# sandialabs/PyNucleus

Measured on AMD Instinct MI355X. Metric: element-pairs/sec assembled (2D P1 fractional s=0.5, dense) + % fp64 roofline, higher is better.
Workload: dtype f64; 1 GPU; 2D unit disc (uniform_disc refined 7x, 98304 cells), P1, 48769 DoFs, fractional s=0.5, horizon=inf, dense getDense incl. zeroExterior; 4831887360 element pairs/step; noRef=7, num_dofs=48769, num_cells=98304, parallelism=block rows of the upper triangle dealt over 1 GPU(s), row-owned one-sided slabs

## Files before the change

include/pnl_hip.h:

```cpp
#ifndef PNL_HIP_H
#define PNL_HIP_H
#include <stdint.h>

#ifdef __cplusplus
extern "C" {
#endif

typedef struct pnl_context pnl_context;

enum pnl_status {
    PNL_OK = 0,
    PNL_ERR_INVALID = -1,
    PNL_ERR_UNSUPPORTED = -2,
    PNL_ERR_HIP = -3,
    PNL_ERR_STATE = -4,
    PNL_ERR_ORDER = -5
};

enum pnl_kernel_type { PNL_FRACTIONAL = 0, PNL_INDICATOR = 1, PNL_PERIDYNAMIC = 2, PNL_GAUSSIAN = 3, PNL_EXPONENTIAL = 4,
                       PNL_GAUSSIAN_BOUNDARY = 5, PNL_EXPONENTIAL_BOUNDARY = 6 };

typedef struct {
    int32_t ktype;
    int32_t interaction;
    double exponent;
    double scale;
    double horizon2;
} pnl_kernel;

typedef struct {
    double c0, a, b, e, den0;
    int32_t clip_num;
    int32_t pad;
} pnl_order_formula;

#define PNL_INTERIOR 0
#define PNL_BOUNDARY 1

enum pnl_counter {
    PNL_C_NUM_CELL_PAIRS = 0,
    PNL_C_NUM_ASSEMBLED_CELL_PAIRS,
    PNL_C_NUM_INTEGRATIONS,
    PNL_C_NUM_BOUNDARY_PAIRS,
    PNL_C_NUM_BOUNDARY_INTEGRATIONS,
    PNL_C_ORDER_OVERFLOW,
    PNL_C_UNIFORM_TILE_PAIRS,
    PNL_C_RESERVED7,
    PNL_C_HIST0 = 8,
    PNL_C_UNIFORM_Q2 = 131,
    PNL_C_SETTLED_TILES = 134,
    PNL_C_CODE_BUILDS = 135,
    PNL_C_WORKLIST_LENGTH = 136
};
#define PNL_NUM_COUNTERS 137

int pnl_set_option(const char *name, const char *value);

enum { PNL_SELFTEST_LOG = 0, PNL_SELFTEST_EXP = 1, PNL_SELFTEST_EXP_RANGED = 2, PNL_SELFTEST_KERNEL = 3, PNL_SELFTEST_SCALING = 4,
       PNL_SELFTEST_QORDER = 5, PNL_SELFTEST_SETTLED_LAYOUT = 6 };
#define PNL_SELFTEST_DISPATCH 100
int pnl_selftest(int op, int path, int dim, int boundary, const void *param, int n, const double *in, double *out);

int pnl_create(int device_id, pnl_context **ctx);
void pnl_destroy(pnl_context *ctx);
const char *pnl_error_string(pnl_context *ctx);
const char *pnl_version(void);
int pnl_set_stream(pnl_context *ctx, void *hip_stream);
int pnl_synchronize(pnl_context *ctx);

int pnl_upload_mesh(pnl_context *ctx, int dim, int nv, const double *vertices_host, int nc, const int32_t *cells_host,
                    const double *vol_host, const double *h_host, double H0);
int pnl_set_cell_order(pnl_context *ctx, int nc, const int32_t *orig_host);
int pnl_set_interaction_transform(pnl_context *ctx, int dim, const double *T_host);
int pnl_upload_dofmap(pnl_context *ctx, int dpe, int dofs_per_vertex, int dofs_per_edge, int num_dofs,
                      const int32_t *dofs_host, const int32_t *dof_perm_table_host);
int pnl_set_classes(pnl_context *ctx, int nclasses, int num_labels, const int32_t *cell_labels_host,
                    const int32_t *facet_labels_host, const int32_t *cls_of_host);
int pnl_set_nonsymmetric(pnl_context *ctx, int on);
int pnl_select_class(pnl_context *ctx, int k);
int pnl_set_kernel(pnl_context *ctx, int which, const pnl_kernel *kernel);
int pnl_set_order_formula(pnl_context *ctx, int which, const pnl_order_formula *formula);
int pnl_upload_distant_rules(pnl_context *ctx, int qmax, const int32_t *off_host, const double *bary_host,
                             const double *w_host, const double *phi_host, const int32_t *foff_host,
                             const double *fbary_host, const double *fw_host);
int pnl_upload_singular_rule(pnl_context *ctx, int which, int panel, int M, int rows, const double *nodes_host,
                             const double *w_host, const double *psi_host, double fac);
int pnl_upload_boundary(pnl_context *ctx, int nb, const int32_t *bcells_host);

int pnl_assemble_pairs_in_horizon(pnl_context *ctx, double *data, double *diag);
int pnl_assemble_pairs_in_horizon_range(pnl_context *ctx, double *data_dev, double *diag_dev, int cell_begin, int cell_end);

#define PNL_FLAG_NO_MIRROR 1
#define PNL_FLAG_SYMMETRIC_FLUSH 2
int pnl_assemble_dense(pnl_context *ctx, double *A_dev, int64_t ldA, int zero_exterior, int cell_begin, int cell_end,
                       int flags);
int pnl_block_row_costs(pnl_context *ctx, double *cost_out, int n);
int pnl_dense_overwrites(pnl_context *ctx, int cell_begin, int cell_end, int flags);
int pnl_tile_cells(pnl_context *ctx);
int pnl_assemble_dense_tiles(pnl_context *ctx, double *A_dev, int64_t ldA, int zero_exterior, int ntiles,
                             const int32_t *tiles_host, int cell_begin, int cell_end, int flags);
int pnl_upload_sparsity(pnl_context *ctx, int nnz, const int32_t *indptr_host, const int32_t *indices_host);
int pnl_upload_sparsity_device(pnl_context *ctx, int nnz, const int32_t *indptr_dev, const int32_t *indices_dev);
int pnl_assemble_pairs_masked(pnl_context *ctx, int np, const int32_t *pairs_host, const uint64_t *masks_host,
                              double *data_dev, double *diag_dev);
int pnl_assemble_boundary_masked(pnl_context *ctx, int ni, const int32_t *cells_host, const int32_t *facets_host,
                                 const uint32_t *masks_host, double fac, double *data_dev, double *diag_dev);
typedef struct {
    int32_t npairs, nnodes, nchunks, chunk_stride, ntiles, num_dslots, nfacets, tile;
    const int32_t *pair_nodes, *node_off, *node_dofs;
    const int32_t *chunk_cells, *chunk_ndof, *chunk_dofs;
    const int16_t *chunk_slot;
    const int32_t *tile_chunkA, *tile_chunkB, *tile_pair, *tile_flags, *tile_dslotA, *tile_dslotB;
    const int32_t *d_cell, *d_pair;
    int32_t n_sing[3];
    int32_t n_btouch;
    const int32_t *sing_items[3];
    const int32_t *pair_foff, *fvid;
    const int32_t *bt_slot, *bt_cell, *bt_facet;
} pnl_cluster_plan;
int pnl_assemble_clusters_tiled(pnl_context *ctx, const pnl_cluster_plan *plan, int cluster_boundary, double *data_dev,
                                double *diag_dev);
typedef struct {
    int32_t nnodes, nleaves, nfar, m, nlevels, nq;
    const double *box;
    const int32_t *parent, *level;
    const int32_t *leaf_node, *leaf_dof_off, *leaf_dofs, *leaf_cell_off, *leaf_cells;
    const int32_t *far;
    const double *transfer;
    const double *qbary, *qw, *qphi;
    const int32_t *far_class;
    int32_t partial_leaves;
} pnl_h2_plan;
int pnl_h2_setup(pnl_context *ctx, const pnl_h2_plan *plan);
int pnl_h2_matvec(pnl_context *ctx, const double *x_dev, double *y_dev);
int pnl_h2_upward(pnl_context *ctx, const double *x_dev, double *cup_dev);
int pnl_h2_interact(pnl_context *ctx, const double *cup_dev, double *cdown_dev);
int pnl_h2_downward(pnl_context *ctx, double *cdown_dev, double *y_dev);
int pnl_h2_sizes(pnl_context *ctx, int32_t *out2);
int pnl_h2_get(pnl_context *ctx, int which, double *dst_host);
int pnl_h2_set(pnl_context *ctx, int which, const double *src_host);

int pnl_spmv(pnl_context *ctx, const double *data_dev, const double *diag_dev, const double *x_dev, double *y_dev);

typedef struct pnl_order_function {
    int32_t type, normalized;
    double p[6];
    int32_t scal_n, pad;
    double scal_mid, scal_half;
    double scal_cheb[32];
} pnl_order_function;

int pnl_set_order_function(pnl_context *ctx, const pnl_order_function *f, const double *cell_smax, const double *facet_smax,
                           double c0, double bc0, double sing_fac, double bsing_fac);
int pnl_set_order_vertex_values(pnl_context *ctx, int nv, const double *values_host);
int pnl_upload_pointwise_rules(pnl_context *ctx, int which, int panel, int nkeys, int M, int rows, const double *nodes,
                               const double *w, const double *phi0, const double *phi1);
int pnl_assemble_dense_pointwise(pnl_context *ctx, double *A, int64_t ldA, int zero_exterior, int cell_begin, int cell_end,
                                 int npairs, const int32_t *pairs, int nbpairs, const int32_t *bpairs);
int pnl_assemble_pairs_masked_pointwise(pnl_context *ctx, int np, const int32_t *pairs, const uint64_t *masks, const int32_t *rule,
                                        double *data);
int pnl_assemble_boundary_masked_pointwise(pnl_context *ctx, int ni, const int32_t *cells, const int32_t *facets, const uint32_t *masks,
                                           const int32_t *rule, const double *sv, double fac, double *data, double *diag);

int pnl_get_counters(pnl_context *ctx, int64_t *out, int n);
int pnl_get_phase_ms(pnl_context *ctx, float *out, int n);
int pnl_get_fold_stages(pnl_context *ctx, int64_t *out, int n);
int pnl_get_fold_plan(pnl_context *ctx, int32_t *images, int64_t nimages, int8_t *tile_stage, int8_t *tile_order, int64_t ntiles);
int pnl_get_settled_tiles(pnl_context *ctx, int32_t *tiles, int64_t ntiles);
enum pnl_kernel_slot { PNL_K_TILE_GENERAL = 0, PNL_K_TILE_UNIFORM2, PNL_K_TILE_UNIFORM3, PNL_K_TILE_UNIFORM4, PNL_K_FOLD_MIRROR,
                       PNL_K_WORKLIST, PNL_K_TILE_SETTLED, PNL_NUM_KERNEL_SLOTS };
int pnl_get_kernel_ms(pnl_context *ctx, float *out, int n);

typedef struct pnl_tree pnl_tree;
typedef struct pnl_nfplan pnl_nfplan;
int pnl_tree_build(int N, int dim, const double *boxes, const int64_t *d2c_ptr, const int32_t *d2c_idx, int nc, double eta,
                   int min_size, int max_levels, int do_admissibility, pnl_tree **out);
int pnl_tree_build_blocks(int N, int dim, const double *boxes, const int64_t *d2c_ptr, const int32_t *d2c_idx, int nc, double eta,
                          int min_size, int max_levels, int do_admissibility, const int32_t *dof_block, int mixed_block,
                          pnl_tree **out);
int pnl_tree_build_refined(int N, int dim, const double *boxes, const int64_t *d2c_ptr, const int32_t *d2c_idx, int nc, double eta,
                           int min_size, int max_levels, int do_admissibility, const int32_t *dof_block, int mixed_block, int ref_type,
                           pnl_tree **out);
int pnl_tree_build_horizon(int N, int dim, const double *boxes, const int64_t *d2c_ptr, const int32_t *d2c_idx, int nc, double eta,
                           int min_size, int max_levels, int do_admissibility, const int32_t *dof_block, int mixed_block, int ref_type,
                           double horizon, pnl_tree **out);
int pnl_tree_build_device(int N, int dim, const double *boxes, const int64_t *d2c_ptr, const int32_t *d2c_idx, int nc, double eta,
                          int min_size, int max_levels, int do_admissibility, int ref_type, pnl_tree **out);
void pnl_tree_destroy(pnl_tree *T);
int pnl_tree_sizes(const pnl_tree *T, int64_t *out3);
int pnl_tree_get(const pnl_tree *T, int32_t *range, int32_t *parent, int32_t *children, int32_t *level, double *box, int32_t *perm,
                 int32_t *near, int32_t *far);
int pnl_tree_node_cells(const pnl_tree *T, int n, const int32_t *node_ids, int64_t *off, int32_t *cells);
int pnl_h2_transfer_matrices(int nnodes, int dim, int m, const double *box, const int32_t *parent, double *out);
int pnl_nfplan_build(int dim, int nv, const double *vertices, int nc, const int32_t *cells, int dpe, int N, const int32_t *dofs,
                     int nnodes, const int64_t *node_off, const int32_t *node_dofs, const int64_t *node_cell_off,
                     const int32_t *node_cells, int npairs, const int32_t *pair_nodes, int tile, int max_chunk_dofs,
                     pnl_nfplan **out);
void pnl_nfplan_destroy(pnl_nfplan *P);
int pnl_nfplan_sizes(const pnl_nfplan *P, int64_t *out9);
int pnl_nfplan_get(const pnl_nfplan *P, int which, void *dst);

typedef struct pnl_pattern pnl_pattern;
int pnl_horizon_pattern(int dim, int nv, const double *vertices, int nc, const int32_t *cells, int dpe, int N, const int32_t *dofs,
                        double delta, int strict_lower, pnl_pattern **out);
int pnl_near_pattern(const pnl_tree *T, int npairs, const int32_t *pairs, int strict_lower, pnl_pattern **out);
int64_t pnl_pattern_set_max_nnz(int64_t max_nnz);
int64_t pnl_pattern_nnz(const pnl_pattern *P);
int pnl_pattern_get(const pnl_pattern *P, int32_t *indptr, int32_t *indices);
void pnl_pattern_destroy(pnl_pattern *P);

int pnl_set_row_slab(pnl_context *ctx, int nrows, const int32_t *rowdofs_host, int ncols, const int32_t *coldofs_host);
int pnl_diag_blocks_size(pnl_context *ctx);
int pnl_get_diag_blocks(pnl_context *ctx, double *dst_dev);
int pnl_slab_matvec(pnl_context *ctx, const double *slab_dev, int64_t ld, const double *diag_blocks_dev, const double *x_dev,
                    double *y_dev);
int pnl_slab_diagonal(pnl_context *ctx, const double *slab_dev, int64_t ld, const double *diag_blocks_dev, double *diag_dev);

int pnl_gemv(pnl_context *ctx, const double *A_dev, int64_t ldA, int n, const double *x_dev, double *y_dev,
             int symmetric_half);
int pnl_cg_jacobi(pnl_context *ctx, const double *A_dev, int64_t ldA, int n, const double *b_dev, double *x_dev,
                  double tol, int maxiter, int *iters, double *residual);

int pnl_gemv_axpby(pnl_context *ctx, const double *A_dev, int64_t ldA, int nrows, int ncols, const double *x_dev, double alpha,
                   double beta, const double *b_dev, double *y_dev);
int pnl_csr_matvec(pnl_context *ctx, int nrows, const int32_t *indptr_dev, const int32_t *indices_dev, const double *data_dev,
                   const double *x_dev, double alpha, double beta, double *y_dev);
typedef struct {
    int32_t n;
    int32_t pad;
    const double *A_dev;
    int64_t ldA;
    const double *diag_dev;
    const int32_t *R_indptr_dev, *R_indices_dev;
    const double *R_data_dev;
    const int32_t *P_indptr_dev, *P_indices_dev;
    const double *P_data_dev;
    int32_t kind, pad2;
    const int32_t *near_indptr_dev, *near_indices_dev;
    const double *near_data_dev;
} pnl_mg_level_desc;
typedef struct pnl_mg pnl_mg;
int pnl_mg_create(pnl_context *ctx, int nlevels, const pnl_mg_level_desc *levels, const double *coarse_inverse_dev, double omega,
                  int presmooth, int postsmooth, pnl_mg **out);
int pnl_mg_destroy(pnl_mg *mg);
int pnl_mg_cycle(pnl_mg *mg, const double *b_dev, double *x_dev, int x_is_zero);
int pnl_mg_solve(pnl_mg *mg, const double *b_dev, double *x_dev, double tol, int maxiter, int x_is_zero, int *iters, double *residuals,
                 int residuals_cap);
int pnl_mg_cg(pnl_mg *mg, const double *A_dev, int64_t ldA, const double *b_dev, double *x_dev, double tol, int maxiter, int x_is_zero,
              int *iters, double *residuals, int residuals_cap);
int pnl_theta_step(pnl_mg *mg, const double *S_dev, int64_t ldS, const int32_t *M_indptr_dev, const int32_t *M_indices_dev,
                   const double *M_data_dev, double dt, double theta, const double *forcing_dev, double *u_dev, double tol, int maxiter,
// ... 53 lines not shown
```

pynucleus_amd/_lib.py:

```python
import ctypes as C
import os
import numpy as np

_HERE = os.path.dirname(os.path.abspath(__file__))
LIB_PATH = os.environ.get('PNL_LIB', os.path.join(_HERE, 'libpnl_hip.so'))

PNL_OK = 0
PNL_ERR_INVALID = -1
PNL_ERR_UNSUPPORTED = -2
PNL_ERR_HIP = -3
PNL_ERR_STATE = -4
PNL_ERR_ORDER = -5
PNL_INTERIOR = 0
PNL_BOUNDARY = 1
PNL_FLAG_NO_MIRROR = 1
PNL_FLAG_SYMMETRIC_FLUSH = 2
PNL_NUM_COUNTERS = 137

EXPORTS = ['pnl_create', 'pnl_destroy', 'pnl_error_string', 'pnl_version', 'pnl_set_stream', 'pnl_synchronize',
           'pnl_upload_mesh', 'pnl_upload_dofmap', 'pnl_set_kernel', 'pnl_set_order_formula', 'pnl_upload_distant_rules',
           'pnl_upload_singular_rule', 'pnl_upload_boundary', 'pnl_assemble_dense', 'pnl_dense_overwrites', 'pnl_block_row_costs', 'pnl_tile_cells',
           'pnl_assemble_dense_tiles', 'pnl_get_counters', 'pnl_get_phase_ms', 'pnl_get_kernel_ms', 'pnl_get_fold_stages', 'pnl_get_fold_plan', 'pnl_get_settled_tiles', 'pnl_tree_build', 'pnl_tree_build_blocks', 'pnl_tree_build_refined', 'pnl_tree_build_horizon', 'pnl_tree_build_device', 'pnl_tree_destroy', 'pnl_tree_sizes', 'pnl_tree_get', 'pnl_tree_node_cells', 'pnl_h2_transfer_matrices', 'pnl_nfplan_build', 'pnl_nfplan_destroy', 'pnl_nfplan_sizes', 'pnl_nfplan_get', 'pnl_horizon_pattern', 'pnl_near_pattern', 'pnl_pattern_set_max_nnz', 'pnl_set_option', 'pnl_set_cell_order', 'pnl_set_interaction_transform', 'pnl_set_order_vertex_values', 'pnl_h2_get', 'pnl_h2_set', 'pnl_pattern_nnz', 'pnl_pattern_get', 'pnl_pattern_destroy', 'pnl_set_row_slab', 'pnl_diag_blocks_size', 'pnl_get_diag_blocks', 'pnl_slab_matvec', 'pnl_slab_diagonal', 'pnl_gemv', 'pnl_cg_jacobi',
           'pnl_inv_diagonal', 'pnl_set_classes', 'pnl_select_class', 'pnl_upload_sparsity', 'pnl_upload_sparsity_device', 'pnl_assemble_pairs_masked', 'pnl_assemble_boundary_masked', 'pnl_assemble_clusters_tiled', 'pnl_h2_setup', 'pnl_h2_matvec', 'pnl_h2_upward', 'pnl_h2_interact', 'pnl_h2_downward', 'pnl_h2_sizes', 'pnl_spmv',
           'pnl_assemble_pairs_in_horizon', 'pnl_assemble_pairs_in_horizon_range', 'pnl_set_nonsymmetric', 'pnl_set_order_function', 'pnl_upload_pointwise_rules', 'pnl_assemble_dense_pointwise',
           'pnl_assemble_pairs_masked_pointwise', 'pnl_assemble_boundary_masked_pointwise',
           'pnl_gemv_axpby', 'pnl_csr_matvec', 'pnl_mg_create', 'pnl_mg_destroy', 'pnl_mg_cycle', 'pnl_mg_solve', 'pnl_mg_cg', 'pnl_theta_step', 'pnl_selftest',
           'pnl_potrf', 'pnl_potrs', 'pnl_getrf', 'pnl_getrs',
           'pnl_csr_cg_jacobi', 'pnl_fe_space_create', 'pnl_fe_space_destroy', 'pnl_assemble_nonlinearity', 'pnl_imex_create',
           'pnl_imex_destroy', 'pnl_imex_sweep', 'pnl_lincomb', 'pnl_gemv_multi']

PNL_FUN_BRUSSELATOR, PNL_FUN_CUBIC = 0, 1
PNL_IMEX_CG_MG, PNL_IMEX_CHOL = 0, 1
PNL_IMEX_MAX_STAGES, PNL_IMEX_MAX_COMP = 4, 2
PNL_INTERP_MAX_OPS = 21


def source_sha16():
    import glob
    import hashlib
    root = os.path.dirname(_HERE)
    files = sorted(glob.glob(os.path.join(_HERE, 'csrc', '*.h'))+glob.glob(os.path.join(_HERE, 'csrc', '*.hip'))
                   +[os.path.join(root, 'include', 'pnl_hip.h'), os.path.join(_HERE, 'csrc', 'Makefile')])
    h = hashlib.sha256()
    for fn in files:
        with open(fn, 'rb') as f:
            h.update(os.path.basename(fn).encode()+b'\0'+f.read())
    return h.hexdigest()[:16]


class pnl_kernel(C.Structure):
    _fields_ = [('ktype', C.c_int32), ('interaction', C.c_int32), ('exponent', C.c_double), ('scale', C.c_double),
                ('horizon2', C.c_double)]


class pnl_order_formula(C.Structure):
    _fields_ = [('c0', C.c_double), ('a', C.c_double), ('b', C.c_double), ('e', C.c_double), ('den0', C.c_double),
                ('clip_num', C.c_int32), ('pad', C.c_int32)]


class pnl_mg_level_desc(C.Structure):
    _fields_ = [('n', C.c_int32), ('pad', C.c_int32), ('A_dev', C.c_void_p), ('ldA', C.c_int64), ('diag_dev', C.c_void_p),
                ('R_indptr_dev', C.c_void_p), ('R_indices_dev', C.c_void_p), ('R_data_dev', C.c_void_p),
                ('P_indptr_dev', C.c_void_p), ('P_indices_dev', C.c_void_p), ('P_data_dev', C.c_void_p),
                ('kind', C.c_int32), ('pad2', C.c_int32), ('near_indptr_dev', C.c_void_p), ('near_indices_dev', C.c_void_p),
                ('near_data_dev', C.c_void_p)]


class pnl_order_function(C.Structure):
    _fields_ = [('type', C.c_int32), ('normalized', C.c_int32), ('p', C.c_double*6), ('scal_n', C.c_int32), ('pad', C.c_int32),
                ('scal_mid', C.c_double), ('scal_half', C.c_double), ('scal_cheb', C.c_double*32)]


class pnl_cluster_plan(C.Structure):
    _fields_ = ([(n, C.c_int32) for n in ('npairs', 'nnodes', 'nchunks', 'chunk_stride', 'ntiles', 'num_dslots', 'nfacets', 'tile')] +
                [(n, C.c_void_p) for n in ('pair_nodes', 'node_off', 'node_dofs', 'chunk_cells', 'chunk_ndof', 'chunk_dofs', 'chunk_slot',
                                           'tile_chunkA', 'tile_chunkB', 'tile_pair', 'tile_flags', 'tile_dslotA', 'tile_dslotB',
                                           'd_cell', 'd_pair')] +
                [('n_sing', C.c_int32*3), ('n_btouch', C.c_int32), ('sing_items', C.c_void_p*3)] +
                [(n, C.c_void_p) for n in ('pair_foff', 'fvid', 'bt_slot', 'bt_cell', 'bt_facet')])


class pnl_h2_plan(C.Structure):
    _fields_ = ([(n, C.c_int32) for n in ('nnodes', 'nleaves', 'nfar', 'm', 'nlevels', 'nq')] +
                [(n, C.c_void_p) for n in ('box', 'parent', 'level', 'leaf_node', 'leaf_dof_off', 'leaf_dofs', 'leaf_cell_off',
                                           'leaf_cells', 'far', 'transfer', 'qbary', 'qw', 'qphi', 'far_class')] +
                [('partial_leaves', C.c_int32)])


class pnl_imex_desc(C.Structure):
    _fields_ = ([(n, C.c_int32) for n in ('s', 'ncomp', 'n', 'fun', 'nparams', 'solver', 'maxiter', 'mass_maxiter')] +
                [('AE', C.c_double*(PNL_IMEX_MAX_STAGES**2)), ('AI', C.c_double*(PNL_IMEX_MAX_STAGES**2)),
                 ('bE', C.c_double*PNL_IMEX_MAX_STAGES), ('bI', C.c_double*PNL_IMEX_MAX_STAGES),
                 ('mass_scale', C.c_double*PNL_IMEX_MAX_COMP), ('params', C.c_double*4),
                 ('dt', C.c_double), ('tol', C.c_double), ('mass_tol', C.c_double),
                 ('S_dev', C.c_void_p), ('ldS', C.c_int64), ('M_indptr_dev', C.c_void_p), ('M_indices_dev', C.c_void_p),
                 ('M_data_dev', C.c_void_p), ('space', C.c_void_p), ('mg', C.c_void_p*PNL_IMEX_MAX_COMP),
                 ('chol_dev', C.c_void_p*PNL_IMEX_MAX_COMP), ('ldchol', C.c_int64*PNL_IMEX_MAX_COMP)])


class PnlError(RuntimeError):
    pass


_LIB = None


def load():
    global _LIB
    if _LIB is not None:
        return _LIB
    if not os.path.exists(LIB_PATH):
        raise PnlError('{} is missing: the HIP extension has not been built (run __graft_entry__.build()); '
                       'there is no CPU fallback for the assembly path'.format(LIB_PATH))
    import torch
    L = C.CDLL(LIB_PATH)
    vp, i32, i64, dbl = C.c_void_p, C.c_int, C.c_int64, C.c_double
    L.pnl_create.argtypes = [i32, C.POINTER(vp)]
    L.pnl_destroy.argtypes = [vp]
    L.pnl_destroy.restype = None
    L.pnl_error_string.argtypes = [vp]
    L.pnl_error_string.restype = C.c_char_p
    L.pnl_version.restype = C.c_char_p
    L.pnl_set_stream.argtypes = [vp, vp]
    L.pnl_synchronize.argtypes = [vp]
    L.pnl_upload_mesh.argtypes = [vp, i32, i32, vp, i32, vp, vp, vp, dbl]
    L.pnl_upload_dofmap.argtypes = [vp, i32, i32, i32, i32, vp, vp]
    L.pnl_set_kernel.argtypes = [vp, i32, C.POINTER(pnl_kernel)]
    L.pnl_selftest.argtypes = [i32, i32, i32, i32, vp, i32, vp, vp]
    L.pnl_set_order_formula.argtypes = [vp, i32, C.POINTER(pnl_order_formula)]
    L.pnl_upload_distant_rules.argtypes = [vp, i32, vp, vp, vp, vp, vp, vp, vp]
    L.pnl_upload_singular_rule.argtypes = [vp, i32, i32, i32, i32, vp, vp, vp, dbl]
    L.pnl_upload_boundary.argtypes = [vp, i32, vp]
    L.pnl_assemble_dense.argtypes = [vp, vp, i64, i32, i32, i32, i32]
    L.pnl_dense_overwrites.argtypes = [vp, i32, i32, i32]
    L.pnl_block_row_costs.argtypes = [vp, vp, i32]
    L.pnl_tile_cells.argtypes = [vp]
    L.pnl_assemble_dense_tiles.argtypes = [vp, vp, i64, i32, i32, vp, i32, i32, i32]
    L.pnl_get_counters.argtypes = [vp, vp, i32]
    L.pnl_get_phase_ms.argtypes = [vp, vp, i32]
    L.pnl_get_kernel_ms.argtypes = [vp, vp, i32]
    L.pnl_get_fold_stages.argtypes = [vp, vp, i32]
    L.pnl_get_fold_plan.argtypes = [vp, vp, C.c_int64, vp, vp, C.c_int64]
    L.pnl_get_settled_tiles.argtypes = [vp, vp, C.c_int64]
    L.pnl_set_row_slab.argtypes = [vp, i32, vp, i32, vp]
    L.pnl_tree_build.argtypes = [i32, i32, vp, vp, vp, i32, dbl, i32, i32, i32, C.POINTER(vp)]
    L.pnl_tree_build_blocks.argtypes = [i32, i32, vp, vp, vp, i32, dbl, i32, i32, i32, vp, i32, C.POINTER(vp)]
    L.pnl_tree_build_refined.argtypes = [i32, i32, vp, vp, vp, i32, dbl, i32, i32, i32, vp, i32, i32, C.POINTER(vp)]
    L.pnl_tree_build_horizon.argtypes = [i32, i32, vp, vp, vp, i32, dbl, i32, i32, i32, vp, i32, i32, dbl, C.POINTER(vp)]
    L.pnl_tree_build_device.argtypes = [i32, i32, vp, vp, vp, i32, dbl, i32, i32, i32, i32, C.POINTER(vp)]
    L.pnl_tree_destroy.argtypes = [vp]
    L.pnl_tree_destroy.restype = None
    L.pnl_tree_sizes.argtypes = [vp, vp]
    L.pnl_tree_get.argtypes = [vp, vp, vp, vp, vp, vp, vp, vp, vp]
    L.pnl_tree_node_cells.argtypes = [vp, i32, vp, vp, vp]
    L.pnl_h2_transfer_matrices.argtypes = [i32, i32, i32, vp, vp, vp]
    L.pnl_nfplan_build.argtypes = [i32, i32, vp, i32, vp, i32, i32, vp, i32, vp, vp, vp, vp, i32, vp, i32, i32, C.POINTER(vp)]
    L.pnl_nfplan_destroy.argtypes = [vp]
    L.pnl_nfplan_destroy.restype = None
    L.pnl_nfplan_sizes.argtypes = [vp, vp]
    L.pnl_nfplan_get.argtypes = [vp, i32, vp]
    L.pnl_horizon_pattern.argtypes = [i32, i32, vp, i32, vp, i32, i32, vp, dbl, i32, C.POINTER(vp)]
    L.pnl_near_pattern.argtypes = [vp, i32, vp, i32, C.POINTER(vp)]
    L.pnl_pattern_nnz.argtypes = [vp]
    L.pnl_pattern_set_max_nnz.argtypes = [i64]
    L.pnl_set_option.argtypes = [C.c_char_p, C.c_char_p]
    L.pnl_set_cell_order.argtypes = [vp, i32, vp]
    L.pnl_set_interaction_transform.argtypes = [vp, i32, vp]
    L.pnl_set_order_vertex_values.argtypes = [vp, i32, vp]
    L.pnl_h2_get.argtypes = [vp, i32, vp]
    L.pnl_h2_set.argtypes = [vp, i32, vp]
    L.pnl_pattern_get.argtypes = [vp, vp, vp]
    L.pnl_pattern_destroy.argtypes = [vp]
    L.pnl_diag_blocks_size.argtypes = [vp]
    L.pnl_get_diag_blocks.argtypes = [vp, vp]
    L.pnl_slab_matvec.argtypes = [vp, vp, i64, vp, vp, vp]
    L.pnl_slab_diagonal.argtypes = [vp, vp, i64, vp, vp]
    L.pnl_gemv.argtypes = [vp, vp, i64, i32, vp, vp, i32]
    L.pnl_cg_jacobi.argtypes = [vp, vp, i64, i32, vp, vp, dbl, i32, C.POINTER(C.c_int), C.POINTER(C.c_double)]
    L.pnl_inv_diagonal.argtypes = [vp, vp, i64, i32, vp]
    L.pnl_gemv_axpby.argtypes = [vp, vp, i64, i32, i32, vp, dbl, dbl, vp, vp]
    L.pnl_csr_matvec.argtypes = [vp, i32, vp, vp, vp, vp, dbl, dbl, vp]
    L.pnl_mg_create.argtypes = [vp, i32, C.POINTER(pnl_mg_level_desc), vp, dbl, i32, i32, C.POINTER(C.c_void_p)]
    L.pnl_mg_destroy.argtypes = [vp]
    L.pnl_mg_cycle.argtypes = [vp, vp, vp, i32]
    L.pnl_mg_solve.argtypes = [vp, vp, vp, dbl, i32, i32, C.POINTER(C.c_int), C.POINTER(C.c_double), i32]
    L.pnl_mg_cg.argtypes = [vp, vp, i64, vp, vp, dbl, i32, i32, C.POINTER(C.c_int), C.POINTER(C.c_double), i32]
    L.pnl_theta_step.argtypes = [vp, vp, i64, vp, vp, vp, dbl, dbl, vp, vp, dbl, i32, C.POINTER(C.c_int), C.POINTER(C.c_double)]
    L.pnl_potrf.argtypes = [vp, vp, i64, i32, C.POINTER(C.c_int)]
    L.pnl_potrs.argtypes = [vp, vp, i64, i32, vp, i64, i32]
    L.pnl_getrf.argtypes = [vp, vp, i64, i32, vp, C.POINTER(C.c_int)]
    L.pnl_getrs.argtypes = [vp, vp, i64, i32, vp, vp, i64, i32]
    L.pnl_csr_cg_jacobi.argtypes = [vp, i32, vp, vp, vp, dbl, vp, vp, dbl, i32, i32, C.POINTER(C.c_int), C.POINTER(C.c_double)]
    L.pnl_fe_space_create.argtypes = [vp, i32, i32, i32, i32, vp, vp, vp, vp, C.POINTER(vp)]
    L.pnl_fe_space_destroy.argtypes = [vp]
    L.pnl_assemble_nonlinearity.argtypes = [vp, i32, vp, i32, i32, vp, i64, i32, dbl, dbl, vp, i64]
    L.pnl_imex_create.argtypes = [vp, C.POINTER(pnl_imex_desc), C.POINTER(vp)]
    L.pnl_imex_destroy.argtypes = [vp]
    L.pnl_imex_sweep.argtypes = [vp, vp, vp, vp, vp]
    L.pnl_lincomb.argtypes = [vp, i32, vp, i64, i32, i32, vp, vp, i64]
    L.pnl_gemv_multi.argtypes = [vp, i32, vp, i64, i32, i32, vp, vp, dbl, dbl, vp, vp]
    L.pnl_upload_sparsity.argtypes = [vp, i32, vp, vp]
    L.pnl_upload_sparsity_device.argtypes = [vp, i32, vp, vp]
    L.pnl_set_classes.argtypes = [vp, i32, i32, vp, vp, vp]
    L.pnl_select_class.argtypes = [vp, i32]
    L.pnl_set_nonsymmetric.argtypes = [vp, i32]
    L.pnl_assemble_pairs_masked.argtypes = [vp, i32, vp, vp, vp, vp]
    L.pnl_assemble_boundary_masked.argtypes = [vp, i32, vp, vp, vp, dbl, vp, vp]
    L.pnl_spmv.argtypes = [vp, vp, vp, vp, vp]
    L.pnl_assemble_clusters_tiled.argtypes = [vp, C.POINTER(pnl_cluster_plan), i32, vp, vp]
    L.pnl_h2_setup.argtypes = [vp, C.POINTER(pnl_h2_plan)]
    L.pnl_h2_matvec.argtypes = [vp, vp, vp]
    L.pnl_h2_upward.argtypes = [vp, vp, vp]
    L.pnl_h2_interact.argtypes = [vp, vp, vp]
    L.pnl_h2_downward.argtypes = [vp, vp, vp]
    L.pnl_h2_sizes.argtypes = [vp, vp]
    L.pnl_assemble_pairs_in_horizon.argtypes = [vp, vp, vp]
    L.pnl_assemble_pairs_in_horizon_range.argtypes = [vp, vp, vp, i32, i32]
    L.pnl_set_order_function.argtypes = [vp, C.POINTER(pnl_order_function), vp, vp, dbl, dbl, dbl, dbl]
    L.pnl_upload_pointwise_rules.argtypes = [vp, i32, i32, i32, i32, i32, vp, vp, vp, vp]
    L.pnl_assemble_dense_pointwise.argtypes = [vp, vp, i64, i32, i32, i32, i32, vp, i32, vp]
    L.pnl_assemble_pairs_masked_pointwise.argtypes = [vp, i32, vp, vp, vp, vp]
    L.pnl_assemble_boundary_masked_pointwise.argtypes = [vp, i32, vp, vp, vp, vp, vp, dbl, vp, vp]
    for name in EXPORTS:
        f = getattr(L, name)
        if name in ('pnl_pattern_nnz', 'pnl_pattern_set_max_nnz'):
            f.restype = C.c_int64
# ... 216 lines not shown
        ip, pip = _hp(indptr, np.int32)
        ix, pix = _hp(indices, np.int32)
        self.check(self.L.pnl_upload_sparsity(self.h, ix.shape[0], pip, pix))

    def upload_sparsity_device(self, indptr_t, indices_t):
        self.check(self.L.pnl_upload_sparsity_device(self.h, int(indices_t.numel()), C.c_void_p(indptr_t.data_ptr()),
                                                     C.c_void_p(indices_t.data_ptr()) if indices_t.numel() else None))

    def assemble_pairs_masked(self, pairs, masks, data_ptr, diag_ptr=None):
        p, pp = _hp(pairs, np.int32)
        if masks is None:
            pm = None
        else:
            m, pm = _hp(masks, np.uint64)
            assert m.shape == (p.shape[0], 4)
        assert p.ndim == 2 and p.shape[1] == 2
        self.check(self.L.pnl_assemble_pairs_masked(self.h, p.shape[0], pp, pm, C.c_void_p(data_ptr),
                                                    C.c_void_p(diag_ptr) if diag_ptr else None))

    def assemble_pairs_masked_pointwise(self, pairs, masks, rule, data_ptr):
        p, pp = _hp(pairs, np.int32)
        m, pm = _hp(masks, np.uint64)
        r, pr = _hp(rule, np.int32)
        assert p.ndim == 2 and p.shape[1] == 2 and m.shape == (p.shape[0], 4) and r.shape == (p.shape[0],)
        self.check(self.L.pnl_assemble_pairs_masked_pointwise(self.h, p.shape[0], pp, pm, pr, C.c_void_p(data_ptr)))

    def assemble_boundary_masked_pointwise(self, cells, facets, masks, rule, sv, fac, data_ptr, diag_ptr=None):
        c, pc = _hp(cells, np.int32)
        f, pf = _hp(facets, np.int32)
        m, pm = _hp(masks, np.uint32)
        r, pr = _hp(rule, np.int32)
        s_, ps = _hp(sv, np.float64)
        assert f.shape[0] == c.shape[0] == m.shape[0] == r.shape[0] == s_.shape[0]
        self.check(self.L.pnl_assemble_boundary_masked_pointwise(self.h, c.shape[0], pc, pf, pm, pr, ps, float(fac), C.c_void_p(data_ptr),
                                                                 C.c_void_p(diag_ptr) if diag_ptr else None))

    def select_class(self, k):
        self.check(self.L.pnl_select_class(self.h, int(k)))

    def assemble_boundary_masked(self, cells, facets, masks, fac, data_ptr, diag_ptr=None):
        c, pc = _hp(cells, np.int32)
        f, pf = _hp(facets, np.int32)
        m, pm = _hp(masks, np.uint32)
        assert f.shape[0] == c.shape[0] == m.shape[0]
        self.check(self.L.pnl_assemble_boundary_masked(self.h, c.shape[0], pc, pf, pm, float(fac), C.c_void_p(data_ptr),
                                                       C.c_void_p(diag_ptr) if diag_ptr else None))

    def assemble_clusters_tiled(self, plan, cluster_boundary, data_ptr, diag_ptr=None):
        keep = []

        def ptr(a, dt):
            a = np.ascontiguousarray(a, dtype=dt)
            keep.append(a)
            return a.ctypes.data

        P = pnl_cluster_plan()
        P.npairs, P.nnodes, P.nchunks = plan.num_pairs, len(plan.nodes), plan.chunk_cells.shape[0]
        P.chunk_stride, P.ntiles, P.num_dslots = plan.nU, plan.tile_chunkA.shape[0], plan.num_dslots
        P.nfacets, P.tile = plan.fvid.shape[0], plan.tile
        for name in ('pair_nodes', 'node_off', 'node_dofs', 'chunk_cells', 'chunk_ndof', 'chunk_dofs', 'tile_chunkA', 'tile_chunkB',
                     'tile_pair', 'tile_flags', 'tile_dslotA', 'tile_dslotB', 'd_cell', 'd_pair', 'pair_foff', 'fvid', 'bt_slot',
                     'bt_cell', 'bt_facet'):
            setattr(P, name, ptr(getattr(plan, name), np.int32))
        P.chunk_slot = ptr(plan.chunk_slot, np.int16)
        for s in range(3):
            P.n_sing[s] = plan.sing_items[s].shape[0]
            P.sing_items[s] = ptr(plan.sing_items[s], np.int32)
        P.n_btouch = plan.bt_cell.shape[0]
        self.check(self.L.pnl_assemble_clusters_tiled(self.h, C.byref(P), int(bool(cluster_boundary)), C.c_void_p(data_ptr),
                                                      C.c_void_p(diag_ptr) if diag_ptr else None))

    def spmv(self, data_ptr, diag_ptr, x_ptr, y_ptr):
        self.check(self.L.pnl_spmv(self.h, C.c_void_p(data_ptr), C.c_void_p(diag_ptr) if diag_ptr else None, C.c_void_p(x_ptr),
                                   C.c_void_p(y_ptr)))

    def counters(self):
        out = np.zeros(PNL_NUM_COUNTERS, dtype=np.int64)
        self.check(self.L.pnl_get_counters(self.h, out.ctypes.data, PNL_NUM_COUNTERS))
        hist = {q: int(out[8+q]) for q in range(120) if out[8+q]}
        sing = {-1-k: int(out[128+k]) for k in range(3)}
        return dict(numCellPairs=int(out[0]), numAssembledCellPairs=int(out[1]), numIntegrations=int(out[2]),
                    numBoundaryPairs=int(out[3]), numBoundaryIntegrations=int(out[4]), orders=hist, singular=sing,
                    uniformTilePairs=int(out[6]), uniformTilePairsByOrder={2+k: int(out[131+k]) for k in range(3)},
                    settledTiles=int(out[134]), codeBuilds=int(out[135]), workListLength=int(out[136]))

    def phase_ms(self):
        out = np.zeros(7, dtype=np.float32)
        self.check(self.L.pnl_get_phase_ms(self.h, out.ctypes.data, 7))
        return dict(tiles=float(out[0]), tiles_uniform=float(out[6]), worklist=float(out[1]), singular=float(out[2]),
                    boundary=float(out[3]), scatter_mirror=float(out[4]), total=float(out[5]))

    def set_row_slab(self, rowdofs, coldofs):
        rd = np.ascontiguousarray(rowdofs, dtype=np.int32)
        cd = np.ascontiguousarray(coldofs, dtype=np.int32)
        self.check(self.L.pnl_set_row_slab(self.h, int(rd.shape[0]), rd.ctypes.data if rd.shape[0] else None, int(cd.shape[0]),
                                           cd.ctypes.data if cd.shape[0] else None))

    def diag_blocks_size(self):
        n = self.L.pnl_diag_blocks_size(self.h)
        self.check(min(n, 0))
        return n

    def get_diag_blocks(self, dst_ptr):
        self.check(self.L.pnl_get_diag_blocks(self.h, C.c_void_p(dst_ptr)))

    def slab_matvec(self, slab_ptr, ld, dblocks_ptr, x_ptr, y_ptr):
        self.check(self.L.pnl_slab_matvec(self.h, C.c_void_p(slab_ptr), int(ld), C.c_void_p(dblocks_ptr), C.c_void_p(x_ptr), C.c_void_p(y_ptr)))

    def slab_diagonal(self, slab_ptr, ld, dblocks_ptr, diag_ptr):
        self.check(self.L.pnl_slab_diagonal(self.h, C.c_void_p(slab_ptr), int(ld), C.c_void_p(dblocks_ptr), C.c_void_p(diag_ptr)))

    def kernel_ms(self):
        out = np.zeros(7, dtype=np.float32)
        self.check(self.L.pnl_get_kernel_ms(self.h, out.ctypes.data, 7))
        return dict(tile_general=float(out[0]), tile_uniform2=float(out[1]), tile_uniform3=float(out[2]), tile_uniform4=float(out[3]),
                    fold_mirror=float(out[4]), worklist=float(out[5]), tile_settled=float(out[6]))

    def fold_stages(self):
        out = np.zeros((17, 5), dtype=np.int64)
        n = self.L.pnl_get_fold_stages(self.h, out.ctypes.data, 17)
        self.check(min(n, 0))
        return [dict(images=int(r[0]), uniform={2: int(r[1]), 3: int(r[2]), 4: int(r[3])}, mixed=int(r[4])) for r in out[:n]]

    def settled_tiles(self):
        n = self.L.pnl_get_settled_tiles(self.h, None, 0)
        self.check(min(n, 0))
        tiles = np.zeros((n, 2), dtype=np.int32)
        if n:
            self.check(min(self.L.pnl_get_settled_tiles(self.h, tiles.ctypes.data, n), 0))
        return tiles

    def fold_plan(self, nblocks):
        nimg = sum(s['images'] for s in self.fold_stages())
        images = np.zeros((nimg, 3), dtype=np.int32)
        stage = np.zeros((nblocks, nblocks), dtype=np.int8)
        order = np.zeros((nblocks, nblocks), dtype=np.int8)
        self.check(self.L.pnl_get_fold_plan(self.h, images.ctypes.data, nimg, stage.ctypes.data, order.ctypes.data, nblocks*nblocks))
        return images, stage, order

    def gemv(self, A_ptr, ldA, n, x_ptr, y_ptr, symmetric_half=False):
        self.check(self.L.pnl_gemv(self.h, C.c_void_p(A_ptr), int(ldA), int(n), C.c_void_p(x_ptr), C.c_void_p(y_ptr),
                                   int(symmetric_half)))

    def cg_jacobi(self, A_ptr, ldA, n, b_ptr, x_ptr, tol, maxiter):
        it, res = C.c_int(0), C.c_double(0.)
        self.check(self.L.pnl_cg_jacobi(self.h, C.c_void_p(A_ptr), int(ldA), int(n), C.c_void_p(b_ptr), C.c_void_p(x_ptr),
                                        float(tol), int(maxiter), C.byref(it), C.byref(res)))
        return it.value, res.value

    def gemv_axpby(self, A_ptr, ldA, nrows, ncols, x_ptr, alpha, beta, b_ptr, y_ptr):
        self.check(self.L.pnl_gemv_axpby(self.h, C.c_void_p(A_ptr), int(ldA), int(nrows), int(ncols), C.c_void_p(x_ptr), float(alpha),
                                         float(beta), C.c_void_p(b_ptr) if b_ptr else None, C.c_void_p(y_ptr)))

    @staticmethod
    def _block_list(A_ptrs, coeffs):
        c = np.ascontiguousarray(coeffs, dtype=np.float64)
        assert c.ndim == 1 and c.shape[0] == len(A_ptrs)
        return (C.c_void_p*max(len(A_ptrs), 1))(*[int(p) if p else None for p in A_ptrs]), c

    def lincomb(self, A_ptrs, ldA, nrows, ncols, coeffs, B_ptr, ldB):
        arr, c = self._block_list(A_ptrs, coeffs)
        self.check(self.L.pnl_lincomb(self.h, len(A_ptrs), arr, int(ldA), int(nrows), int(ncols), c.ctypes.data, C.c_void_p(B_ptr) if B_ptr else None,
                                      int(ldB)))

    def gemv_multi(self, A_ptrs, ldA, nrows, ncols, coeffs, x_ptr, alpha, beta, b_ptr, y_ptr):
        arr, c = self._block_list(A_ptrs, coeffs)
        self.check(self.L.pnl_gemv_multi(self.h, len(A_ptrs), arr, int(ldA), int(nrows), int(ncols), c.ctypes.data, C.c_void_p(x_ptr), float(alpha),
                                         float(beta), C.c_void_p(b_ptr) if b_ptr else None, C.c_void_p(y_ptr)))

    def csr_matvec(self, nrows, indptr_ptr, indices_ptr, data_ptr, x_ptr, alpha, beta, y_ptr):
        self.check(self.L.pnl_csr_matvec(self.h, int(nrows), C.c_void_p(indptr_ptr), C.c_void_p(indices_ptr), C.c_void_p(data_ptr),
                                         C.c_void_p(x_ptr), float(alpha), float(beta), C.c_void_p(y_ptr)))

    def mg_create(self, descs, coarse_inverse_ptr, omega, presmooth, postsmooth):
        arr = (pnl_mg_level_desc*len(descs))(*descs)
        out = C.c_void_p()
        self.check(self.L.pnl_mg_create(self.h, len(descs), arr, C.c_void_p(coarse_inverse_ptr), float(omega), int(presmooth), int(postsmooth),
                                        C.byref(out)))
        return out

    def mg_destroy(self, mg):
        self.L.pnl_mg_destroy(mg)

    def mg_cycle(self, mg, b_ptr, x_ptr, x_is_zero):
        self.check(self.L.pnl_mg_cycle(mg, C.c_void_p(b_ptr), C.c_void_p(x_ptr), int(bool(x_is_zero))))

    def mg_solve(self, mg, b_ptr, x_ptr, tol, maxiter, x_is_zero):
        it = C.c_int(0)
        res = (C.c_double*(maxiter+2))()
        self.check(self.L.pnl_mg_solve(mg, C.c_void_p(b_ptr), C.c_void_p(x_ptr), float(tol), int(maxiter), int(bool(x_is_zero)), C.byref(it),
                                       res, maxiter+2))
        return it.value, list(res[:it.value+1])

    def mg_cg(self, mg, A_ptr, ldA, b_ptr, x_ptr, tol, maxiter, x_is_zero):
        it = C.c_int(0)
        res = (C.c_double*(maxiter+2))(*([float('nan')]*(maxiter+2)))
        self.check(self.L.pnl_mg_cg(mg, C.c_void_p(A_ptr) if A_ptr else None, int(ldA), C.c_void_p(b_ptr), C.c_void_p(x_ptr), float(tol),
                                    int(maxiter), int(bool(x_is_zero)), C.byref(it), res, maxiter+2))
        out = list(res)
        while len(out) > 1 and out[-1] != out[-1]:
            out.pop()
        return it.value, out

    def theta_step(self, mg, S_ptr, ldS, M_indptr_ptr, M_indices_ptr, M_data_ptr, dt, theta, forcing_ptr, u_ptr, tol, maxiter):
        it, res = C.c_int(0), C.c_double(0.)
        self.check(self.L.pnl_theta_step(mg, C.c_void_p(S_ptr), int(ldS), C.c_void_p(M_indptr_ptr), C.c_void_p(M_indices_ptr),
                                         C.c_void_p(M_data_ptr), float(dt), float(theta), C.c_void_p(forcing_ptr) if forcing_ptr else None,
                                         C.c_void_p(u_ptr), float(tol), int(maxiter), C.byref(it), C.byref(res)))
        return it.value, res.value

    def potrf(self, A_ptr, ldA, n):
        info = C.c_int(0)
        self.check(self.L.pnl_potrf(self.h, C.c_void_p(A_ptr) if A_ptr else None, int(ldA), int(n), C.byref(info)))
# ... 64 lines not shown
```

pynucleus_amd/csrc/pnl_context.h:

```cpp
#pragma once
#include <hip/hip_runtime.h>
#include <algorithm>
#include <cmath>
#include <cstdarg>
#include <cstdio>
#include <cstring>
#include <string>
#include <vector>
#include "pnl_hip.h"
#include "pnl_device.h"

constexpr int TILE_P1 = 64;
constexpr int TILE_P2 = 32;

struct DevBuf {
    void *p = nullptr;
    size_t bytes = 0;
    ~DevBuf() { release(); }
    void release() { if (p) { (void)hipFree(p); p = nullptr; bytes = 0; } }
};

enum PhaseEvent {
    EV_START = 0,
    EV_WORKLIST_DONE = 1,
    EV_MIRROR_DONE = 2,
    EV_SINGULAR_DONE = 3,
    EV_BOUNDARY_DONE = 4,
    EV_END = 5,
    EV_TILES_DONE = 6,
    EV_TILES_UNIFORM_DONE = 7,
    EV_COUNT = 8
};

struct AssemblyRun {
    bool ev_valid = false;
    bool tiles_launched = false, pure_launched = false;
    bool symflush = false;
    bool tile_cell_filter = true;
    bool full_tile_list = false;
    bool slot_used = false, fold_event_set = false, stg_active = false;
    int settled_run = 0;
    int tile_off = 0, n_mixed = 0, n_pure = 0;
    int wl_slots = 0;
    int uni_ctr_next = 0, uni_ctr_fresh = 0;
    int kev_n[PNL_NUM_KERNEL_SLOTS] = {}; bool kev_open[PNL_NUM_KERNEL_SLOTS] = {};
    unsigned long long visited_pairs = 0;
    bool visited_is_assembled = false;
};

struct pnl_context {
    int device = 0;
    hipStream_t own_stream = nullptr, stream = nullptr;
    static constexpr int NAUX = 4;
    hipStream_t aux[NAUX] = {};
    hipEvent_t ev_fork = nullptr, ev_join[NAUX] = {};
    hipEvent_t ev_fold = nullptr;
    static constexpr int MAX_STAGES = 16;
    hipEvent_t ev_stage[MAX_STAGES+1] = {};
    hipEvent_t ev_bnd = nullptr;
    std::string err;
    int dim = 0, nv = 0, nc = 0, dpe = 0, dpv = 0, dped = 0, N = 0, nb = 0, qmax = -1;
    int nreal = 0;
    std::vector<int> cell_orig;
    std::vector<int> real_from;
    double H0 = 0.;
    std::vector<double> vertices, vol, h;
    std::vector<int32_t> cells, dofs, perm_table, bcells;
    struct ClassData {
        pnl_kernel kern[2];
        pnl_order_formula form[2];
        bool have_kernel[2] = {false, false}, have_form[2] = {false, false};
        bool have_sing[2][3] = {{false, false, false}, {false, false, false}};
        DevBuf b_sn[3], b_sw[3], b_sp[3], b_bn[2], b_bw[2], b_bp[2], b_spairs[3], b_bpairs[2], b_spairs1[3];
        int sM[3] = {0, 0, 0}, sRows[3] = {0, 0, 0}, bM[2] = {0, 0};
        double sFac = 0., bFac = 0.;
        int n_spairs[3] = {0, 0, 0}, n_bpairs[2] = {0, 0};
        int n_spairs1[3] = {0, 0, 0};
        ClassData() { std::memset(kern, 0, sizeof(kern)); std::memset(form, 0, sizeof(form)); }
    };
    std::vector<ClassData*> cls;
    int cur = 0;
    ClassData &C() { return *cls[cur]; }
    int nlab = 0;
    bool nonsym = false;
    int orient = 0;
    std::vector<int32_t> cell_labels, facet_labels, cls_of;
    bool have_mesh = false, have_dofs = false, have_rules = false, have_boundary = false;
    bool dirty = true;
    DevProblem P;
    DevBuf b_cellv, b_ccen, b_cvol, b_ch, b_clog, b_cvid, b_cdof, b_cslot, b_blk_ndof, b_blk_dofs, b_perm, b_off, b_bary, b_w, b_phi,
        b_foff, b_fbary, b_fw, b_bvid, b_bv, b_bgeo, b_counters, b_D, b_tiles,
        b_vec[6], b_clabel, b_blabel, b_clsof, b_scal, b_wl, b_wlcount, b_tilectr, b_ttn, b_ttoff, b_tttab, b_ttwphi, b_wlsorted, b_wlaux,
        b_vertices, b_sp_indptr, b_sp_indices, b_mp_pairs, b_mp_masks, b_mp_wl, b_mp_sorted, b_mp_aux, b_bi_cells, b_bi_facets,
        b_bi_masks, b_cp[28], b_cpD, b_wlds, b_wlpair, b_h2[20];
    DevBuf b_kcls, b_fcls, b_uni, b_tilecls, b_ttwphif;
    DevBuf b_scolbase, b_srowoff, b_cpoff, b_cpslot, b_cprow, b_foldtab, b_bkcls, b_bfcls, b_bdefer, b_multitiles, b_slotA, b_candtiles, b_candq;
    int slot_S = 0, n_multitiles = 0;
    DevBuf b_codes;
    int n_settled = 0, settled_want = -1;
    std::vector<int2> settled_tiles;
    long long code_builds = 0;
    std::vector<int32_t> rng_blk_off, rng_blk;
    DevBuf b_foldimg, b_unictr;
    int stg_K = 0, stg_want = -1;
    std::vector<int> stg_img_off;
    std::vector<int> stg_uni_off[3];
    std::vector<unsigned> stg_img;
    std::vector<signed char> stg_tile_stage;
    std::vector<unsigned char> stg_tile_q;
    static constexpr int UNI_CTRS = 64;
    long long slot_total = 0;
    DevBuf b_rowmap, b_rowdof, b_colmap, b_coldof;
    DevBuf b_cholinfo;
    DevBuf b_luwork, b_lutmp;
    std::vector<int32_t> slab_rowdofs, slab_coldofs;
    int slab_rows = 0, slab_cols = 0;
    std::vector<DevKernel> kcls_host;
    std::vector<DevKernel> bkcls_host;
    std::vector<DevFormula> bfcls_host;
    std::vector<DevFormula> fcls_host;
    int uni_off[5] = {-1, -1, -1, -1, -1}, uni_np[5] = {0, 0, 0, 0, 0};
    bool uni_struct[5] = {false, false, false, false, false};
    H2Dev h2;
    bool have_h2 = false;
    bool have_tile_order = false;
    struct TileOrderJob *tile_job = nullptr;
    DevBuf b_cellv_t, b_cdof_t, b_cslot_t, b_Dt;
    PwDev pw;
    bool have_pw = false, have_pw_rules[2][3] = {{false, false, false}, {false, false, false}};
    int pw_nkeys[2] = {0, 0};
    std::vector<double> pw_cell_smax, pw_facet_smax;
    std::vector<double> pw_vertex_s;
    DevBuf b_pw_cellsv;
    DevBuf b_pw_csm, b_pw_fsm, b_pw_rule[2][3][4], b_pw_pairs, b_pw_bpairs;
    std::vector<std::vector<int>> h2_levels;
    long long h2_vtot = 0;
    std::vector<size_t> h2_level_off;
    std::vector<int32_t> rule_off, frule_off;
    int sp_nnz = -1;
    unsigned wl_cap = 0;
    int tile = TILE_P1, nblocks = 0, ncp = 0, nU = 0;
    std::vector<int2> spairs_host[3];
    std::vector<int2> tiles_cached;
    size_t tiles_cap = 0;
    int tiles_cb = -1, tiles_ce = -1;
    std::vector<int> cls_tile_off, cls_n_mixed, cls_n_pure;
    std::vector<int> cls_n_uni[3];
    bool single_launch = false;
    int sl_off[4] = {0, 0, 0, 0}, sl_n[4] = {0, 0, 0, 0};
    unsigned wl_cap_each = 0;
    std::vector<pnl_order_formula> tiles_forms;
    pnl_order_formula tiles_form;
    bool tiles_filter = true;
    bool use_pure = true;
    struct PowTab { double exponent, scale; DevBuf buf; };
    std::vector<PowTab*> powtabs;
    struct BlockAgg { double cx, cy, rad, hmax, hmin, Lmin, Lmax; bool full; double tcx, tcy, trad; };
    bool have_xform = false;
    double xform[4] = {1., 0., 0., 1.};
    std::vector<BlockAgg> blocks;
    hipEvent_t ev[EV_COUNT] = {};
    std::vector<hipEvent_t> kev[PNL_NUM_KERNEL_SLOTS];
    AssemblyRun run;
    int ablate = 0;
    bool wl_lane = true;
};

inline void pnl_begin_assembly(pnl_context *ctx) { ctx->run = AssemblyRun{}; }

inline int fail(pnl_context *ctx, int code, const char *fmt, ...) {
    char buf[512];
    va_list ap;
    va_start(ap, fmt);
    vsnprintf(buf, sizeof(buf), fmt, ap);
    va_end(ap);
    if (ctx) ctx->err = buf;
    return code;
}

#define HIPCHK(ctx, call)                                                                            \
    do {                                                                                             \
        hipError_t e_ = (call);                                                                      \
// ... 74 lines not shown
const char *pnl_tune(const char *name);
inline int pnl_grid_cap(int grid) {
    const char *e = pnl_tune("PNL_TILE_WGS");
    const int cap = e ? atoi(e) : 0;
    return cap > 0 ? std::max(1, std::min(grid, cap)) : grid;
}

inline int acc_stride_of(int nU, size_t fixed_bytes = 0) {
    int st = nU+1;
    const int m = pnl_tune("PNL_ACC_PAD") ? atoi(pnl_tune("PNL_ACC_PAD")) : 32;
    if (m > 1) {
        int padded = st;
        while (padded % m != 1) padded++;
        if (fixed_bytes+sizeof(double)*(size_t)(nU+1)*padded <= 80*1024) st = padded;
        else if (st % 2 == 0 && fixed_bytes+sizeof(double)*(size_t)(nU+1)*(st+1) <= 80*1024) st++;
    }
    return st;
}

inline DevProblem tile_problem(const pnl_context *ctx) {
    DevProblem Pt = ctx->P;
    if (ctx->have_tile_order) {
        Pt.cellv = (const double*)ctx->b_cellv_t.p; Pt.cdof = (const int*)ctx->b_cdof_t.p; Pt.cslot = (const short*)ctx->b_cslot_t.p;
    }
    return Pt;
}

inline DevProblem with_mixed_rules(const pnl_context *ctx, DevProblem Pt) {
    Pt.uni = (const double*)ctx->b_uni.p;
    Pt.mix_struct = 0;
    const bool generic = pnl_tune("PNL_MIXED_GENERIC") != nullptr;
    for (int q = 0; q < 5; q++) {
        Pt.uni_off[q] = ctx->uni_off[q] >= 0 ? ctx->uni_off[q] : 0;
        if (q >= 2 && q <= ctx->qmax && ctx->dim == 2 && ctx->dpe == 3 && ctx->uni_off[q] >= 0 && ctx->uni_struct[q] && !generic)
            Pt.mix_struct |= 1 << q;
    }
    return Pt;
}

inline void kt_begin(pnl_context *ctx, int slot) {
    std::vector<hipEvent_t> &v = ctx->kev[slot];
    const size_t k = 2*(size_t)ctx->run.kev_n[slot];
    ctx->run.kev_open[slot] = false;
    while (v.size() < k+2) {
        hipEvent_t e = nullptr;
        if (hipEventCreate(&e) != hipSuccess) { (void)hipGetLastError(); return; }
        v.push_back(e);
    }
    ctx->run.kev_open[slot] = hipEventRecord(v[k], ctx->stream) == hipSuccess;
}
inline void kt_end(pnl_context *ctx, int slot) {
    if (!ctx->run.kev_open[slot]) return;
    ctx->run.kev_open[slot] = false;
    if (hipEventRecord(ctx->kev[slot][2*(size_t)ctx->run.kev_n[slot]+1], ctx->stream) == hipSuccess) ctx->run.kev_n[slot]++;
}

int pnl_tile_order_ready(pnl_context *ctx);

int pnl_assembly_prepare(pnl_context *ctx);
int pnl_assembly_ready(pnl_context *ctx);
void pnl_refresh_tables(pnl_context *ctx);

struct StreamScope {
    pnl_context *ctx;
    hipStream_t prev;
    StreamScope(pnl_context *c, hipStream_t stream) : ctx(c), prev(c->stream) { ctx->stream = stream; }
    StreamScope(const StreamScope&) = delete; StreamScope &operator=(const StreamScope&) = delete;
    void to(hipStream_t stream) { ctx->stream = stream; }
    ~StreamScope() { ctx->stream = prev; }
};
struct ClassScope {
    pnl_context *ctx;
    int leave_at;
    bool refresh_after;
    ClassScope(pnl_context *c, int leave_at_, bool refresh_after_ = false) : ctx(c), leave_at(leave_at_), refresh_after(refresh_after_) {}
    ClassScope(const ClassScope&) = delete; ClassScope &operator=(const ClassScope&) = delete;
    void select(int k, int orient) { ctx->cur = k; ctx->orient = orient; pnl_refresh_tables(ctx); }
    ~ClassScope() { ctx->cur = leave_at; ctx->orient = 0; if (refresh_after) pnl_refresh_tables(ctx); }
};
int pnl_make_tiles(pnl_context *ctx, std::vector<int2> &tiles, int cell_begin, int cell_end);
int pnl_upload_tiles(pnl_context *ctx, std::vector<int2> &tiles, int cell_begin, int cell_end);
int pnl_tile_order_range(pnl_context *ctx, const DevFormula &qo, int ncand, signed char *host_out);
int pnl_tile_pair_codes(pnl_context *ctx, const DevFormula &qo, const int2 *tiles, int n, unsigned short *codes, int *host_stat);
struct WlBins { unsigned *hist, *offs, *coff, *cursor; };
int pnl_wl_sort(pnl_context *ctx, const int4 *wl, const unsigned *count, unsigned cap, unsigned *aux_base, int4 *sorted, WlBins &B);
void pnl_scatter_diag(pnl_context *ctx, const DevProblem &P, const double *D, double *A, int64_t ldA);
int pnl_tile_uniform_order(const pnl_context *ctx, const pnl_order_formula &F, int ta, int tb, int qlimit);
int pnl_sparse_ready(pnl_context *ctx, double *data, double *diag, SparseOut &S);

int pnl_pw_prepare(pnl_context *ctx, int need_boundary);
int pnl_pw_h2_interp(pnl_context *ctx);

int pnl_launch_gemv_symmetric(pnl_context *ctx, const double *A, long long ldA, int n, const double *x, double alpha, double beta,
                              const double *b, double *y);
int pnl_launch_slab_two_sided(pnl_context *ctx, const double *slab, long long ld, int nrows, int ncols, const int *rowdof, const int *coldof,
                              const double *x, double *y);

int pnl2_launch_uniform(pnl_context *ctx, int kt, const DevProblem &Pt, const int2 *tiles, const int *tile_cls, int ntiles, int q,
                        double *A, int64_t ldA, double *Dglob, const SlotOut &SO, int spare = 0);
int pnl2_launch_p2(pnl_context *ctx, int kt, const int2 *tiles, const int *tile_cls, int ntiles, double *A, int64_t ldA,
                   int cell_begin, int cell_end, unsigned wl_cap_each, const SlotOut &SO);
int pnl2_zero_slot_tiles(pnl_context *ctx, const SlotOut &SO);
int pnl2_fold_mirror(pnl_context *ctx, const SlotOut &SO, double *A, int64_t ldA, const unsigned *images = nullptr, int nimages = 0);
inline SlotOut slot_out(const pnl_context *ctx) {
    SlotOut SO;
    SO.A2 = (double*)ctx->b_slotA.p; SO.rowoff = (const long long*)ctx->b_srowoff.p; SO.colbase = (const int*)ctx->b_scolbase.p;
    SO.S = ctx->slot_S; SO.nU = ctx->nU;
    return SO;
}
```

pynucleus_amd/csrc/pnl_device.h:

```cpp
#pragma once
#include <hip/hip_runtime.h>
#include <stdint.h>

#define PNL_NTHREADS 256
#define PNL_MAXQ 120
#define PNL_NCOUNTERS 134
#define PNL_WL_SLOTS 256
#define PNL_WL_BINS 128
#define PNL_POW_TAB_DOUBLES 384
#define PNL_TT_MAXPTS 96
#define PNL_GEN_MAXPTS 16

struct DevKernel {
    int ktype;
    int fast;
    double exponent, scale, horizon2;
    int interaction, qm;
    double pb[6];
    const double *ptab;
};

struct DevFormula {
    double c0, a, b, e, den0;
    int clip;
    int pad;
};

struct DevProblem {
    int dim, dpe, nc, ncp, N, dpv, dped, nb;
    double H0;
    const double *cellv;
    const double *ccen;
    const double *cvol, *ch;
    const double *clog;
    const int *cvid;
    const int *cdof;
    const short *cslot;
    const int *blk_ndof;
    const int *blk_dofs;
    int blk_stride, nblocks;
    const int *perm_table;
    DevKernel k, bk;
    DevKernel bkn;
    DevFormula qo, bqo;
    int qmax, pad0;
    const int *off;
    const double *bary;
    const double *w;
    const double *phi;
    const int *foff;
    const double *fbary;
    const double *fw;
    const int *tt_n, *tt_off;
    const double *tt_tab;
    const double *tt_wphi;
    const double *tt_wphif;
    int tt_npts, pad1;
    int sM[3], sRows[3];
    const double *sNodes[3], *sW[3], *sPsi[3];
    double sFac;
    int bM[2];
    const double *bNodes[2], *bW[2], *bPhi[2];
    double bFac;
    const int *bvid;
    const double *bv;
    const double *bgeo;
    const int *clabel, *blabel, *cls_of;
    int nlab, cur_class;
    int orient, pad2;
    double idfac;
    unsigned long long *counters;
    const int *rowmap, *colmap;
    int onesided, pad3;
    const double *uni = nullptr;
    int uni_off[5] = {0, 0, 0, 0, 0};
    int mix_struct = 0;
};

#ifndef PNL_DIAG_MULT
#define PNL_DIAG_MULT 21
#endif
__host__ __device__ constexpr int tile_sweep_row(int tid, int k, int tile, int nt) { return k*(nt/tile)+tid/tile; }
__host__ __device__ constexpr int tile_diag_cell(int r, int j, int tile) { return (r+PNL_DIAG_MULT*j)%tile; }

__device__ __forceinline__ long long pnl_row(const DevProblem &P, int I) { return P.rowmap ? (long long)P.rowmap[I] : (long long)I; }
__device__ __forceinline__ int pnl_col(const DevProblem &P, int J) { return P.colmap ? P.colmap[J] : J; }

#define PNL_FOLD_TAB 63
struct FoldEntry { long long off; int ar, cy; };

struct H2Dev {
    int dim, m, M, nnodes, nleaves, nfar;
    const double *box;
    const int *parent;
    const int *leaf_node;
    const int *leaf_dof_off, *leaf_dofs;
    const int *leaf_cell_off, *leaf_cells;
    const long long *leaf_val_off;
    const int *far;
    double *V, *K;
    const double *T;
    double *cup, *cdown;
};

__device__ __forceinline__ double cheb_node(double a, double b, int m, int j) {
    return (b-a)*0.5*(cos((2.0*(m-j)-1.0)/(2.0*m)*3.14159265358979323846)+1.0)+a;
}

__device__ __forceinline__ double lagrange1d(double a, double b, int m, int l, double x) {
    const double xl = cheb_node(a, b, m, l);
    double v = 1.;
    for (int k = 0; k < m; k++)
        if (k != l) {
            const double xk = cheb_node(a, b, m, k);
            v *= (x-xk)/(xl-xk);
        }
    return v;
}

struct PwDev {
    int type, normalized;
    double p[6];
    int scal_n, pad0;
    double scal_mid, scal_inv_half, scal_cheb[32];
    double c0, bc0;
    const double *cell_smax, *facet_smax;
    int M[3], rows[3];
    const double *nodes[3], *w[3], *phi0[3], *phi1[3];
    int bM[2], pad;
    const double *bnodes[2], *bw[2], *bphi[2];
    double sfac, bfac;
    const double *cell_sv;
    long long sv_stride;
};

struct SparseOut {
    const int *indptr, *indices;
    double *data, *diag;
    const int *pairs;
    const unsigned long long *masks;
};

struct SlotOut {
    double *A2;
    const long long *rowoff;
    const int *colbase;
    int S, nU;
};
```

pynucleus_amd/csrc/pnl_hip.hip:

```cpp
#include "pnl_context.h"
#include "pnl_kernels.h"
#include "pnl_bndtile.h"
#include "pnl_launch.h"

namespace {

__global__ void __launch_bounds__(PNL_NTHREADS)
k_mirror(double *__restrict__ A, long long ldA, int N) {
    __shared__ double t1[32][33], t2[32][33];
    const int nb = (N+31)/32;
    int bid = blockIdx.x;
    int bi = 0;
    {
        double fb = ((2.*nb+1.)-sqrt((2.*nb+1.)*(2.*nb+1.)-8.*bid))*0.5;
        bi = (int)fb;
        while (bi > 0 && (long long)bi*nb-(long long)bi*(bi-1)/2 > bid) bi--;
        while ((long long)(bi+1)*nb-(long long)(bi+1)*bi/2 <= bid) bi++;
    }
    const int bj = bi+(bid-(int)((long long)bi*nb-(long long)bi*(bi-1)/2));
    const int tx = threadIdx.x & 31, ty = threadIdx.x >> 5;
    for (int r = ty; r < 32; r += 8) {
        const int I = bi*32+r, J = bj*32+tx;
        t1[r][tx] = (I < N && J < N) ? A[(long long)I*ldA+J] : 0.;
        const int I2 = bj*32+r, J2 = bi*32+tx;
// ... 61 lines not shown
        long long load[pnl_context::NAUX] = {};
        slot.assign(n, 0);
        for (int k : order) {
            int best = 0;
            for (int j = 1; j < pnl_context::NAUX; j++) if (load[j] < load[best]) best = j;
            slot[k] = best; load[best] += std::max(1, weight[k]);
        }
    }
    void use(int k) {
        if (!on) return;
        const int j = k < (int)slot.size() ? slot[k] : k % pnl_context::NAUX;
        if (!used[j]) { (void)hipStreamWaitEvent(ctx->aux[j], start, 0); used[j] = true; }
        scope.to(ctx->aux[j]);
    }
    void join() {
        if (!on) return;
        scope.to(scope.prev);
        for (int j = 0; j < pnl_context::NAUX; j++)
            if (used[j]) {
                (void)hipEventRecord(ctx->ev_join[j], ctx->aux[j]);
                (void)hipStreamWaitEvent(scope.prev, ctx->ev_join[j], 0);
                used[j] = false;
            }
        on = false;
    }
    ~ClassFork() { join(); }
};

template <int DIM, int DPE, int KT>
int run_worklist(pnl_context *ctx, const int4 *wl, const unsigned *wlc, unsigned cap, double *A, int64_t ldA, bool sym, int region = 0,
                 int nregions = 1) {
    int rc;
    if ((rc = ensure(ctx, ctx->b_wlsorted, (size_t)cap*nregions*sizeof(int4)))) return rc;
    if ((rc = ensure(ctx, ctx->b_wlaux, sizeof(unsigned)*(4*(PNL_WL_BINS+1))*nregions))) return rc;
    const int4 *wlsorted = (const int4*)ctx->b_wlsorted.p+(size_t)region*cap;
    WlBins B;
    if ((rc = pnl_wl_sort(ctx, wl, wlc, cap, (unsigned*)ctx->b_wlaux.p+(size_t)region*4*(PNL_WL_BINS+1), (int4*)wlsorted, B))) return rc;
    int dbg = 0;
#ifdef PNL_DEBUG_ABLATE
    dbg = pnl_tune("PNL_WL_DBG") ? atoi(pnl_tune("PNL_WL_DBG")) : 0;
#endif
    const int nmin = ctx->wl_lane ? PNL_WL_LANE_MAXPTS+1 : 0;
    return worklist_eval<DIM, DPE, KT, false>(ctx, "PNL_WL_LDS_KB", 18, wlsorted, B, A, ldA, (double*)ctx->b_D.p, SparseOut{}, ClusterTiles{},
                                              PNL_WL_BINS-1, nmin | (sym ? 1 << 16 : 0), ctx->wl_lane, dbg | (sym ? 8 : 0));
}

int ensure_worklist(pnl_context *ctx, double pairs, int regions) {
    const double frac = pnl_tune("PNL_WL_FRAC") ? atof(pnl_tune("PNL_WL_FRAC")) : 0.05;
    const double floor_entries = pnl_tune("PNL_WL_FRAC") ? 64. : (double)(1 << 20);
    const size_t each = (size_t)std::min<double>(std::max<double>(pairs*frac, floor_entries), 400e6);
    int rc;
    if ((rc = ensure(ctx, ctx->b_wl, each*(size_t)regions*sizeof(int4)))) return rc;
    ctx->wl_cap = (unsigned)std::min<size_t>(ctx->b_wl.bytes/sizeof(int4), 0xffffffffu);
    ctx->wl_cap_each = (unsigned)each;
    if ((rc = ensure(ctx, ctx->b_tilectr, sizeof(unsigned)))) return rc;
    return PNL_OK;
}

template <int DIM, int DPE, int TILE, int KT, bool SETTLED = false>
int launch_mixed_tiles(pnl_context *ctx, unsigned *wlc, double *A, int64_t ldA, int cell_begin, int cell_end, const SlotOut &SO) {
    using S = TileSmem<DIM, DPE, TILE, KT == 0>;
    constexpr bool can_settle = DIM == 2 && DPE == 3 && TILE == 64;
    int ntiles = ctx->run.n_mixed, first = 0, ns = 0;
    unsigned *ctr = (unsigned*)ctx->b_tilectr.p;
    if (can_settle && ctx->cls.size() == 1 && SO.A2 && !ctx->run.symflush && !ctx->nonsym && ctx->b_codes.p && cell_begin <= 0 && cell_end >= ctx->nc)
        ns = std::min(ctx->n_settled, ntiles);
    if (SETTLED) {
        first = ntiles-ns; ntiles = ns;
        ctr = (unsigned*)ctx->b_unictr.p+ctx->run.uni_ctr_next;
        ctx->run.uni_ctr_next = (ctx->run.uni_ctr_next+1)%pnl_context::UNI_CTRS;
        if (ctx->run.uni_ctr_fresh > 0) ctx->run.uni_ctr_fresh--;
        else HIPCHK(ctx, hipMemsetAsync(ctr, 0, sizeof(unsigned), ctx->stream));
    } else {
        ntiles -= ns;
        ctx->run.settled_run = ns;
        HIPCHK(ctx, hipMemsetAsync(ctr, 0, sizeof(unsigned), ctx->stream));
    }
    const int acc_stride = acc_stride_of(ctx->nU, S::fixed_bytes);
    const size_t lds = S::fixed_bytes+sizeof(double)*(size_t)(ctx->nU+1)*acc_stride;
    if (lds > 160*1024)
        return fail(ctx, PNL_ERR_UNSUPPORTED, "a block of %d cells touches %d DoFs: LDS sub-block of %zu bytes exceeds 160 KiB "
                    "(cells must be numbered with spatial locality)", TILE, ctx->nU, lds);
    auto kfun = k_tile_distant<DIM, DPE, TILE, KT, false, false, SETTLED>;
    const int grid_mult = pnl_tune("PNL_GRID_MULT") ? atoi(pnl_tune("PNL_GRID_MULT")) : 1;
    const PersistentGrid g = persistent_grid(ctx, kfun, tile_threads(DPE, KT), lds, ntiles, 2, grid_mult);
    if (g.rc) return g.rc;
    if (pnl_tune("PNL_VERBOSE"))
        fprintf(stderr, "[pnl] %stiles=%d nU=%d lds=%zu bytes, occupancy API: %d blocks/CU\n", SETTLED ? "settled " : "", ntiles, ctx->nU, lds, g.per_cu);
    SlotOut SOk = SO;
    SOk.nU = ctx->nU;
    kt_begin(ctx, PNL_K_TILE_GENERAL);
    if (SETTLED) kt_begin(ctx, PNL_K_TILE_SETTLED);
    if (g.grid > 0)
        hipLaunchKernelGGL(kfun, dim3(g.grid), dim3(tile_threads(DPE, KT)), lds, ctx->stream, with_mixed_rules(ctx, tile_problem(ctx)),
                           (const int2*)ctx->b_tiles.p+ctx->run.tile_off+first, A,
                           (long long)ldA, (double*)(ctx->have_tile_order ? ctx->b_Dt.p : ctx->b_D.p), cell_begin, cell_end, acc_stride, (int4*)ctx->b_wl.p,
                           wlc, ctx->wl_cap_each, ctx->ablate | (ctx->run.symflush ? 256 : 0), ntiles, ClusterTiles{},
                           ctr, SOk, SETTLED ? (const unsigned short*)ctx->b_codes.p : (const unsigned short*)nullptr);
    if (SETTLED) kt_end(ctx, PNL_K_TILE_SETTLED);
    kt_end(ctx, PNL_K_TILE_GENERAL);
    HIPCHK(ctx, hipGetLastError());
    if constexpr (can_settle && !SETTLED) {
        if (ns > 0) return launch_mixed_tiles<DIM, DPE, TILE, KT, true>(ctx, wlc, A, ldA, cell_begin, cell_end, SO);
    }
    return PNL_OK;
}

#ifndef PNL_UNI_SPARE_DEFAULT
#define PNL_UNI_SPARE_DEFAULT 1
#endif
template <int DIM, int DPE, int TILE, int KT>
int launch_tiles(pnl_context *ctx, int wl_slot, double *A, int64_t ldA, int cell_begin, int cell_end, const SlotOut &SO = SlotOut{}) {
    HIPCHK(ctx, hipEventRecord(ctx->ev[EV_TILES_UNIFORM_DONE], ctx->stream));
    ctx->run.pure_launched = false;
    const bool staged = DIM == 2 && DPE == 3 && SO.A2 && ctx->stg_K > 0 && ctx->cls.size() == 1 && !ctx->nonsym;
    ctx->run.stg_active = staged;
    if (staged) {
        int rc;
        const int K = ctx->stg_K;
        const int spare = pnl_tune("PNL_UNI_SPARE") ? atoi(pnl_tune("PNL_UNI_SPARE")) : PNL_UNI_SPARE_DEFAULT;
        const bool side = !pnl_tune("PNL_NO_OVERLAP");
        hipStream_t const caller = ctx->stream;
        hipStream_t const folds = side ? ctx->aux[2] : caller;
        constexpr int wl_aux = 3;
        hipStream_t const wls = side ? ctx->aux[wl_aux] : caller;
        const int2 *tiles = (const int2*)ctx->b_tiles.p+ctx->run.tile_off;
        double *Dt = (double*)(ctx->have_tile_order ? ctx->b_Dt.p : ctx->b_D.p);
        unsigned *wlc = (unsigned*)ctx->b_wlcount.p+wl_slot;
        auto uniform_stage = [&](int s, int spare_s) -> int {
            int off = ctx->run.n_mixed;
            for (int q = 2; q <= 4; q++) {
                const std::vector<int> &so = ctx->stg_uni_off[q-2];
                const int n = so[s+1]-so[s];
                int rcu = pnl2_launch_uniform(ctx, KT, tile_problem(ctx), tiles+off+so[s], nullptr, n, q, A, ldA, Dt, SO, spare_s);
                if (rcu) return rcu;
                ctx->run.pure_launched = ctx->run.pure_launched || n > 0;
                off += so[K+1];
            }
            return PNL_OK;
        };
        auto fold_stage = [&](int s) -> int {
            if (side) HIPCHK(ctx, hipStreamWaitEvent(folds, ctx->ev_stage[s], 0));
            StreamScope on(ctx, folds);
            return pnl2_fold_mirror(ctx, SO, A, ldA, (const unsigned*)ctx->b_foldimg.p+ctx->stg_img_off[s], ctx->stg_img_off[s+1]-ctx->stg_img_off[s]);
        };
        if ((rc = uniform_stage(0, 0))) return rc;
        HIPCHK(ctx, hipEventRecord(ctx->ev[EV_TILES_UNIFORM_DONE], ctx->stream));
        if ((rc = launch_mixed_tiles<DIM, DPE, TILE, KT>(ctx, wlc, A, ldA, cell_begin, cell_end, SO))) return rc;
        HIPCHK(ctx, hipEventRecord(ctx->ev_stage[0], caller));
        if ((rc = fold_stage(0))) return rc;
        HIPCHK(ctx, hipEventRecord(ctx->ev_fold, folds));
        ctx->run.fold_event_set = true;
        if (side && wls != folds) HIPCHK(ctx, hipStreamWaitEvent(wls, ctx->ev_fold, 0));
        {
            StreamScope on(ctx, wls);
            if ((rc = run_worklist<DIM, DPE, KT>(ctx, (const int4*)ctx->b_wl.p, wlc, ctx->wl_cap_each, A, ldA, true))) return rc;
        }
        if (side && wls != folds) HIPCHK(ctx, hipEventRecord(ctx->ev_join[wl_aux], wls));
        for (int s = 1; s <= K; s++) {
            if ((rc = uniform_stage(s, spare))) return rc;
            HIPCHK(ctx, hipEventRecord(ctx->ev_stage[s], caller));
            if ((rc = fold_stage(s))) return rc;
        }
        HIPCHK(ctx, hipEventRecord(ctx->ev[EV_TILES_DONE], caller));
        if (side) {
            HIPCHK(ctx, hipEventRecord(ctx->ev_join[2], folds));
            HIPCHK(ctx, hipStreamWaitEvent(caller, ctx->ev_join[2], 0));
            if (wls != folds) HIPCHK(ctx, hipStreamWaitEvent(caller, ctx->ev_join[wl_aux], 0));
        }
        return PNL_OK;
    }
    if (TILE == 64 && DPE <= 3) {
        int rc;
        if (DIM == 2 && DPE == 3 && !pnl_tune("PNL_PURE_V1") && ctx->uni_off[2] >= 0 && ctx->uni_np[2] == 3)
            rc = pnl2_launch_uniform(ctx, KT, tile_problem(ctx), (const int2*)ctx->b_tiles.p+ctx->run.tile_off+ctx->run.n_mixed, nullptr, ctx->run.n_pure, 2,
                                     A, ldA, (double*)(ctx->have_tile_order ? ctx->b_Dt.p : ctx->b_D.p), SO);
        else rc = launch_pure<DIM, (DPE <= 3 ? DPE : 3), KT>(ctx, A, ldA, SO);
        if (rc) return rc;
        ctx->run.pure_launched = ctx->run.n_pure > 0;
        if (DIM == 2 && DPE == 3) {
            int off = ctx->run.tile_off+ctx->run.n_mixed+ctx->run.n_pure;
// ... 531 lines not shown
__global__ void k_wl_scan(const unsigned *__restrict__ hist, unsigned *__restrict__ offs, unsigned *__restrict__ chunk_off,
                          unsigned *__restrict__ cursor) {
    if (threadIdx.x == 0) {
        unsigned run = 0, crun = 0;
        for (int q = 0; q < PNL_WL_BINS; q++) {
            offs[q] = run; chunk_off[q] = crun; cursor[q] = 0;
            run += hist[q]; crun += (hist[q]+15)/16;
        }
        offs[PNL_WL_BINS] = run; chunk_off[PNL_WL_BINS] = crun;
    }
}

__global__ void __launch_bounds__(PNL_NTHREADS)
k_wl_scatter(const int4 *__restrict__ wl, const unsigned *__restrict__ wl_count, unsigned wl_cap, const unsigned *__restrict__ offs,
             unsigned *__restrict__ cursor, int4 *__restrict__ sorted) {
    constexpr int NW = PNL_NTHREADS/64;
    __shared__ unsigned h[NW][PNL_WL_BINS], base[NW][PNL_WL_BINS];
    const unsigned count = min(*wl_count, wl_cap);
    const unsigned per = (count+gridDim.x-1)/gridDim.x;
    const unsigned b0 = blockIdx.x*per, b1 = min(count, b0+per);
    const int lane = threadIdx.x & 63, wave = threadIdx.x >> 6;
    const unsigned perw = ((b1 > b0 ? b1-b0 : 0u)+NW-1)/NW;
    const unsigned i0 = min(b1, b0+wave*perw), i1 = min(b1, i0+perw);
    const unsigned long long lt = (1ull << lane)-1ull;
    for (int t = threadIdx.x; t < NW*PNL_WL_BINS; t += PNL_NTHREADS) (&h[0][0])[t] = 0;
    __syncthreads();
    auto sweep = [&](bool place) {
        for (unsigned i = i0; i < i1; i += 64) {
            const bool act = i+lane < i1;
            int4 e = make_int4(0, 0, 0, 0);
            if (act) e = wl[i+lane];
            const int q = act ? ((e.w >> 16) & (PNL_WL_BINS-1)) : -1;
            unsigned long long todo = __ballot(act);
            while (todo) {
                const int leader = __ffsll((long long)todo)-1;
                const int qL = __builtin_amdgcn_readlane(q, leader);
                const unsigned long long same = __ballot(q == qL);
                if (place) {
                    const unsigned start = base[wave][qL]+h[wave][qL];
                    if (q == qL) sorted[start+__popcll(same & lt)] = e;
                }
                __builtin_amdgcn_wave_barrier();
                if (lane == leader) h[wave][qL] += (unsigned)__popcll(same);
                __builtin_amdgcn_fence(__ATOMIC_ACQ_REL, "wavefront");
                __builtin_amdgcn_wave_barrier();
                todo &= ~same;
            }
        }
    };
    sweep(false);
    __syncthreads();
    if (threadIdx.x < PNL_WL_BINS) {
        unsigned tot = 0;
        for (int w = 0; w < NW; w++) tot += h[w][threadIdx.x];
        unsigned run = tot ? offs[threadIdx.x]+atomicAdd(&cursor[threadIdx.x], tot) : 0u;
        for (int w = 0; w < NW; w++) { base[w][threadIdx.x] = run; run += h[w][threadIdx.x]; h[w][threadIdx.x] = 0; }
    }
    __syncthreads();
    sweep(true);
}

int pnl_wl_sort(pnl_context *ctx, const int4 *wl, const unsigned *count, unsigned cap, unsigned *aux_base, int4 *sorted, WlBins &B) {
    B.hist = aux_base; B.offs = B.hist+(PNL_WL_BINS+1); B.coff = B.offs+(PNL_WL_BINS+1); B.cursor = B.coff+(PNL_WL_BINS+1);
    HIPCHK(ctx, hipMemsetAsync(B.hist, 0, sizeof(unsigned)*(PNL_WL_BINS+1), ctx->stream));
    hipLaunchKernelGGL(k_wl_hist, dim3(512), dim3(PNL_NTHREADS), 0, ctx->stream, wl, count, cap, B.hist);
    hipLaunchKernelGGL(k_wl_scan, dim3(1), dim3(64), 0, ctx->stream, (const unsigned*)B.hist, B.offs, B.coff, B.cursor);
    hipLaunchKernelGGL(k_wl_scatter, dim3(512), dim3(PNL_NTHREADS), 0, ctx->stream, wl, count, cap, (const unsigned*)B.offs, B.cursor, sorted);
    return PNL_OK;
}

int pnl_tile_pair_codes(pnl_context *ctx, const DevFormula &qo, const int2 *tiles, int n, unsigned short *codes, int *host_stat) {
    if (n <= 0) return PNL_OK;
    if (ctx->tile != 64) return fail(ctx, PNL_ERR_STATE, "pair codes: tiles of 64 cells");
    int rc;
    if (host_stat && (rc = ensure(ctx, ctx->b_candq, sizeof(int)*(size_t)n))) return rc;
    DevProblem P = ctx->P;
    P.qmax = ctx->qmax;
    P.tt_n = (const int*)ctx->b_ttn.p;
    if (!P.tt_n || !P.cslot) return fail(ctx, PNL_ERR_STATE, "pair codes: rules and DoF map first");
    hipLaunchKernelGGL(k_tile_pair_codes<64>, dim3(std::min(n, 256*8)), dim3(512), 0, ctx->stream, P, qo, tiles, n, codes,
                       host_stat ? (int*)ctx->b_candq.p : (int*)nullptr);
    HIPCHK(ctx, hipGetLastError());
    if (host_stat) HIPCHK(ctx, hipMemcpyAsync(host_stat, ctx->b_candq.p, sizeof(int)*(size_t)n, hipMemcpyDeviceToHost, ctx->stream));
    HIPCHK(ctx, hipStreamSynchronize(ctx->stream));
    return PNL_OK;
}

int pnl_tile_order_range(pnl_context *ctx, const DevFormula &qo, int ncand, signed char *host_out) {
    const int grid = std::min(ncand, 256*8);
    if (ctx->tile == 64)
        hipLaunchKernelGGL(k_tile_order_range<64>, dim3(grid), dim3(256), 0, ctx->stream, ctx->P, qo, (const int2*)ctx->b_candtiles.p,
                           ncand, (signed char*)ctx->b_candq.p);
    else
        hipLaunchKernelGGL(k_tile_order_range<32>, dim3(grid), dim3(256), 0, ctx->stream, ctx->P, qo, (const int2*)ctx->b_candtiles.p,
                           ncand, (signed char*)ctx->b_candq.p);
    HIPCHK(ctx, hipGetLastError());
    HIPCHK(ctx, hipMemcpyAsync(host_out, ctx->b_candq.p, ncand, hipMemcpyDeviceToHost, ctx->stream));
    HIPCHK(ctx, hipStreamSynchronize(ctx->stream));
    return PNL_OK;
}

extern "C" {

static int slab_prepare(pnl_context *ctx, int &flags, int cell_begin, int cell_end) {
    if (ctx->slab_rows <= 0) return PNL_OK;
    if (flags & PNL_FLAG_SYMMETRIC_FLUSH) return fail(ctx, PNL_ERR_INVALID, "a row slab is one-sided: PNL_FLAG_SYMMETRIC_FLUSH does not apply");
    if (ctx->have_pw) return fail(ctx, PNL_ERR_UNSUPPORTED, "row slabs are not implemented for kernels with an order per quadrature point");
    const auto &rd = ctx->slab_rowdofs, &cd = ctx->slab_coldofs;
    for (int c = cell_begin; c < ctx->nc; c++)
        for (int k = 0; k < ctx->dpe; k++) {
            const int g = ctx->dofs[(size_t)c*ctx->dpe+k];
            if (g < 0) continue;
            if (c < cell_end && !std::binary_search(rd.begin(), rd.end(), g))
                return fail(ctx, PNL_ERR_INVALID, "DoF %d of cell %d is not a row of the slab", g, c);
            if (!std::binary_search(cd.begin(), cd.end(), g))
                return fail(ctx, PNL_ERR_INVALID, "DoF %d of cell %d is not a column of the slab", g, c);
        }
    flags |= PNL_FLAG_NO_MIRROR;
    return PNL_OK;
}

int pnl_assemble_dense(pnl_context *ctx, double *A, int64_t ldA, int zero_exterior, int cell_begin, int cell_end, int flags) {
    if (!ctx) return PNL_ERR_INVALID;
    int rc;
    if ((rc = pnl_assembly_ready(ctx))) return rc;
    if ((rc = pnl_tile_order_ready(ctx))) return rc;
    if (!A || ldA < (ctx->slab_rows ? ctx->slab_cols : ctx->N)) return fail(ctx, PNL_ERR_INVALID, "bad output matrix (ldA=%lld, num_dofs=%d)", (long long)ldA, ctx->N);
    if (cell_begin < 0 || cell_end > ctx->nc || cell_begin > cell_end) return fail(ctx, PNL_ERR_INVALID, "bad cell range");
    if ((rc = slab_prepare(ctx, flags, cell_begin, cell_end))) return rc;
    pnl_begin_assembly(ctx);
    ctx->run.full_tile_list = true;
    std::vector<int2> tiles;
    if (cell_end > cell_begin) pnl_make_tiles(ctx, tiles, cell_begin, cell_end);
    if ((rc = pnl_upload_tiles(ctx, tiles, cell_begin, cell_end))) return rc;
    for (long long c = cell_begin; c < cell_end; c++)
        if (ctx->real_from[c] != ctx->real_from[c+1]) ctx->run.visited_pairs += (unsigned long long)ctx->real_from[c];
    if (pnl_tune("PNL_FORCE_SYMFLUSH")) flags |= PNL_FLAG_SYMMETRIC_FLUSH;
    return dispatch(ctx, A, ldA, zero_exterior, (int)tiles.size(), cell_begin, cell_end, flags);
}

int pnl_dense_overwrites(pnl_context *ctx, int cell_begin, int cell_end, int flags) {
    if (!ctx) return PNL_ERR_INVALID;
    int rc;
    if ((rc = pnl_assembly_ready(ctx))) return rc;
    if (pnl_tune("PNL_FORCE_SYMFLUSH")) return 0;
    return slot_eligible(ctx, true, cell_begin, cell_end, flags) && slot_storage_ready(ctx) ? 1 : 0;
}

int pnl_assemble_dense_tiles(pnl_context *ctx, double *A, int64_t ldA, int zero_exterior, int ntiles, const int32_t *tiles_host,
                             int cell_begin, int cell_end, int flags) {
    if (!ctx) return PNL_ERR_INVALID;
    int rc;
    if ((rc = pnl_assembly_ready(ctx))) return rc;
    if ((rc = pnl_tile_order_ready(ctx))) return rc;
    if (!A || ldA < (ctx->slab_rows ? ctx->slab_cols : ctx->N) || ntiles < 0 || (ntiles && !tiles_host)) return fail(ctx, PNL_ERR_INVALID, "bad arguments");
    if (cell_begin < 0 || cell_end > ctx->nc || cell_begin > cell_end) return fail(ctx, PNL_ERR_INVALID, "bad cell range");
    if ((rc = slab_prepare(ctx, flags, cell_begin, cell_end))) return rc;
    std::vector<int2> tiles(ntiles);
    for (int i = 0; i < ntiles; i++) {
        tiles[i] = make_int2(tiles_host[2*i], tiles_host[2*i+1]);
        if (tiles[i].x < 0 || tiles[i].y >= ctx->nblocks || tiles[i].x > tiles[i].y) return fail(ctx, PNL_ERR_INVALID, "bad tile %d", i);
    }
    pnl_begin_assembly(ctx);
    ctx->run.tile_cell_filter = false;
    if ((rc = pnl_upload_tiles(ctx, tiles, cell_begin, cell_end))) return rc;
    return dispatch(ctx, A, ldA, zero_exterior, ntiles, cell_begin, cell_end, flags);
// ... 136 lines not shown
```

pynucleus_amd/csrc/pnl_kernels.h:

```cpp
#pragma once
#include "pnl_device.h"
#include "pnl_common.h"


template <int DIM, int DPE, int KT>
__device__ __forceinline__ void eval_distant_generic(const DevProblem &P, int off, int n, const double *av, const double *bv,
                                                     PairAcc<DIM, DPE> &R) {
    constexpr int NV = DIM+1;
    const double *__restrict__ bary = P.bary+3*(size_t)off;
    const double *__restrict__ w = P.w+off;
    const double *__restrict__ phi = P.phi+(size_t)off*DPE;
    for (int i = 0; i < n; i++) {
        double x[DIM];
#pragma unroll
        for (int d = 0; d < DIM; d++) {
            double s = 0.;
#pragma unroll
            for (int k = 0; k < NV; k++) s = __builtin_fma(bary[3*i+k], av[k*DIM+d], s);
            x[d] = s;
        }
        const double wi = w[i];
        double r = 0., u[DPE];
#pragma unroll
        for (int b = 0; b < DPE; b++) u[b] = 0.;
// ... 384 lines not shown
    static constexpr size_t fixed_bytes = sizeof(double)*n_dbl+sizeof(int)*n_int+sizeof(short)*((n_short+3)/4*4);
};

__device__ __forceinline__ int wave_bucket_add(int *counters, int q, bool fetch) {
    int pos = 0;
    unsigned long long todo = __ballot(q > 0);
    const unsigned long long lt = (1ull << (threadIdx.x & 63))-1ull;
    while (todo) {
        const int leader = __ffsll((long long)todo)-1;
        const int qL = __builtin_amdgcn_readlane(q, leader);
        const unsigned long long same = __ballot(q == qL);
        int base = 0;
        if ((int)(threadIdx.x & 63) == leader) base = atomicAdd(&counters[qL], __popcll(same));
        if (fetch) {
            base = __builtin_amdgcn_readlane(base, leader);
            if (q == qL) pos = base+__popcll(same & lt);
        }
        todo &= ~same;
    }
    return pos;
}

#ifdef PNL_ONLY_N3
__device__ __forceinline__ bool tile_eligible(int n) { return n == 3; }
#else
__device__ __forceinline__ bool tile_eligible(int n) { return n == 2 || n == 3 || n == 4 || n == 6 || n == 7; }
#endif

#ifndef PNL_PURE_WAVES
#define PNL_PURE_WAVES 4
#endif
#define PNL_CUT_SHIFT 60
#define PNL_INTERACT 0
#define PNL_REMOTE 1
#define PNL_CUT 2
#define PNL_WL_LANE_MAXPTS 40
template <int DIM>
__device__ __forceinline__ int rel_position(double h2, const double *av, const double *bv);
template <int DIM, int DPE>
__device__ __forceinline__ unsigned eval_distant_cut(const DevProblem &P, const double *__restrict__ tab, int stp, int n, const double *av,
                                                     const double *bv, PairAcc<DIM, DPE> &R);

template <int DIM, int TILE, class Between>
__device__ __forceinline__ int tile_pair_order(const DevFormula &qo, bool sel, int2 cfa, int2 cfb, const double *s_cen, const double (&cenb)[DIM],
                                               const int *s_vid, const float *s_lh, float lhb, float Llb, const double *s_h, const double *s_Ld,
                                               int i, int j, bool order2, Between &&between) {
    constexpr int NV = DIM+1;
    if (!((cfa.x & cfb.x & 1) && sel)) return 0;
    const bool any_dof = ((cfa.x | cfb.x) & 2) != 0;
    double d2 = 0.;
#pragma unroll
    for (int d = 0; d < DIM; d++) {
        const double t = s_cen[(0*DIM+d)*TILE+i]-cenb[d];
        d2 += t*t;
    }
    bool shared = false;
    const float rs = __int_as_float(cfa.y)+__int_as_float(cfb.y);
    if ((float)d2 <= rs*rs) {
#pragma unroll
        for (int k = 0; k < NV; k++) {
            const int va = s_vid[(0*NV+k)*TILE+i];
#pragma unroll
            for (int m = 0; m < NV; m++) shared = shared || (va == s_vid[(1*NV+m)*TILE+j]);
        }
    }
    if (!between(any_dof, shared) || !any_dof || shared) return 0;
    if (order2) return 2;
    int q = quad_order_try(qo, s_lh[i], lhb, s_lh[TILE+i], Llb, d2);
    if (q < 0) q = quad_order_exact(qo, s_h[i], s_h[TILE+j], s_Ld[i], s_Ld[TILE+j], sqrt(d2));
    return q;
}

#ifndef PNL_TILE_THREADS
#define PNL_TILE_THREADS 512
#endif
#ifndef PNL_TILE_WAVES
#define PNL_TILE_WAVES 4
#endif
#ifndef PNL_KT0_WIDE
#define PNL_KT0_WIDE 1
#endif
__host__ __device__ constexpr int tile_threads(int dpe, int kt, bool fh = false) { return (dpe > 3 || (kt == 0 && !PNL_KT0_WIDE) || fh) ? 256 : PNL_TILE_THREADS; }
__host__ __device__ constexpr int tile_waves(int dpe, int kt, bool fh = false) { return dpe > 3 ? 1 : (((kt == 0 && !PNL_KT0_WIDE) || fh) ? 2 : PNL_TILE_WAVES); }
template <int DIM, int DPE, int TILE, int KT, bool CLUSTER, bool FH = false, bool SETTLED = false>
__global__ void __launch_bounds__(tile_threads(DPE, KT, FH), tile_waves(DPE, KT, FH))
k_tile_distant(const DevProblem P, const int2 *__restrict__ tiles, double *__restrict__ A, long long ldA,
               double *__restrict__ Dglob, int cell_begin, int cell_end, int acc_stride, int4 *__restrict__ worklist,
               unsigned *__restrict__ wl_count, unsigned wl_cap, int ablate, int ntiles, const ClusterTiles CT,
               unsigned *__restrict__ tile_ctr, const SlotOut SO, const unsigned short *__restrict__ codes) {
    static_assert(!SETTLED || (!CLUSTER && !FH && DIM == 2 && DPE == 3 && TILE*TILE == 8*tile_threads(DPE, KT, FH)),
                  "settled tiles: dense 2D P1, eight pairs per thread");
#ifdef PNL_DEBUG_ABLATE
    const int abl = ablate;
#else
    const int abl = ablate & 256;
#endif
    using S = TileSmem<DIM, DPE, TILE, KT == 0>;
    constexpr int NV = S::NV, NC = S::NC, ND = S::ND, NT = tile_threads(DPE, KT, FH);
    constexpr int PAIRS = TILE*TILE, PER_THREAD = (PAIRS+NT-1)/NT;
    extern __shared__ double smem[];
    double *s_dbl = smem;
    int *s_int = (int*)(s_dbl+S::n_dbl);
    short *s_short = (short*)(s_int+S::n_int);
    double *s_acc = (double*)(s_short+(S::n_short+3)/4*4);
    double *s_v = s_dbl+S::o_v, *s_cen = s_dbl+S::o_cen, *s_vol = s_dbl+S::o_vol, *s_h = s_dbl+S::o_h, *s_D = s_dbl+S::o_D;
    int *s_vid = s_int+S::o_vid, *s_cnt = s_int+S::o_cnt, *s_cur = s_int+S::o_cur, *s_misc = s_int+S::o_misc;
    int2 *s_cf = (int2*)(s_int+S::o_cf);
    short *s_slot = s_short+S::o_slot;
    unsigned short *s_list = (unsigned short*)(s_short+S::o_list);
    float *s_lh = (float*)(s_int+S::o_lh);
    int *s_ttn = s_int+S::o_ttn, *s_tto = s_int+S::o_tto;
    double *s_tt = s_dbl+S::o_tt, *s_Ld = s_dbl+S::o_Ld;

    const int tid = threadIdx.x;
    int *s_chunk = s_int+S::o_chunk;
    int *s_dslot = s_int+S::o_dslot, *s_cell = s_int+S::o_cell;
    unsigned short *s_code = (unsigned short*)s_vid;
    unsigned long long st_cnt[(PNL_MAXQ+NT)/NT] = {0}, st_ev[(PNL_MAXQ+NT)/NT] = {0};
    for (int t = tid; t < PNL_MAXQ+2; t += NT) { s_ttn[t] = P.tt_n[t]; s_tto[t] = P.tt_off[t]; }
    for (int t = tid; t < P.tt_npts*(4+DPE); t += NT) s_tt[t] = P.tt_tab[t];
    double *s_pow = s_dbl+S::o_pow;
    if (KT == 0) pnl_pow_tab_fill(s_pow, P.k.ptab, tid, NT);
    const double *__restrict__ lpow = (KT == 0 && P.k.ptab) ? s_pow : nullptr;
    constexpr bool fh = !CLUSTER && FH;
    int qA0 = 0, qB0 = 0;
    for (int q = 17; q >= 2; q--) {
        const int n = P.tt_n[q];
        qA0 = (n == ((DIM == 2) ? 3 : 2)) ? q : qA0;
        qB0 = (n == ((DIM == 2) ? 6 : 3)) ? q : qB0;
    }
    __shared__ int s_tile_next;
    auto stage = [&](int tile_idx) {
    const int ta = CLUSTER ? CT.chunkA[tile_idx] : tiles[tile_idx].x, tb = CLUSTER ? CT.chunkB[tile_idx] : tiles[tile_idx].y;
    const int nA = CLUSTER ? CT.chunk_ndof[ta] : P.blk_ndof[ta], nB = CLUSTER ? CT.chunk_ndof[tb] : P.blk_ndof[tb];
    for (int t = tid; t < 2*TILE; t += NT) {
        const int side = t/TILE, l = t%TILE;
        const int craw = CLUSTER ? CT.chunk_cells[(size_t)(side ? tb : ta)*TILE+l] : (side ? tb : ta)*TILE+l;
        const bool real = craw >= 0;
        const int c = real ? craw : 0;
        if (CLUSTER) {
            s_cell[side*TILE+l] = craw;
            s_dslot[side*TILE+l] = (side ? CT.dslotB : CT.dslotA)[(size_t)tile_idx*TILE+l];
        }
#pragma unroll
        for (int k = 0; k < NC; k++) s_v[(side*NC+k)*TILE+l] = P.cellv[(size_t)k*P.ncp+c];
        s_vol[side*TILE+l] = P.cvol[c];
        int vid0 = -1;
        if (!SETTLED) {
#pragma unroll
        for (int d = 0; d < DIM; d++) s_cen[(side*DIM+d)*TILE+l] = P.ccen[(size_t)d*P.ncp+c];
        s_h[side*TILE+l] = P.ch[c];
        const double lh = P.clog[c], Ld = P.clog[(size_t)P.ncp+c];
        s_Ld[side*TILE+l] = Ld;
        s_lh[(side*2+0)*TILE+l] = (float)lh;
        s_lh[(side*2+1)*TILE+l] = (float)Ld;
#pragma unroll
        for (int k = 0; k < NV; k++) {
            const int v = real ? P.cvid[(size_t)k*P.ncp+c] : -1-k;
            s_vid[(side*NV+k)*TILE+l] = v;
            vid0 = k == 0 ? v : vid0;
        }
        }
        bool has_dof = false;
#pragma unroll
        for (int k = 0; k < DPE; k++) {
            const short sl = CLUSTER ? (real ? CT.chunk_slot[((size_t)(side ? tb : ta)*DPE+k)*TILE+l] : (short)-1) : P.cslot[(size_t)k*P.ncp+c];
            s_slot[(side*DPE+k)*TILE+l] = sl >= 0 ? sl : (short)(side ? nB : nA);
            has_dof = has_dof || sl >= 0;
        }
        if (!SETTLED) s_cf[side*TILE+l] = make_int2((vid0 >= 0 ? 1 : 0) | (has_dof ? 2 : 0), __float_as_int((float)P.clog[2*(size_t)P.ncp+c]));
    }
    if (SETTLED) s_code[tid] = codes[(size_t)tile_idx*NT+tid];
    };
    const bool pipe = !(abl & 256);
    if (pipe) {
        for (int t = tid; t < ((CLUSTER ? CT.chunk_stride : SO.nU)+1)*acc_stride; t += NT) s_acc[t] = 0.;
        for (int t = tid; t < 2*TILE*ND; t += NT) s_D[t] = 0.;
        for (int t = tid; t < 2*(PNL_MAXQ+2)+4; t += NT) s_cnt[t] = 0;
        if ((int)blockIdx.x < ntiles) stage(blockIdx.x);
    }
#pragma unroll 1
    for (int tile_idx = blockIdx.x; tile_idx < ntiles; tile_idx = s_tile_next) {
    const int ta = CLUSTER ? CT.chunkA[tile_idx] : tiles[tile_idx].x, tb = CLUSTER ? CT.chunkB[tile_idx] : tiles[tile_idx].y;
    const int nA = CLUSTER ? CT.chunk_ndof[ta] : P.blk_ndof[ta], nB = CLUSTER ? CT.chunk_ndof[tb] : P.blk_ndof[tb];
    const bool sym = CLUSTER ? (CT.flags[tile_idx] & 1) != 0 : true;
    if (!pipe) {
        stage(tile_idx);
        for (int t = tid; t < (nA+1)*acc_stride; t += NT) s_acc[t] = 0.;
        for (int t = tid; t < 2*TILE*ND; t += NT) s_D[t] = 0.;
        for (int t = tid; t < 2*(PNL_MAXQ+2)+4; t += NT) s_cnt[t] = 0;
    }
    lds_barrier();

    constexpr int NA = (DIM == 2) ? 3 : 2, NB = (DIM == 2) ? 6 : 3;
    int *s_l32 = (int*)(s_list+PAIRS+((((size_t)(s_list+PAIRS)) & 2) ? 1 : 0));
    int overflow = 0;
    const int lane = tid & 63;
    const unsigned long long lt = (1ull << lane)-1ull;
    int cnt234[3] = {0, 0, 0};
    static_assert(NT%TILE == 0 && PAIRS%NT == 0 && PER_THREAD <= 16, "tile workgroup: whole rows of the tile per sweep");
    constexpr int NG = (PER_THREAD+3)/4;
    const int j = tid%TILE;
    const unsigned code = SETTLED ? s_code[tid] : 0u;
    double cenb[DIM] = {};
    int2 cfb = make_int2(0, 0);
    float lhb = 0.f, Llb = 0.f;
    int labb = 0;
    if constexpr (!SETTLED) {
#pragma unroll
        for (int d = 0; d < DIM; d++) cenb[d] = s_cen[(1*DIM+d)*TILE+j];
        cfb = s_cf[TILE+j];
        lhb = s_lh[2*TILE+j]; Llb = s_lh[3*TILE+j];
        labb = (!CLUSTER && P.cur_class >= 0) ? P.clabel[tb*TILE+j] : 0;
    }
    int nw0 = 0, nw1 = 0, nw2 = 0, nw3 = 0;
    unsigned long long recs[NG];
#pragma unroll
    for (int g = 0; g < NG; g++) {
    recs[g] = 0ull;
#pragma unroll 2
    for (int it4 = 0; it4 < (PER_THREAD-4*g < 4 ? PER_THREAD-4*g : 4); it4++) {
        const int r = tile_sweep_row(tid, 4*g+it4, TILE, NT);
        const int i = tile_diag_cell(r, j, TILE);
        int q = 0, fkey = 0;
        if constexpr (SETTLED) {
            const int c = (int)(code >> (2*(4*g+it4))) & 3;
            q = c ? c+1 : 0;
        } else {
        const int ca = ta*TILE+i;
        bool sel = !(abl & 8) &&
                   (CLUSTER ? (!sym || ta < tb || i < j) : ((ta < tb || i < j || (fh && i == j)) && (ca >= cell_begin) && (ca < cell_end)));
        if (!CLUSTER && P.cur_class >= 0 && sel) {
            const int la = P.clabel[ca];
            sel = P.cls_of[P.orient ? labb*P.nlab+la : la*P.nlab+labb] == P.cur_class;
        }
        int rel = PNL_INTERACT;
        q = tile_pair_order<DIM, TILE>(P.qo, sel, s_cf[i], cfb, s_cen, cenb, s_vid, s_lh, lhb, Llb, s_h, s_Ld, i, j, (abl & 16) != 0,
                                       [&](bool any_dof, bool shared) {
            if (!CLUSTER && fh && any_dof) {
                if (shared) {
                    int common = 0;
#pragma unroll
                    for (int k = 0; k < NV; k++)
#pragma unroll
                        for (int m = 0; m < NV; m++) common += (s_vid[(0*NV+k)*TILE+i] == s_vid[(1*NV+m)*TILE+j]);
                    fkey = 121+common-1;
                } else {
                    double av[NC], bv[NC];
#pragma unroll
                    for (int k = 0; k < NC; k++) { av[k] = s_v[(0*NC+k)*TILE+i]; bv[k] = s_v[(1*NC+k)*TILE+j]; }
                    rel = rel_position<DIM>(P.k.horizon2, av, bv);
                }
            }
            return rel != PNL_REMOTE;
        });
        if (q) {
            if (q > P.qmax || q > PNL_MAXQ) { overflow++; q = 0; }
            else if (rel == PNL_CUT) {
                if (q > PNL_CUT_SHIFT || P.off[q+1]-P.off[q] > PNL_WL_LANE_MAXPTS) { overflow++; q = 0; }
                else fkey = q+PNL_CUT_SHIFT;
            }
        }
        }
        const int nq = SETTLED ? 1 : (q ? s_ttn[q] : 0);
        const int key = fkey ? fkey : q;
        const int cls = !key ? 0 : (fkey ? 4 : (q == qA0 ? 1 : (q == qB0 ? 2 : (nq > 0 ? 3 : 4))));
        const int qs = (fh && cls == 4) ? 0 : q;
        if (!(abl & 32)) {
        cnt234[0] += __popcll(__ballot(qs == 2)); cnt234[1] += __popcll(__ballot(qs == 3)); cnt234[2] += __popcll(__ballot(qs == 4));
        if (!SETTLED) wave_bucket_add(s_cnt, qs > 4 ? qs : 0, false);
        }
        nw0 += __popcll(__ballot(cls == 1)); nw1 += __popcll(__ballot(cls == 2));
        if (!SETTLED) nw2 += __popcll(__ballot(cls == 4));
        nw3 += __popcll(__ballot(cls == 3));
        const unsigned rec = (unsigned)cls | ((unsigned)key << 3) | ((fh && fkey > PNL_CUT_SHIFT+1 && fkey < 121 && nq > 0) ? (1u << 11) : 0u);
        recs[g] |= (unsigned long long)rec << (16*it4);
    }
    }
    {
        int mybase = 0;
        const int mine = lane == 0 ? nw0 : (lane == 1 ? nw1 : (lane == 2 ? nw2 : nw3));
        if (lane < 4 && mine) mybase = atomicAdd(&s_misc[lane], mine);
        int bA = __builtin_amdgcn_readlane(mybase, 0), bB = __builtin_amdgcn_readlane(mybase, 1);
        int bF = __builtin_amdgcn_readlane(mybase, 2), bC = __builtin_amdgcn_readlane(mybase, 3);
        if (!(abl & 128))
#pragma unroll
        for (int g = 0; g < NG; g++)
#pragma unroll
            for (int it4 = 0; it4 < (PER_THREAD-4*g < 4 ? PER_THREAD-4*g : 4); it4++) {
                const unsigned rec = (unsigned)(recs[g] >> (16*it4)) & 0xffffu;
                const int cls = rec & 7, key = (rec >> 3) & 255;
                const int p = tile_sweep_row(tid, 4*g+it4, TILE, NT)*TILE+j;
                if (nw0) {
                    const unsigned long long m = __ballot(cls == 1);
                    if (cls == 1) s_list[bA+__popcll(m & lt)] = (unsigned short)(p | ((qA0-2) << 12));
                    bA += __popcll(m);
                }
                if (nw1) {
                    const unsigned long long m = __ballot(cls == 2);
                    if (cls == 2) s_l32[bB+__popcll(m & lt)] = p | ((qB0-2) << 12);
                    bB += __popcll(m);
                }
                if (nw3) {
                    const unsigned long long m = __ballot(cls == 3);
                    if (cls == 3) s_list[PAIRS-1-(bC+__popcll(m & lt))] = (unsigned short)(p | ((key-2) << 12));
                    bC += __popcll(m);
                }
                if (!SETTLED && nw2) {
                    const unsigned long long m = __ballot(cls == 4);
                    if (cls == 4) s_l32[PAIRS-1-(bF+__popcll(m & lt))] = p | (key << 12) | ((rec & (1u << 11)) ? (1 << 20) : 0);
                    bF += __popcll(m);
                }
            }
    }
    if (!SETTLED && overflow) atomicAdd(&P.counters[5], (unsigned long long)overflow);
    if (lane == 0) {
#pragma unroll
        for (int k = 0; k < 3; k++) if (cnt234[k]) atomicAdd(&s_cnt[2+k], cnt234[k]);
    }
    lds_barrier();
    int next_tile = 0;
    if (tid == 0) next_tile = (int)(gridDim.x+atomicAdd(tile_ctr, 1u));
    const int nC = __builtin_amdgcn_readfirstlane(s_misc[3]), nBl = __builtin_amdgcn_readfirstlane(s_misc[1]);
    if (nC && tid == 64 && !(abl & 2)) {
        int run = 0, nch = 0;
        for (int q = min(17, P.qmax); q >= 2; q--) {
            const int nq = s_ttn[q], c = s_cnt[q];
            if (!c || nq == 0 || q == qA0 || q == qB0) continue;
            s_cur[q] = run;
            for (int st = 0; st < c && nch < PNL_GEN_MAXCHUNKS; st += 64) s_chunk[nch++] = (q << 20) | ((run+st) << 7) | (min(64, c-st)-1);
            run += c;
        }
        s_cnt[0] = nch;
    }
    bool published = false;
    {
        const int nF = SETTLED ? 0 : s_misc[2];
        if (fh) {
#pragma unroll 1
            for (int t0 = (tid >> 6)*64; t0 < nF; t0 += NT) {
                const int t = t0+lane;
                const int ent = t < nF ? s_l32[PAIRS-1-t] : (1 << 20);
                const bool exp = !(ent & (1 << 20));
                const unsigned long long m = __ballot(exp);
                if (m) {
                    unsigned base = 0;
                    const int leader = __ffsll((long long)m)-1;
                    if (lane == leader) base = atomicAdd(wl_count, (unsigned)__popcll(m));
                    base = (unsigned)__builtin_amdgcn_readlane((int)base, leader);
                    const unsigned pos = base+(unsigned)__popcll(m & lt);
                    if (exp && pos < wl_cap) {
                        const int p = ent & 4095, key = (ent >> 12) & 255;
                        const int j = p%TILE, i = (p/TILE+PNL_DIAG_MULT*j)%TILE;
                        const int qq = key >= 121 ? 0 : (key > PNL_CUT_SHIFT+1 ? key-PNL_CUT_SHIFT : key);
                        const int o2 = qq ? P.off[qq] : 0, n2 = qq ? P.off[qq+1]-o2 : 0;
                        worklist[pos] = make_int4((int)pos, 0, o2, n2 | (key << 16));
                        CT.wl_ds[pos] = make_int2(ta*TILE+i, tb*TILE+j);
                    }
                }
            }
        } else if (nF) {
            if (tid == 0) s_cur[0] = (int)atomicAdd(wl_count, (unsigned)nF);
            lds_barrier();
            published = true;
            const unsigned base = (unsigned)s_cur[0];
            for (int t = tid; t < nF; t += NT) {
                const int ent = s_l32[PAIRS-1-t];
                const int p = ent & 4095, q = ent >> 12;
                const int j = p%TILE, i = (p/TILE+PNL_DIAG_MULT*j)%TILE;
                const int off = P.off[q];
                if (base+t < wl_cap) {
                    if (CLUSTER) {
                        worklist[base+t] = make_int4(s_cell[i], s_cell[TILE+j], (int)(base+t), (P.off[q+1]-off) | (q << 16));
                        const int dA = s_dslot[i], dB = s_dslot[TILE+j];
                        CT.wl_ds[base+t] = make_int2(dA, (dB >= 0 && (sym || dA < 0)) ? dB : -1);
                        CT.wl_pair[base+t] = CT.pair[tile_idx];
                    } else
                        worklist[base+t] = make_int4(ta*TILE+i, tb*TILE+j, off, (P.off[q+1]-off) | (q << 16));
                }
            }
        }
    }
#pragma unroll
    for (int r = 0; r < (PNL_MAXQ+NT)/NT; r++) {
        const int q = 2+tid+r*NT;
        if (q <= P.qmax) {
            const int cq = s_cnt[q];
            if (cq) {
                const int ne = s_ttn[q];
                const unsigned long long n = (unsigned long long)(ne ? ne : P.off[q+1]-P.off[q]);
                st_cnt[r] += (unsigned long long)cq;
                st_ev[r] += n*n*cq;
            }
        }
    }

    const int wave = tid >> 6;
    auto accumulate = [&](const PairAcc<DIM, DPE> &R, int i, int j) {
        const double vv = 2.*s_vol[i]*s_vol[TILE+j]*kern_scale<KT>(P.k);
        if (abl & 1) {
            double keep = 0.;
#pragma unroll
            for (int a = 0; a < DPE; a++)
#pragma unroll
                for (int b = 0; b < DPE; b++) keep += R.G[a][b];
#pragma unroll
            for (int e2 = 0; e2 < ND; e2++) keep += R.S1[e2]+R.S2[e2];
            if (keep == 1.2345e300) s_D[0] = keep*vv;
            return;
        }
        int e = 0;
#pragma unroll
        for (int a = 0; a < DPE; a++) {
            const int sa = s_slot[(0*DPE+a)*TILE+i];
#pragma unroll
            for (int b = 0; b < DPE; b++) {
                const int sb = s_slot[(1*DPE+b)*TILE+j];
                lds_add_f64(&s_acc[sa*acc_stride+sb], -vv*R.G[a][b]);
            }
#pragma unroll
            for (int b = a; b < DPE; b++) {
                if (CLUSTER) {
                    const int dA = s_dslot[i], dB = s_dslot[TILE+j];
                    if (dA >= 0) lds_add_f64(&s_D[(0*TILE+i)*ND+e], vv*R.S1[e]);
                    if (dB >= 0 && (sym || dA < 0)) lds_add_f64(&s_D[(1*TILE+j)*ND+e], vv*R.S2[e]);
                } else if (!(abl & 64)) {
                    lds_add_f64(&s_D[(0*TILE+i)*ND+e], vv*R.S1[e]);
                    lds_add_f64(&s_D[(1*TILE+j)*ND+e], vv*R.S2[e]);
                } else if (R.S1[e]+R.S2[e] == 1.2345e300) s_D[0] = 1.;
                e++;
            }
        }
    };
    if (nC && !(abl & 2)) {
        if (!published) lds_barrier();
        for (int t = tid; t < nC; t += NT) {
            const int ent = s_list[PAIRS-1-t];
            const int q = (ent >> 12)+2;
            s_l32[nBl+atomicAdd(&s_cur[q], 1)] = ent & 4095;
        }
        lds_barrier();
    }
    if (!(abl & 2))
    kern_dispatch<KT, fh>(P.k, lpow, [&](auto ktag) {
    constexpr int KTE = decltype(ktag)::value;
    const int nAl = __builtin_amdgcn_readfirstlane(s_misc[0]);
    const int nchC = nC ? __builtin_amdgcn_readfirstlane(s_cnt[0]) : 0, nchB = (nBl+63) >> 6, nchA = (nAl+63) >> 6;
    const int total = nchC+nchB+nchA;
#pragma unroll 1
    for (;;) {
        int c = 0;
        if (lane == 0) c = atomicAdd(&s_cnt[1], 1);
        c = __builtin_amdgcn_readfirstlane(c);
        if (c >= total) break;
        int q, p;
        bool act;
        if (c < nchC) {
            const int desc = __builtin_amdgcn_readfirstlane(s_chunk[c]);
            const int start = (desc >> 7) & 8191, cnt = (desc & 127)+1;
            q = desc >> 20;
            act = lane < cnt;
            p = s_l32[nBl+start+(act ? lane : 0)];
        } else if (c < nchC+nchB) {
            const int idx = (c-nchC)*64+lane;
            q = qB0;
            act = idx < nBl;
            p = s_l32[act ? idx : 0] & 4095;
        } else {
            const int idx = (c-nchC-nchB)*64+lane;
            q = qA0;
            act = idx < nAl;
            p = (int)s_list[act ? idx : 0] & 4095;
        }
        const int j = p%TILE, i = (p/TILE+PNL_DIAG_MULT*j)%TILE;
        double av[NC], bv[NC];
#pragma unroll
        for (int k = 0; k < NC; k++) { av[k] = s_v[(0*NC+k)*TILE+i]; bv[k] = s_v[(1*NC+k)*TILE+j]; }
        PairAcc<DIM, DPE> R;
        R.clear();
        const int nq = __builtin_amdgcn_readfirstlane(s_ttn[q]), to = __builtin_amdgcn_readfirstlane(s_tto[q]);
        if constexpr (DIM == 2 && DPE == 3 && !FH) {
            if (q <= 4 && ((P.mix_struct >> q) & 1) && (nq == 3 || nq == 6)) {
                const pnl_const_f64_ptr rule = (pnl_const_f64_ptr)(unsigned long long)(P.uni+P.uni_off[q]);
                if (nq == 6) eval_struct6<KTE>(P.k, rule, s_tt+to*(4+DPE), av, bv, R, lpow);
                else eval_struct3<KTE>(P.k, rule, av, bv, R, lpow);
                if (act) accumulate(R, i, j);
                continue;
            }
        }
        if (nq == NB) eval_distant_fixed<DIM, DPE, KTE, NB>(P, s_tt+to*(4+DPE), P.tt_wphi+to*DPE, av, bv, R, lpow);
        else if (nq == NA) eval_distant_fixed<DIM, DPE, KTE, NA>(P, s_tt+to*(4+DPE), P.tt_wphi+to*DPE, av, bv, R, lpow);
        else eval_distant_lds<DIM, DPE, KTE>(P, s_tt+to*(4+DPE), 4+DPE, nq, av, bv, R, lpow);
        if (act) accumulate(R, i, j);
    }
    });
    if (fh) {
        const int nF = __builtin_amdgcn_readfirstlane(s_misc[2]);
        unsigned long long ncutp = 0, ncute = 0;
#pragma unroll 1
        for (int t0 = wave*64; t0 < nF; t0 += NT) {
            const int t = t0+lane;
            const int ent = t < nF ? s_l32[PAIRS-1-t] : 0;
            const bool cutl = (ent & (1 << 20)) != 0;
            if (!__ballot(cutl)) continue;
            const int p = ent & 4095, q = cutl ? ((ent >> 12) & 255)-PNL_CUT_SHIFT : 2;
            const int j = p%TILE, i = (p/TILE+PNL_DIAG_MULT*j)%TILE;
            double av[NC], bv[NC];
#pragma unroll
            for (int k = 0; k < NC; k++) { av[k] = s_v[(0*NC+k)*TILE+i]; bv[k] = s_v[(1*NC+k)*TILE+j]; }
            PairAcc<DIM, DPE> R;
            R.clear();
            if (cutl) {
                ncute += eval_distant_cut<DIM, DPE>(P, s_tt+s_tto[q]*(4+DPE), 4+DPE, s_ttn[q], av, bv, R);
                ncutp++;
                accumulate(R, i, j);
            }
            unsigned long long todo = __ballot(cutl);
            while (todo) {
                const int leader = __ffsll((long long)todo)-1;
                const int qL = __builtin_amdgcn_readlane(q, leader);
                const unsigned long long same = __ballot(cutl && q == qL);
                if (lane == leader) atomicAdd(&P.counters[8+qL], (unsigned long long)__popcll(same));
                todo &= ~same;
            }
        }
        if (ncutp) { atomicAdd(&P.counters[1], ncutp); atomicAdd(&P.counters[2], ncute); }
    }
    if (tid == 0) s_tile_next = next_tile;
    lds_barrier();

    if (pipe) {
        const int nx = s_tile_next;
        auto flush_D = [&]() {
            for (int t = tid; t < 2*TILE*ND; t += NT) {
                const double v = s_D[t];
                s_D[t] = 0.;
                if (v != 0. && !(abl & 4)) {
                    const int side = t/(TILE*ND), rem = t-side*TILE*ND;
                    if (CLUSTER) {
// ... 2094 lines not shown
        int mn = 1 << 30, mx = 0, bad = 0;
        for (int p = tid; p < TILE*TILE; p += 256) {
            const int i = p/TILE, j = p-i*TILE;
            const int a0 = s_vid[0][i], a1 = s_vid[1][i], a2 = s_vid[2][i];
            const int b0 = s_vid[3][j], b1 = s_vid[4][j], b2 = s_vid[5][j];
            if (a0 < 0 || b0 < 0) continue;
            bad |= (a0 == b0) | (a0 == b1) | (a0 == b2) | (a1 == b0) | (a1 == b1) | (a1 == b2) | (a2 == b0) | (a2 == b1) | (a2 == b2);
            const double dx = s_cen[0][i]-s_cen[2][j], dy = s_cen[1][i]-s_cen[3][j];
            const int q = quad_order_fast(qo, s_h[0][i], s_h[1][j], s_lh[0][i], s_lh[2][j], s_lh[1][i], s_lh[3][j], s_Ld[0][i], s_Ld[1][j],
                                          dx*dx+dy*dy);
            mn = min(mn, q); mx = max(mx, q);
        }
        atomicMin(&s_red[0], mn); atomicMax(&s_red[1], mx); atomicOr(&s_red[2], bad);
        __syncthreads();
        if (tid == 0)
            out[t] = (signed char)((!s_red[2] && s_red[0] == s_red[1] && s_red[0] >= 2 && s_red[0] < 120) ? s_red[0]
                                   : ((!s_red[2] && s_red[0] >= 2 && s_red[0] < s_red[1] && s_red[1] <= 4) ? -1 : 0));
        __syncthreads();
    }
}

template <int TILE>
__global__ void __launch_bounds__(512)
k_tile_pair_codes(const DevProblem P, const DevFormula qo, const int2 *__restrict__ tiles, int ntiles, unsigned short *__restrict__ codes,
                  int *__restrict__ stat) {
    constexpr int DIM = 2, NV = 3, DPE = 3, NT = 512, SWEEPS = TILE*TILE/NT;
    static_assert(SWEEPS == 8, "2 bits per pair, one 16-bit word per thread");
    __shared__ double s_cen[2*DIM*TILE], s_h[2*TILE], s_Ld[2*TILE];
    __shared__ float s_lh[4*TILE];
    __shared__ int s_vid[2*NV*TILE];
    __shared__ int2 s_cf[2*TILE];
    __shared__ int s_red[2];
    const int tid = threadIdx.x;
#pragma unroll 1
    for (int t = blockIdx.x; t < ntiles; t += gridDim.x) {
        const int2 tl = tiles[t];
        for (int u = tid; u < 2*TILE; u += NT) {
            const int side = u/TILE, l = u%TILE, c = (side ? tl.y : tl.x)*TILE+l;
#pragma unroll
            for (int d = 0; d < DIM; d++) s_cen[(side*DIM+d)*TILE+l] = P.ccen[(size_t)d*P.ncp+c];
            s_h[side*TILE+l] = P.ch[c];
            const double lh = P.clog[c], Ld = P.clog[(size_t)P.ncp+c];
            s_Ld[side*TILE+l] = Ld;
            s_lh[(side*2+0)*TILE+l] = (float)lh;
            s_lh[(side*2+1)*TILE+l] = (float)Ld;
#pragma unroll
            for (int k = 0; k < NV; k++) s_vid[(side*NV+k)*TILE+l] = P.cvid[(size_t)k*P.ncp+c];
            bool has_dof = false;
#pragma unroll
            for (int k = 0; k < DPE; k++) has_dof = has_dof || P.cslot[(size_t)k*P.ncp+c] >= 0;
            s_cf[side*TILE+l] = make_int2((P.cvid[c] >= 0 ? 1 : 0) | (has_dof ? 2 : 0), __float_as_int((float)P.clog[2*(size_t)P.ncp+c]));
        }
        if (tid < 2) s_red[tid] = 0;
        __syncthreads();
        const int j = tid%TILE;
        double cenb[DIM];
#pragma unroll
        for (int d = 0; d < DIM; d++) cenb[d] = s_cen[(1*DIM+d)*TILE+j];
        const int2 cfb = s_cf[TILE+j];
        const float lhb = s_lh[2*TILE+j], Llb = s_lh[3*TILE+j];
        unsigned code = 0u;
        int bad = 0, n6 = 0;
#pragma unroll 2
        for (int k = 0; k < SWEEPS; k++) {
            const int i = tile_diag_cell(tile_sweep_row(tid, k, TILE, NT), j, TILE);
            const int q = tile_pair_order<DIM, TILE>(qo, true, s_cf[i], cfb, s_cen, cenb, s_vid, s_lh, lhb, Llb, s_h, s_Ld, i, j, false,
                                                     [&](bool any_dof, bool shared) { bad |= (any_dof && shared) ? 1 : 0; return true; });
            if (q) {
                const int nq = (q <= 4 && q <= P.qmax) ? P.tt_n[q] : 0;
                if (nq <= 0) bad = 1;
                else { code |= (unsigned)(q-1) << (2*k); n6 += nq == 6 ? 1 : 0; }
            }
        }
        if (codes) codes[(size_t)t*NT+tid] = (unsigned short)code;
        if (stat) {
            if (bad) atomicOr(&s_red[0], 1);
            if (n6) atomicAdd(&s_red[1], n6);
            __syncthreads();
            if (tid == 0) stat[t] = s_red[0] ? -1 : s_red[1];
        }
        __syncthreads();
    }
}
```

pynucleus_amd/csrc/pnl_setup.hip:

```cpp
#include <hip/hip_runtime.h>
#include <algorithm>
#include <cmath>
#include <cstdio>
#include <cstring>
#include <deque>
#include <map>
#include <mutex>
#include <string>
#include <thread>
#include <vector>
#include "pnl_hip.h"
#include "pnl_context.h"

template <class F>
static void host_threads(F body) {
    const int nthr = (int)std::max(1u, std::min(8u, std::thread::hardware_concurrency()));
    std::vector<std::thread> pool;
    for (int th = 0; th < nthr; th++) pool.emplace_back([&body, th, nthr]() { body(th, nthr); });
    for (auto &t : pool) t.join();
}

struct TileOrderJob {
    std::vector<int> cells, lperm;
    int nc = 0, T = 0, nblocks = 0, ncp = 0, dim = 0, dpe = 0;
// ... 514 lines not shown
    P.k = to_dev(ctx->C().kern[0], ctx->dim);
    P.bk = to_dev(ctx->C().kern[1], ctx->dim);
    P.bkn = to_dev_bkn(ctx->C().kern[1], ctx->dim);
    P.qo = to_dev(ctx->C().form[0]);
    P.bqo = to_dev(ctx->C().form[1]);
    P.qmax = ctx->qmax;
    P.off = (const int*)ctx->b_off.p; P.bary = (const double*)ctx->b_bary.p; P.w = (const double*)ctx->b_w.p;
    P.phi = (const double*)ctx->b_phi.p; P.foff = (const int*)ctx->b_foff.p; P.fbary = (const double*)ctx->b_fbary.p;
    P.fw = (const double*)ctx->b_fw.p;
    P.tt_n = (const int*)ctx->b_ttn.p; P.tt_off = (const int*)ctx->b_ttoff.p; P.tt_tab = (const double*)ctx->b_tttab.p;
    P.tt_wphi = (const double*)ctx->b_ttwphi.p;
    P.tt_wphif = (const double*)ctx->b_ttwphif.p;
    for (int s = 0; s < 3; s++) {
        P.sNodes[s] = (const double*)ctx->C().b_sn[s].p; P.sW[s] = (const double*)ctx->C().b_sw[s].p; P.sPsi[s] = (const double*)ctx->C().b_sp[s].p;
    }
    for (int s = 0; s < 2; s++) {
        P.bNodes[s] = (const double*)ctx->C().b_bn[s].p; P.bW[s] = (const double*)ctx->C().b_bw[s].p; P.bPhi[s] = (const double*)ctx->C().b_bp[s].p;
    }
    for (int s = 0; s < 3; s++) { P.sM[s] = ctx->C().sM[s]; P.sRows[s] = ctx->C().sRows[s]; }
    for (int s = 0; s < 2; s++) P.bM[s] = ctx->C().bM[s];
    P.sFac = ctx->C().sFac; P.bFac = ctx->C().bFac;
    P.cur_class = ctx->nlab > 0 ? ctx->cur : -1;
    P.orient = ctx->nonsym ? ctx->orient : 0;
    P.idfac = ctx->nonsym ? 2. : 1.;
    if (ctx->nonsym) P.k.scale *= 0.5;
    P.k.ptab = pnl_pow_table(ctx, P.k);
}

static int check_ready(pnl_context *ctx) {
    for (auto *c : ctx->cls)
        if (!c->have_kernel[0] || !c->have_form[0] || !ctx->have_rules)
            return fail(ctx, PNL_ERR_STATE, "kernel, order formula and distant rules must be set (for every class) before assembling");
    return PNL_OK;
}

int pnl_assembly_ready(pnl_context *ctx) {
    int rc;
    if ((rc = check_ready(ctx))) return rc;
    return finalize(ctx);
}
int pnl_assembly_prepare(pnl_context *ctx) {
    int rc;
    if ((rc = pnl_assembly_ready(ctx))) return rc;
    pnl_refresh_tables(ctx);
    return PNL_OK;
}

int pnl_tile_uniform_order(const pnl_context *ctx, const pnl_order_formula &F, int ta, int tb, int qlimit) {
    if (ta == tb) return 0;
    const auto &A = ctx->blocks[ta], &B = ctx->blocks[tb];
    if (!A.full || !B.full || !(F.e >= 0.) || !(F.den0 > 0.)) return 0;
    const double dx = A.cx-B.cx, dy = A.cy-B.cy, dc = std::sqrt(dx*dx+dy*dy);
    const double dmin = dc-A.rad-B.rad, dmax = dc+A.rad+B.rad;
    if (!(dmin > A.hmax+B.hmax)) return 0;
    typedef pnl_context::BlockAgg Agg;
    auto upper = [&](const Agg &S, const Agg &O, double q) {
        const double l_self = std::log(dmin/S.hmax), n_other = std::log(dmin/O.hmax);
        const double aL = std::max(F.a*O.Lmin, F.a*O.Lmax);
        const double bL = std::max(F.b*std::max(S.Lmin, O.Lmin), F.b*std::max(S.Lmax, O.Lmax));
        const double num = F.c0+aL+bL-F.e*n_other, den = l_self+F.den0;
        return num <= q*den*(1.-1e-9)-1e-9;
    };
    auto lower = [&](const Agg &S, const Agg &O, double q) {
        const double l_self = std::log(dmax/S.hmin), n_other = std::log(dmax/O.hmin);
        const double aL = std::min(F.a*O.Lmin, F.a*O.Lmax);
        const double bL = std::min(F.b*std::max(S.Lmin, O.Lmin), F.b*std::max(S.Lmax, O.Lmax));
        const double num = F.c0+aL+bL-F.e*n_other, den = l_self+F.den0;
        return den > 0. && num >= q*den*(1.+1e-9)+1e-9;
    };
    for (int q = 2; q <= qlimit; q++)
        if (upper(A, B, q) && upper(B, A, q)) {
            if (q == 2) return 2;
            return (lower(A, B, q-1) || lower(B, A, q-1)) ? q : 0;
        }
    return 0;
}

namespace {
std::mutex g_opt_mutex;
std::map<std::string, const std::string*> g_options;
std::deque<std::string> g_option_values;
const char *const k_product_options[] = {"PNL_WL_FRAC", "PNL_FH_NOTILES", "PNL_NO_POWTAB", "PNL_VERBOSE", "PNL_PLAN_TIMING", "PNL_PLAN_THREADS", "PNL_BND_OLD",
                                         "PNL_NO_OVERLAP", "PNL_NO_FORK",
                                         "PNL_TILE_WGS", "PNL_UNI_GENERIC", "PNL_MIXED_GENERIC", "PNL_MIXED_UNSETTLED",
                                         "PNL_FOLD_STAGES", "PNL_UNI_SPARE", "PNL_BND_MODE"};
}

const char *pnl_tune(const char *name) {
    {
        std::lock_guard<std::mutex> lk(g_opt_mutex);
        auto it = g_options.find(name);
        if (it != g_options.end()) return it->second->c_str();
    }
#ifdef PNL_TUNING
    return getenv(name);
#else
    return nullptr;
#endif
}

extern "C" {

const char *pnl_version(void) {
#ifdef PNL_TUNING
    return "pnl_hip 0.1 (gfx950, tuning build)";
#else
    return "pnl_hip 0.1 (gfx950)";
#endif
}

int pnl_set_option(const char *name, const char *value) {
    if (!name) return PNL_ERR_INVALID;
#ifndef PNL_TUNING
    bool known = false;
    for (const char *k : k_product_options) known = known || std::strcmp(k, name) == 0;
    if (!known) return PNL_ERR_UNSUPPORTED;
#endif
    std::lock_guard<std::mutex> lk(g_opt_mutex);
    if (value) {
        const std::string *v = nullptr;
        for (const std::string &have : g_option_values) if (have == value) { v = &have; break; }
        if (!v) { g_option_values.emplace_back(value); v = &g_option_values.back(); }
        g_options[name] = v;
    } else g_options.erase(name);
    return PNL_OK;
}

int pnl_create(int device_id, pnl_context **out) {
    if (!out) return PNL_ERR_INVALID;
    *out = nullptr;
    int ndev = 0;
    hipError_t e0;
    auto hiperr = [](const char *what, hipError_t e) { fprintf(stderr, "[pnl] pnl_create: %s failed: %s\n", what, hipGetErrorString(e)); return PNL_ERR_HIP; };
    if ((e0 = hipGetDeviceCount(&ndev)) != hipSuccess || ndev <= 0) return hiperr("hipGetDeviceCount", e0);
    if (device_id < 0 || device_id >= ndev) return PNL_ERR_INVALID;
    if ((e0 = hipSetDevice(device_id)) != hipSuccess) return hiperr("hipSetDevice", e0);
    pnl_context *ctx = new pnl_context();
    ctx->device = device_id;
    if ((e0 = hipStreamCreate(&ctx->own_stream)) != hipSuccess) { delete ctx; return hiperr("hipStreamCreate", e0); }
    ctx->stream = ctx->own_stream;
    for (auto &st : ctx->aux)
        if ((e0 = hipStreamCreateWithFlags(&st, hipStreamNonBlocking)) != hipSuccess) { delete ctx; return hiperr("hipStreamCreateWithFlags", e0); }
    if (hipEventCreateWithFlags(&ctx->ev_fork, hipEventDisableTiming) != hipSuccess) { delete ctx; return PNL_ERR_HIP; }
    if (hipEventCreateWithFlags(&ctx->ev_fold, hipEventDisableTiming) != hipSuccess) { delete ctx; return PNL_ERR_HIP; }
    if (hipEventCreateWithFlags(&ctx->ev_bnd, hipEventDisableTiming) != hipSuccess) { delete ctx; return PNL_ERR_HIP; }
    for (auto &e : ctx->ev_join)
        if (hipEventCreateWithFlags(&e, hipEventDisableTiming) != hipSuccess) { delete ctx; return PNL_ERR_HIP; }
    for (auto &e : ctx->ev)
        if (hipEventCreate(&e) != hipSuccess) { delete ctx; return PNL_ERR_HIP; }
    for (auto &e : ctx->ev_stage)
        if (hipEventCreateWithFlags(&e, hipEventDisableTiming) != hipSuccess) { delete ctx; return PNL_ERR_HIP; }
    std::memset(&ctx->P, 0, sizeof(ctx->P));
#ifdef PNL_DEBUG_ABLATE
    if (const char *e = pnl_tune("PNL_ABLATE")) ctx->ablate = atoi(e);
#endif
    if (const char *e = pnl_tune("PNL_WL_LANE")) ctx->wl_lane = atoi(e) != 0;
    if (const char *e = pnl_tune("PNL_PURE")) ctx->use_pure = atoi(e) != 0;
    ctx->cls.push_back(new pnl_context::ClassData());
    *out = ctx;
    return PNL_OK;
}

void pnl_destroy(pnl_context *ctx) {
    if (!ctx) return;
    (void)hipSetDevice(ctx->device);
    (void)hipStreamSynchronize(ctx->stream);
    for (auto &e : ctx->ev)
// ... 271 lines not shown
            npts += npad; nb++;
            (void)st;
        }
        if ((rc = upload(ctx, ctx->b_ttn, tn.data(), tn.size()))) return rc;
        if ((rc = upload(ctx, ctx->b_ttoff, to.data(), to.size()))) return rc;
        if ((rc = upload(ctx, ctx->b_tttab, tab.data(), tab.size()))) return rc;
        if ((rc = upload(ctx, ctx->b_ttwphi, wphi.data(), wphi.size()))) return rc;
        ctx->P.tt_npts = npts;
        std::vector<double> wphif;
        for (int q = 2; q <= qmax && q < 18; q++)
            for (int i = 0; i < tn[q]; i++) {
                const size_t p = (size_t)off[q]+(i < tn[q] ? i : 0);
                const double wp = i < tn[q] ? w[p] : 0.;
                wphif.push_back(wp);
                for (int a = 0; a < dpe; a++) wphif.push_back(wp*phi[p*dpe+a]);
            }
        if ((rc = upload(ctx, ctx->b_ttwphif, wphif.data(), wphif.size()))) return rc;
        if ((rc = upload_uniform_rule_blocks(ctx, qmax, off, bary, w, phi))) return rc;
        ctx->tiles_cached.clear(); ctx->tiles_forms.clear();
    }
    ctx->qmax = qmax;
    ctx->have_rules = true;
    return PNL_OK;
}

int pnl_upload_singular_rule(pnl_context *ctx, int which, int panel, int M, int rows, const double *nodes, const double *w,
                             const double *psi, double facv) {
    if (!ctx) return PNL_ERR_INVALID;
    if (!ctx->have_dofs) return fail(ctx, PNL_ERR_STATE, "upload the DoF map first");
    const int slot = -panel-1;
    const int nslots = which == PNL_INTERIOR ? ctx->dim+1 : ctx->dim;
    if (which < 0 || which > 1 || slot < 0 || slot >= nslots || M <= 0 || rows <= 0 || !nodes || !w || !psi)
        return fail(ctx, PNL_ERR_INVALID, "bad singular-rule arguments");
    const int dim = ctx->dim, dpe = ctx->dpe, dpv = ctx->dpv, dped = ctx->dped, nV = dim+1;
    int rc;
    if (which == PNL_INTERIOR) {
        const int common = slot+1;
        const int expect = common == nV ? dpe : (common == 1 ? 2*dpe-dpv : 2*dpe-2*dpv-dped);
        if (rows != expect) return fail(ctx, PNL_ERR_INVALID, "singular rule has %d rows, expected %d", rows, expect);
        if ((rc = upload(ctx, ctx->C().b_sn[slot], nodes, (size_t)2*nV*M))) return rc;
        if ((rc = upload(ctx, ctx->C().b_sw[slot], w, (size_t)M))) return rc;
        if ((rc = upload(ctx, ctx->C().b_sp[slot], psi, (size_t)rows*M))) return rc;
        ctx->C().sM[slot] = M; ctx->C().sRows[slot] = rows; ctx->C().sFac = facv;
    } else {
        if (rows != dpe) return fail(ctx, PNL_ERR_INVALID, "boundary singular rule has %d rows, expected %d", rows, dpe);
        if ((rc = upload(ctx, ctx->C().b_bn[slot], nodes, (size_t)(nV+dim)*M))) return rc;
        if ((rc = upload(ctx, ctx->C().b_bw[slot], w, (size_t)M))) return rc;
        if ((rc = upload(ctx, ctx->C().b_bp[slot], psi, (size_t)rows*M))) return rc;
        ctx->C().bM[slot] = M; ctx->C().bFac = facv;
    }
    ctx->C().have_sing[which][slot] = true;
    return PNL_OK;
}

int pnl_upload_boundary(pnl_context *ctx, int nb, const int32_t *bcells) {
    if (!ctx) return PNL_ERR_INVALID;
    if (!ctx->have_mesh) return fail(ctx, PNL_ERR_STATE, "upload the mesh first");
    if (nb < 0 || (nb > 0 && !bcells)) return fail(ctx, PNL_ERR_INVALID, "bad boundary arguments");
    ctx->nb = nb;
    ctx->bcells.assign(bcells, bcells+(size_t)nb*ctx->dim);
    ctx->have_boundary = true;
    ctx->dirty = true;
    return PNL_OK;
}

int pnl_tile_cells(pnl_context *ctx) {
    if (!ctx) return PNL_ERR_INVALID;
    int rc = finalize(ctx);
    return rc ? rc : ctx->tile;
}

}

struct TilePlan {
    int T, ncls, L, qlimit, cell_begin, cell_end;
    bool filter, p1, p2, allow, q2ok;
    std::vector<pnl_order_formula> forms;
    std::vector<std::vector<int>> blk_labels;
    std::vector<std::vector<int2>> mixed, uni[3];
};

static int fold_stages_wanted();
static int settled_wanted() { return pnl_tune("PNL_MIXED_UNSETTLED") ? 0 : 1; }

static bool tiles_resident(const pnl_context *ctx, const std::vector<int2> &tiles, const TilePlan &R) {
    const std::vector<pnl_order_formula> &forms = R.forms;
    return tiles.size() == ctx->tiles_cached.size() && ctx->b_tiles.p && ctx->tiles_cb == R.cell_begin && ctx->tiles_ce == R.cell_end &&
        forms.size() == ctx->tiles_forms.size() && std::memcmp(forms.data(), ctx->tiles_forms.data(), sizeof(pnl_order_formula)*R.ncls) == 0 &&
        ctx->tiles_filter == ctx->run.tile_cell_filter && ctx->stg_want == fold_stages_wanted() && ctx->settled_want == settled_wanted() &&
        (tiles.empty() || std::memcmp(tiles.data(), ctx->tiles_cached.data(), tiles.size()*sizeof(int2)) == 0);
}

static int tile_orders(pnl_context *ctx, const TilePlan &R, const std::vector<int2> &tiles, int k, std::vector<signed char> &qof,
                       std::vector<size_t> &open_234) {
    open_234.clear();
    const int T = R.T, L = R.L, qlimit = R.qlimit, cell_begin = R.cell_begin, cell_end = R.cell_end;
    const bool filter = R.filter, allow = R.allow, q2ok = R.q2ok;
    const std::vector<std::vector<int>> &blk_labels = R.blk_labels;
    host_threads([&](int th, int nthr) {
        const size_t i0 = tiles.size()*th/nthr, i1 = tiles.size()*(th+1)/nthr;
        for (size_t i = i0; i < i1; i++) {
            const int2 &t = tiles[i];
            bool single = true;
            if (L > 0) {
                bool has = false;
                for (int la : blk_labels[t.x]) for (int lb : blk_labels[t.y])
                    has = has || ctx->cls_of[(size_t)la*L+lb] == k || ctx->cls_of[(size_t)lb*L+la] == k;
                if (!has) { qof[i] = -1; continue; }
                single = blk_labels[t.x].size() == 1 && blk_labels[t.y].size() == 1;
            }
            int q = (allow && single) ? pnl_tile_uniform_order(ctx, R.forms[k], t.x, t.y, qlimit) : 0;
            if (q == 2 && !q2ok) q = 0;
            if (q && filter && !(t.x*T >= cell_begin && (t.x+1)*T <= cell_end)) q = 0;
            qof[i] = (signed char)q;
        }
    });
    if (!(allow && ctx->dim == 2 && (T == 64 || T == 32) && !pnl_tune("PNL_NO_EXACT_TILES"))) return PNL_OK;
    std::vector<int2> cand;
    std::vector<size_t> cand_idx;
    for (size_t i = 0; i < tiles.size(); i++) {
        const int2 &t = tiles[i];
        if (qof[i] != 0 || t.x == t.y || !ctx->blocks[t.x].full || !ctx->blocks[t.y].full) continue;
        if (L > 0 && !(blk_labels[t.x].size() == 1 && blk_labels[t.y].size() == 1)) continue;
        if (filter && !(t.x*T >= cell_begin && (t.x+1)*T <= cell_end)) continue;
        cand.push_back(t); cand_idx.push_back(i);
    }
    if (cand.empty()) return PNL_OK;
    int rc;
    if ((rc = upload(ctx, ctx->b_candtiles, cand.data(), cand.size()))) return rc;
    if ((rc = ensure(ctx, ctx->b_candq, cand.size()))) return rc;
    std::vector<signed char> cq(cand.size());
    if ((rc = pnl_tile_order_range(ctx, to_dev(R.forms[k]), (int)cand.size(), cq.data()))) return rc;
    size_t moved = 0;
    for (size_t c = 0; c < cand.size(); c++) {
        const int q = cq[c];
        if (q == -1) open_234.push_back(cand_idx[c]);
        if (q < 2 || q > qlimit || (q == 2 && !q2ok)) continue;
        qof[cand_idx[c]] = (signed char)q; moved++;
    }
    if (pnl_tune("PNL_VERBOSE")) fprintf(stderr, "[pnl] exact order range: %zu of %zu open tiles are uniform\n", moved, cand.size());
    return PNL_OK;
}

static int settle_tiles(pnl_context *ctx, const TilePlan &R, const std::vector<int2> &tiles, const std::vector<size_t> &open_234,
                        std::vector<int2> &settled, std::vector<char> &is_settled) {
    settled.clear();
    is_settled.assign(tiles.size(), 0);
    if (!settled_wanted() || open_234.empty() || !(R.p1 && ctx->dim == 2 && ctx->dpe == 3 && R.T == 64) || R.ncls != 1 || R.L > 0 ||
        ctx->nonsym || !ctx->b_ttn.p || !ctx->b_cslot.p || R.cell_begin > 0 || R.cell_end < ctx->nc || open_234.size() > (size_t)0x7fffffff/512) return PNL_OK;
    std::vector<int2> cand(open_234.size());
    for (size_t c = 0; c < cand.size(); c++) cand[c] = tiles[open_234[c]];
    int rc;
    if ((rc = upload(ctx, ctx->b_candtiles, cand.data(), cand.size()))) return rc;
    std::vector<int> stat(cand.size());
    if ((rc = pnl_tile_pair_codes(ctx, to_dev(R.forms[0]), (const int2*)ctx->b_candtiles.p, (int)cand.size(), nullptr, stat.data()))) return rc;
    std::vector<size_t> keep;
    for (size_t c = 0; c < cand.size(); c++) if (stat[c] >= 0) keep.push_back(c);
    if (keep.empty()) return PNL_OK;
    if (ensure(ctx, ctx->b_codes, keep.size()*512*sizeof(unsigned short)) != PNL_OK) {
        (void)hipGetLastError();
        ctx->err.clear();
        return PNL_OK;
    }
    std::stable_sort(keep.begin(), keep.end(), [&](size_t x, size_t y) { return stat[x] > stat[y]; });
    for (size_t c : keep) { settled.push_back(cand[c]); is_settled[open_234[c]] = 1; }
    return PNL_OK;
}

#ifndef PNL_FOLD_STAGES_DEFAULT
#define PNL_FOLD_STAGES_DEFAULT 0
#endif
static int fold_stages_wanted() {
// ... 146 lines not shown
        for (int o = 0; o < norient; o++)
            for (const int2 &t : mixed[k]) {
                if (one_visit) { const unsigned m = tile_mask[(size_t)t.x*ctx->nblocks+t.y]; if (m & (m-1u)) continue; }
                all.push_back(t); allcls.push_back(2*k+o);
            }
    }
    ctx->sl_n[0] = (int)all.size();
    for (int u = 0; u < 3; u++) {
        ctx->sl_off[u+1] = (int)all.size();
        for (int k = 0; k < ncls; k++) {
            ctx->cls_n_uni[u][k] = (int)uni[u][k].size();
            for (const int2 &t : uni[u][k]) { all.push_back(t); allcls.push_back(2*k); }
        }
        ctx->sl_n[u+1] = (int)all.size()-ctx->sl_off[u+1];
    }
    for (int k = 0; k < ncls; k++) ctx->cls_n_pure[k] = ctx->cls_n_uni[0][k];
    std::vector<long long> keys(all.size());
    for (size_t i = 0; i < all.size(); i++) keys[i] = (long long)all[i].x*ctx->nblocks+all[i].y;
    std::vector<long long> sorted(keys);
    std::sort(sorted.begin(), sorted.end());
    std::vector<int2> multi;
    for (size_t i = 0; i+1 < sorted.size(); i++)
        if (sorted[i] == sorted[i+1] && (i == 0 || sorted[i-1] != sorted[i]))
            multi.push_back(make_int2((int)(sorted[i]/ctx->nblocks), (int)(sorted[i]%ctx->nblocks)));
    std::vector<long long> mk(multi.size());
    for (size_t i = 0; i < multi.size(); i++) mk[i] = (long long)multi[i].x*ctx->nblocks+multi[i].y;
    for (size_t i = 0; i < all.size(); i++)
        if (std::binary_search(mk.begin(), mk.end(), keys[i])) allcls[i] |= (1 << 30);
    ctx->n_multitiles = (int)multi.size();
    int rc;
    if ((rc = upload(ctx, ctx->b_multitiles, multi.data(), multi.size()))) return rc;
    return upload(ctx, ctx->b_tilecls, allcls.data(), allcls.size());
}

int pnl_upload_tiles(pnl_context *ctx, std::vector<int2> &tiles, int cell_begin, int cell_end) {
    TilePlan R;
    const int ncls = R.ncls = (int)ctx->cls.size();
    R.cell_begin = cell_begin; R.cell_end = cell_end;
    R.forms = std::vector<pnl_order_formula>(ncls);
    for (int k = 0; k < ncls; k++) R.forms[k] = ctx->cls[k]->form[0];
    if (tiles_resident(ctx, tiles, R)) return PNL_OK;
    const int T = R.T = ctx->tile;
    R.filter = ctx->run.tile_cell_filter;
    R.p1 = T == 64 && (ctx->dpe == 3 || ctx->dpe == 2); R.p2 = ctx->dim == 2 && ctx->dpe == 6;
    R.allow = ctx->use_pure && (R.p1 || R.p2) && ctx->qmax >= 2 && !ctx->nonsym;
    int qlimit = 2;
    if (ctx->dim == 2) for (int q = 3; q <= 4 && ctx->uni_off[q] >= 0 && ctx->uni_np[q] == 6 && q <= ctx->qmax; q++) qlimit = q;
    R.q2ok = R.p1 ? true : (ctx->uni_off[2] >= 0 && ctx->uni_np[2] == 3);
    if (pnl_tune("PNL_UNI_QMAX")) qlimit = std::min(qlimit, std::max(2, atoi(pnl_tune("PNL_UNI_QMAX"))));
    R.qlimit = qlimit;
    const int L = R.L = ctx->nlab;
    std::vector<std::vector<int>> &blk_labels = R.blk_labels;
    if (L > 0) {
        blk_labels.resize(ctx->nblocks);
        for (int b = 0; b < ctx->nblocks; b++) {
            auto &v = blk_labels[b];
            for (int c = b*T; c < std::min((b+1)*T, ctx->nc); c++) v.push_back(ctx->cell_labels[c]);
            std::sort(v.begin(), v.end());
            v.erase(std::unique(v.begin(), v.end()), v.end());
        }
    }
    ctx->cls_tile_off.assign(ncls, 0); ctx->cls_n_mixed.assign(ncls, 0); ctx->cls_n_pure.assign(ncls, 0);
    for (int u = 0; u < 3; u++) ctx->cls_n_uni[u].assign(ncls, 0);
    std::vector<std::vector<int2>> &mixed = R.mixed, *uni = R.uni;
    mixed.resize(ncls);
    for (int u = 0; u < 3; u++) uni[u].resize(ncls);
    std::vector<signed char> qof(tiles.size());
    std::vector<size_t> open_234;
    std::vector<int2> settled;
    std::vector<char> is_settled;
    int rc;
    ctx->n_settled = 0;
    for (int k = 0; k < ncls; k++) {
        if ((rc = tile_orders(ctx, R, tiles, k, qof, open_234))) return rc;
        if ((rc = settle_tiles(ctx, R, tiles, open_234, settled, is_settled))) return rc;
        for (size_t i = 0; i < tiles.size(); i++) {
            const int q = qof[i];
            if (q < 0 || is_settled[i]) continue;
            (q ? uni[q-2][k] : mixed[k]).push_back(tiles[i]);
        }
        mixed[k].insert(mixed[k].end(), settled.begin(), settled.end());
    }
    if (settled.empty()) ctx->b_codes.release();
    ctx->settled_tiles.clear();
    std::vector<int2> all;
    ctx->single_launch = R.p2;
    const int stages_wanted = fold_stages_wanted();
    if ((rc = stage_plan(ctx, R, tiles, stages_wanted))) return rc;
    if (!R.p2) tile_lists_per_class(ctx, R, all);
    else if ((rc = tile_lists_single_launch(ctx, R, tiles, all))) return rc;
    if (pnl_tune("PNL_VERBOSE")) {
        size_t nm = 0, nu[3] = {0, 0, 0};
        for (int k = 0; k < ncls; k++) { nm += mixed[k].size(); for (int u = 0; u < 3; u++) nu[u] += uni[u][k].size(); }
        fprintf(stderr, "[pnl] tiles: %zu mixed (%zu of them settled), uniform order 2/3/4: %zu / %zu / %zu (qlimit %d)\n", nm, settled.size(),
                nu[0], nu[1], nu[2], qlimit);
    }
    if ((rc = upload(ctx, ctx->b_tiles, all.data(), all.size()))) return rc;
    if (!settled.empty()) {
        const int first = ctx->cls_tile_off[0]+ctx->cls_n_mixed[0]-(int)settled.size();
        if ((rc = pnl_tile_pair_codes(ctx, to_dev(R.forms[0]), (const int2*)ctx->b_tiles.p+first, (int)settled.size(),
                                      (unsigned short*)ctx->b_codes.p, nullptr))) return rc;
        ctx->n_settled = (int)settled.size();
        ctx->settled_tiles = settled;
        ctx->code_builds++;
    }
    ctx->settled_want = settled_wanted();
    ctx->tiles_cached = tiles; ctx->tiles_cb = cell_begin; ctx->tiles_ce = cell_end; ctx->tiles_forms = R.forms;
    ctx->tiles_filter = ctx->run.tile_cell_filter;
    ctx->stg_want = stages_wanted;
    return PNL_OK;
}

int pnl_make_tiles(pnl_context *ctx, std::vector<int2> &tiles, int cell_begin, int cell_end) {
    const int T = ctx->tile, nbk = ctx->nblocks;
    const int a0 = cell_begin/T, a1 = (cell_end+T-1)/T;
    for (int d = 0; d < nbk; d++)
        for (int a = a0; a < a1 && a+d < nbk; a++) tiles.push_back(make_int2(a, a+d));
    return PNL_OK;
}

extern "C" {

int pnl_block_row_costs(pnl_context *ctx, double *out, int n) {
    if (!ctx || !out) return PNL_ERR_INVALID;
    int rc;
    if ((rc = check_ready(ctx))) return rc;
    if ((rc = finalize(ctx))) return rc;
    if (n != ctx->nblocks) return fail(ctx, PNL_ERR_INVALID, "pnl_block_row_costs: %d blocks expected", ctx->nblocks);
    const int T = ctx->tile, nb = ctx->nblocks;
    const bool p1 = T == 64 && (ctx->dpe == 3 || ctx->dpe == 2), p2 = ctx->dim == 2 && ctx->dpe == 6;
    const bool allow = ctx->use_pure && (p1 || p2) && ctx->qmax >= 2 && !ctx->nonsym && ctx->cls.size() == 1;
    int qlimit = 2;
    if (ctx->dim == 2) for (int q = 3; q <= 4 && ctx->uni_off[q] >= 0 && ctx->uni_np[q] == 6 && q <= ctx->qmax; q++) qlimit = q;
    const pnl_order_formula F = ctx->cls[0]->form[0];
    const double w_uni3 = p2 ? 1.75 : 2.7, w_mixed = p2 ? 2.5 : 4.0, w_cells = p2 ? 30. : 57.;
    host_threads([&](int t, int nthreads) {
        for (int a = t; a < nb; a += nthreads) {
            double c = w_cells;
            for (int b = a; b < nb; b++) {
                const int q = allow ? pnl_tile_uniform_order(ctx, F, a, b, qlimit) : 0;
                c += q == 2 ? 1. : (q ? w_uni3 : w_mixed);
            }
            out[a] = c;
        }
    });
    return PNL_OK;
}

int pnl_set_order_function(pnl_context *ctx, const pnl_order_function *f, const double *cell_smax, const double *facet_smax,
                           double c0, double bc0, double sing_fac, double bsing_fac) {
    if (!ctx || !f || !cell_smax) return fail(ctx, PNL_ERR_INVALID, "bad order-function arguments");
    if (!ctx->have_mesh) return fail(ctx, PNL_ERR_STATE, "upload the mesh first");
    if (f->type < 1 || f->type > 5) return fail(ctx, PNL_ERR_UNSUPPORTED, "order function type %d is not implemented", f->type);
    if (ctx->have_dofs && !(ctx->dpe == ctx->dim+1 || (ctx->dim == 2 && ctx->dpe == 6) || (ctx->dim == 1 && ctx->dpe == 3)))
        return fail(ctx, PNL_ERR_UNSUPPORTED, "pointwise variable orders: P1 and P2 elements");
    if (!pw_set_function(ctx->pw, *f)) return fail(ctx, PNL_ERR_INVALID, "bad Chebyshev series of the scaling");
    ctx->pw.c0 = c0; ctx->pw.bc0 = bc0; ctx->pw.sfac = sing_fac; ctx->pw.bfac = bsing_fac;
    ctx->pw_cell_smax.assign(cell_smax, cell_smax+ctx->nc);
    ctx->pw_facet_smax.clear();
    if (facet_smax && ctx->have_boundary) ctx->pw_facet_smax.assign(facet_smax, facet_smax+ctx->nb);
    for (int w = 0; w < 2; w++) for (int s = 0; s < 3; s++) ctx->have_pw_rules[w][s] = false;
    ctx->pw_vertex_s.clear();
    ctx->have_pw = true;
    return PNL_OK;
}

int pnl_set_order_vertex_values(pnl_context *ctx, int nv, const double *values) {
    if (!ctx || !values) return PNL_ERR_INVALID;
    if (!ctx->have_pw || ctx->pw.type != 5) return fail(ctx, PNL_ERR_STATE, "set an order function of type 5 first");
    if (nv != ctx->nv) return fail(ctx, PNL_ERR_INVALID, "pnl_set_order_vertex_values: %d vertices expected", ctx->nv);
    ctx->pw_vertex_s.assign(values, values+nv);
    return PNL_OK;
}

int pnl_upload_pointwise_rules(pnl_context *ctx, int which, int panel, int nkeys, int M, int rows, const double *nodes,
                               const double *w, const double *phi0, const double *phi1) {
    if (!ctx) return PNL_ERR_INVALID;
    if (!ctx->have_pw || !ctx->have_dofs) return fail(ctx, PNL_ERR_STATE, "set the order function and the DoF map first");
    const int slot = -panel-1, dim = ctx->dim, nV = dim+1, dpe = ctx->dpe;
    const int nslots = which == PNL_INTERIOR ? nV : dim;
    if (which < 0 || which > 1 || slot < 0 || slot >= nslots || nkeys <= 0 || M <= 0 || !nodes || !w || !phi0 ||
        (which == PNL_INTERIOR && !phi1))
        return fail(ctx, PNL_ERR_INVALID, "bad pointwise-rule arguments");
    int rc;
    if (which == PNL_INTERIOR) {
        const int common = slot+1;
        const int expect = common == nV ? dpe : (common == 1 ? 2*dpe-ctx->dpv : 2*dpe-2*ctx->dpv-ctx->dped);
        if (rows != expect) return fail(ctx, PNL_ERR_INVALID, "pointwise rule has %d rows, expected %d", rows, expect);
        if ((rc = upload(ctx, ctx->b_pw_rule[0][slot][0], nodes, (size_t)nkeys*2*nV*M))) return rc;
        if ((rc = upload(ctx, ctx->b_pw_rule[0][slot][1], w, (size_t)nkeys*M))) return rc;
        if ((rc = upload(ctx, ctx->b_pw_rule[0][slot][2], phi0, (size_t)nkeys*rows*M))) return rc;
        if ((rc = upload(ctx, ctx->b_pw_rule[0][slot][3], phi1, (size_t)nkeys*rows*M))) return rc;
        ctx->pw.M[slot] = M; ctx->pw.rows[slot] = rows;
        ctx->pw.nodes[slot] = (const double*)ctx->b_pw_rule[0][slot][0].p; ctx->pw.w[slot] = (const double*)ctx->b_pw_rule[0][slot][1].p;
        ctx->pw.phi0[slot] = (const double*)ctx->b_pw_rule[0][slot][2].p; ctx->pw.phi1[slot] = (const double*)ctx->b_pw_rule[0][slot][3].p;
    } else {
        if (rows != dpe) return fail(ctx, PNL_ERR_INVALID, "pointwise boundary rule has %d rows, expected %d", rows, dpe);
        if ((rc = upload(ctx, ctx->b_pw_rule[1][slot][0], nodes, (size_t)nkeys*(nV+dim)*M))) return rc;
        if ((rc = upload(ctx, ctx->b_pw_rule[1][slot][1], w, (size_t)nkeys*M))) return rc;
        if ((rc = upload(ctx, ctx->b_pw_rule[1][slot][2], phi0, (size_t)nkeys*rows*M))) return rc;
        ctx->pw.bM[slot] = M;
        ctx->pw.bnodes[slot] = (const double*)ctx->b_pw_rule[1][slot][0].p; ctx->pw.bw[slot] = (const double*)ctx->b_pw_rule[1][slot][1].p;
        ctx->pw.bphi[slot] = (const double*)ctx->b_pw_rule[1][slot][2].p;
    }
    ctx->pw_nkeys[which] = nkeys;
    ctx->have_pw_rules[which][slot] = true;
    return PNL_OK;
}

}

int pnl_pw_prepare(pnl_context *ctx, int need_boundary) {
    int rc;
    if (!ctx->have_pw || !ctx->have_rules) return fail(ctx, PNL_ERR_STATE, "order function and distant rules must be set before assembling");
    if ((rc = finalize(ctx))) return rc;
    if (ctx->pw.type == 5) {
        if ((int)ctx->pw_vertex_s.size() != ctx->nv) return fail(ctx, PNL_ERR_STATE, "order function of type 5 without vertex values");
        const int nV = ctx->dim+1;
        std::vector<double> sv((size_t)nV*ctx->ncp, 0.);
        for (int c = 0; c < ctx->nc; c++)
            for (int k = 0; k < nV; k++) sv[(size_t)k*ctx->ncp+c] = ctx->pw_vertex_s[ctx->cells[(size_t)c*nV+k]];
        if ((rc = upload(ctx, ctx->b_pw_cellsv, sv.data(), sv.size()))) return rc;
        ctx->pw.cell_sv = (const double*)ctx->b_pw_cellsv.p; ctx->pw.sv_stride = ctx->ncp;
    }
    if (!(ctx->dpe == ctx->dim+1 || (ctx->dim == 2 && ctx->dpe == 6) || (ctx->dim == 1 && ctx->dpe == 3)))
        return fail(ctx, PNL_ERR_UNSUPPORTED, "pointwise variable orders: P1 and P2 elements");
    for (int s = 0; s <= ctx->dim; s++)
        if (!ctx->have_pw_rules[0][s]) return fail(ctx, PNL_ERR_STATE, "pointwise rule for %d common vertices not uploaded", s+1);
    if (need_boundary) {
        if (!ctx->have_boundary || (int)ctx->pw_facet_smax.size() != ctx->nb)
            return fail(ctx, PNL_ERR_STATE, "the boundary term needs boundary facets and their orders");
        for (int s = 0; s < ctx->dim; s++)
            if (!ctx->have_pw_rules[1][s]) return fail(ctx, PNL_ERR_STATE, "pointwise boundary rule for %d common vertices not uploaded", s+1);
    }
    std::vector<double> sm(ctx->ncp, 0.);
    std::copy(ctx->pw_cell_smax.begin(), ctx->pw_cell_smax.end(), sm.begin());
    if ((rc = upload(ctx, ctx->b_pw_csm, sm.data(), sm.size()))) return rc;
    if ((rc = upload(ctx, ctx->b_pw_fsm, ctx->pw_facet_smax.data(), ctx->pw_facet_smax.size()))) return rc;
    ctx->pw.cell_smax = (const double*)ctx->b_pw_csm.p; ctx->pw.facet_smax = (const double*)ctx->b_pw_fsm.p;
    DevProblem &P = ctx->P;
    P.qmax = ctx->qmax;
    P.off = (const int*)ctx->b_off.p; P.bary = (const double*)ctx->b_bary.p; P.w = (const double*)ctx->b_w.p;
    P.phi = (const double*)ctx->b_phi.p; P.foff = (const int*)ctx->b_foff.p; P.fbary = (const double*)ctx->b_fbary.p;
    P.fw = (const double*)ctx->b_fw.p;
    P.cur_class = -1;
    return PNL_OK;
}

extern "C" {

int pnl_get_counters(pnl_context *ctx, int64_t *out, int n) {
    if (!ctx || !out || n <= 0) return PNL_ERR_INVALID;
    if (!ctx->b_counters.p) return fail(ctx, PNL_ERR_STATE, "nothing assembled yet");
    unsigned long long tmp[PNL_NCOUNTERS];
    HIPCHK(ctx, hipStreamSynchronize(ctx->stream));
    HIPCHK(ctx, hipMemcpy(tmp, ctx->b_counters.p, sizeof(tmp), hipMemcpyDeviceToHost));
    tmp[0] = ctx->run.visited_is_assembled ? tmp[1] : ctx->run.visited_pairs;
    for (int i = 0; i < n && i < PNL_NCOUNTERS; i++) out[i] = (int64_t)tmp[i];
    if (n > PNL_C_SETTLED_TILES) out[PNL_C_SETTLED_TILES] = ctx->run.settled_run;
    if (n > PNL_C_CODE_BUILDS) out[PNL_C_CODE_BUILDS] = ctx->code_builds;
    if (n > PNL_C_WORKLIST_LENGTH) {
        unsigned wl[PNL_WL_SLOTS];
        const int ns = std::min(ctx->run.wl_slots, PNL_WL_SLOTS);
        out[PNL_C_WORKLIST_LENGTH] = 0;
        if (ctx->b_wlcount.p && ctx->wl_cap_each > 0) {
            HIPCHK(ctx, hipMemcpy(wl, ctx->b_wlcount.p, sizeof(unsigned)*std::max(1, ns), hipMemcpyDeviceToHost));
            for (int i = 0; i < ns; i++) out[PNL_C_WORKLIST_LENGTH] += wl[i];
        }
    }
    return check_overflow(ctx);
}

int pnl_get_phase_ms(pnl_context *ctx, float *out, int n) {
    if (!ctx || !out || n <= 0) return PNL_ERR_INVALID;
    if (!ctx->run.ev_valid) return fail(ctx, PNL_ERR_STATE, "nothing assembled yet");
    HIPCHK(ctx, hipEventSynchronize(ctx->ev[EV_END]));
    float t[7] = {0, 0, 0, 0, 0, 0, 0}, tmp;
    if (ctx->run.tiles_launched) {
        HIPCHK(ctx, hipEventElapsedTime(&t[0], ctx->ev[EV_START], ctx->ev[EV_TILES_DONE]));
        HIPCHK(ctx, hipEventElapsedTime(&t[1], ctx->ev[EV_TILES_DONE], ctx->ev[EV_WORKLIST_DONE]));
        if (ctx->run.pure_launched && ctx->cls.size() == 1) {
            HIPCHK(ctx, hipEventElapsedTime(&t[6], ctx->ev[EV_START], ctx->ev[EV_TILES_UNIFORM_DONE]));
            t[0] -= t[6];
        }
    }
    HIPCHK(ctx, hipEventElapsedTime(&tmp, ctx->ev[EV_WORKLIST_DONE], ctx->ev[EV_MIRROR_DONE]));
    HIPCHK(ctx, hipEventElapsedTime(&t[2], ctx->ev[EV_MIRROR_DONE], ctx->ev[EV_SINGULAR_DONE]));
    HIPCHK(ctx, hipEventElapsedTime(&t[3], ctx->ev[EV_SINGULAR_DONE], ctx->ev[EV_BOUNDARY_DONE]));
    HIPCHK(ctx, hipEventElapsedTime(&t[4], ctx->ev[EV_BOUNDARY_DONE], ctx->ev[EV_END]));
    t[4] += tmp;
    HIPCHK(ctx, hipEventElapsedTime(&t[5], ctx->ev[EV_START], ctx->ev[EV_END]));
    for (int i = 0; i < n && i < 7; i++) out[i] = t[i];
    return PNL_OK;
}

int pnl_get_fold_stages(pnl_context *ctx, int64_t *out, int n) {
    if (!ctx || n < 0 || (n && !out)) return PNL_ERR_INVALID;
    if (!ctx->b_tiles.p || ctx->cls_n_mixed.empty()) return fail(ctx, PNL_ERR_STATE, "no tile plan yet");
    const int K = ctx->stg_K;
    for (int s = 0; s <= K && s < n; s++) {
        int64_t *o = out+5*(size_t)s;
        if (K == 0) {
            const long long nr = (ctx->N+31)/32;
            o[0] = nr*(nr+1)/2;
            for (int u = 0; u < 3; u++) { o[1+u] = 0; for (int k : ctx->cls_n_uni[u]) o[1+u] += k; }
        } else {
            o[0] = ctx->stg_img_off[s+1]-ctx->stg_img_off[s];
            for (int u = 0; u < 3; u++) o[1+u] = ctx->stg_uni_off[u][s+1]-ctx->stg_uni_off[u][s];
        }
        o[4] = 0;
        if (s == 0) for (int k : ctx->cls_n_mixed) o[4] += k;
    }
    return K+1;
}

int pnl_get_settled_tiles(pnl_context *ctx, int32_t *tiles, int64_t ntiles) {
    if (!ctx || ntiles < 0 || (ntiles && !tiles)) return PNL_ERR_INVALID;
    if (!ctx->b_tiles.p || ctx->cls_n_mixed.empty()) return fail(ctx, PNL_ERR_STATE, "no tile plan yet");
    const std::vector<int2> &st = ctx->settled_tiles;
    if ((int)st.size() != ctx->n_settled) return fail(ctx, PNL_ERR_STATE, "the resident tile list is not that of a dense assembly");
    for (size_t i = 0; i < st.size() && (int64_t)i < ntiles; i++) { tiles[2*i] = st[i].x; tiles[2*i+1] = st[i].y; }
    return (int)st.size();
}

int pnl_get_fold_plan(pnl_context *ctx, int32_t *images, int64_t nimages, int8_t *tile_stage, int8_t *tile_order, int64_t ntiles) {
    if (!ctx) return PNL_ERR_INVALID;
    if (ctx->stg_K <= 0) return fail(ctx, PNL_ERR_STATE, "the resident tile plan has no fold stages");
    const int K = ctx->stg_K;
    const size_t nb2 = (size_t)ctx->nblocks*ctx->nblocks;
    if (images) {
        if (nimages != ctx->stg_img_off[K+1]) return fail(ctx, PNL_ERR_INVALID, "the plan has %d images", ctx->stg_img_off[K+1]);
        for (int s = 0; s <= K; s++)
            for (int i = ctx->stg_img_off[s]; i < ctx->stg_img_off[s+1]; i++) {
                images[3*(size_t)i] = (int32_t)(ctx->stg_img[i] >> 16); images[3*(size_t)i+1] = (int32_t)(ctx->stg_img[i] & 0xffffu);
                images[3*(size_t)i+2] = s;
            }
    }
    if (tile_stage || tile_order) {
        if ((size_t)ntiles != nb2) return fail(ctx, PNL_ERR_INVALID, "the tile tables have %zu entries", nb2);
        if (tile_stage) std::memcpy(tile_stage, ctx->stg_tile_stage.data(), nb2);
        if (tile_order) std::memcpy(tile_order, ctx->stg_tile_q.data(), nb2);
    }
    return PNL_OK;
}

int pnl_get_kernel_ms(pnl_context *ctx, float *out, int n) {
    if (!ctx || !out || n <= 0) return PNL_ERR_INVALID;
    if (!ctx->run.ev_valid) return fail(ctx, PNL_ERR_STATE, "nothing assembled yet");
    HIPCHK(ctx, hipEventSynchronize(ctx->ev[EV_END]));
    for (int s = 0; s < n && s < PNL_NUM_KERNEL_SLOTS; s++) {
        out[s] = 0.f;
        for (int k = 0; k < ctx->run.kev_n[s]; k++) {
            float t = 0.f;
            HIPCHK(ctx, hipEventElapsedTime(&t, ctx->kev[s][2*k], ctx->kev[s][2*k+1]));
            out[s] += t;
        }
    }
    return PNL_OK;
}

}
```

Measured before the change: 62.31 billion element-pairs/s.

## Precompute per-tile sorted pair lists for settled tiles to skip in-kernel classification

Adds a setup kernel that turns each settled tile's 2-bit quadrature-order codes into a compact record: counts per order (4, 3, 2) followed by pair indices grouped by order. The settled tile kernel gains a LISTS variant that copies this record into LDS and walks the grouped pairs directly, skipping the per-tile counting, binning and chunk-building pass it used to run. This trades about 8 KiB of extra device memory per settled tile, plus a one-time list build at plan setup, for less per-tile classification work and fewer barriers at assembly time. It is on by default and can be disabled with PNL_SETTLED_CODES.

```diff
diff --git a/include/pnl_hip.h b/include/pnl_hip.h
--- a/include/pnl_hip.h
+++ b/include/pnl_hip.h
@@ -50,9 +50,10 @@
     PNL_C_UNIFORM_Q2 = 131,
     PNL_C_SETTLED_TILES = 134,
     PNL_C_CODE_BUILDS = 135,
-    PNL_C_WORKLIST_LENGTH = 136
+    PNL_C_WORKLIST_LENGTH = 136,
+    PNL_C_SETTLED_LIST_TILES = 137
 };
-#define PNL_NUM_COUNTERS 137
+#define PNL_NUM_COUNTERS 138
 
 int pnl_set_option(const char *name, const char *value);
 
@@ -167,6 +168,7 @@
 int pnl_get_fold_stages(pnl_context *ctx, int64_t *out, int n);
 int pnl_get_fold_plan(pnl_context *ctx, int32_t *images, int64_t nimages, int8_t *tile_stage, int8_t *tile_order, int64_t ntiles);
 int pnl_get_settled_tiles(pnl_context *ctx, int32_t *tiles, int64_t ntiles);
+int pnl_get_settled_lists(pnl_context *ctx, uint16_t *codes, uint16_t *lists, int64_t ntiles);
 enum pnl_kernel_slot { PNL_K_TILE_GENERAL = 0, PNL_K_TILE_UNIFORM2, PNL_K_TILE_UNIFORM3, PNL_K_TILE_UNIFORM4, PNL_K_FOLD_MIRROR,
                        PNL_K_WORKLIST, PNL_K_TILE_SETTLED, PNL_NUM_KERNEL_SLOTS };
 int pnl_get_kernel_ms(pnl_context *ctx, float *out, int n);
diff --git a/pynucleus_amd/_lib.py b/pynucleus_amd/_lib.py
--- a/pynucleus_amd/_lib.py
+++ b/pynucleus_amd/_lib.py
@@ -15,7 +15,7 @@
 PNL_BOUNDARY = 1
 PNL_FLAG_NO_MIRROR = 1
 PNL_FLAG_SYMMETRIC_FLUSH = 2
-PNL_NUM_COUNTERS = 137
+PNL_NUM_COUNTERS = 138
 
 EXPORTS = ['pnl_create', 'pnl_destroy', 'pnl_error_string', 'pnl_version', 'pnl_set_stream', 'pnl_synchronize',
            'pnl_upload_mesh', 'pnl_upload_dofmap', 'pnl_set_kernel', 'pnl_set_order_formula', 'pnl_upload_distant_rules',
@@ -23,7 +23,7 @@
            'pnl_assemble_dense_tiles', 'pnl_get_counters', 'pnl_get_phase_ms', 'pnl_get_kernel_ms', 'pnl_get_fold_stages', 'pnl_get_fold_plan', 'pnl_get_settled_tiles', 'pnl_tree_build', 'pnl_tree_build_blocks', 'pnl_tree_build_refined', 'pnl_tree_build_horizon', 'pnl_tree_build_device', 'pnl_tree_destroy', 'pnl_tree_sizes', 'pnl_tree_get', 'pnl_tree_node_cells', 'pnl_h2_transfer_matrices', 'pnl_nfplan_build', 'pnl_nfplan_destroy', 'pnl_nfplan_sizes', 'pnl_nfplan_get', 'pnl_horizon_pattern', 'pnl_near_pattern', 'pnl_pattern_set_max_nnz', 'pnl_set_option', 'pnl_set_cell_order', 'pnl_set_interaction_transform', 'pnl_set_order_vertex_values', 'pnl_h2_get', 'pnl_h2_set', 'pnl_pattern_nnz', 'pnl_pattern_get', 'pnl_pattern_destroy', 'pnl_set_row_slab', 'pnl_diag_blocks_size', 'pnl_get_diag_blocks', 'pnl_slab_matvec', 'pnl_slab_diagonal', 'pnl_gemv', 'pnl_cg_jacobi',
            'pnl_inv_diagonal', 'pnl_set_classes', 'pnl_select_class', 'pnl_upload_sparsity', 'pnl_upload_sparsity_device', 'pnl_assemble_pairs_masked', 'pnl_assemble_boundary_masked', 'pnl_assemble_clusters_tiled', 'pnl_h2_setup', 'pnl_h2_matvec', 'pnl_h2_upward', 'pnl_h2_interact', 'pnl_h2_downward', 'pnl_h2_sizes', 'pnl_spmv',
            'pnl_assemble_pairs_in_horizon', 'pnl_assemble_pairs_in_horizon_range', 'pnl_set_nonsymmetric', 'pnl_set_order_function', 'pnl_upload_pointwise_rules', 'pnl_assemble_dense_pointwise',
-           'pnl_assemble_pairs_masked_pointwise', 'pnl_assemble_boundary_masked_pointwise',
+           'pnl_assemble_pairs_masked_pointwise', 'pnl_assemble_boundary_masked_pointwise', 'pnl_get_settled_lists',
            'pnl_gemv_axpby', 'pnl_csr_matvec', 'pnl_mg_create', 'pnl_mg_destroy', 'pnl_mg_cycle', 'pnl_mg_solve', 'pnl_mg_cg', 'pnl_theta_step', 'pnl_selftest',
            'pnl_potrf', 'pnl_potrs', 'pnl_getrf', 'pnl_getrs',
            'pnl_csr_cg_jacobi', 'pnl_fe_space_create', 'pnl_fe_space_destroy', 'pnl_assemble_nonlinearity', 'pnl_imex_create',
@@ -142,6 +142,7 @@
     L.pnl_get_fold_stages.argtypes = [vp, vp, i32]
     L.pnl_get_fold_plan.argtypes = [vp, vp, C.c_int64, vp, vp, C.c_int64]
     L.pnl_get_settled_tiles.argtypes = [vp, vp, C.c_int64]
+    L.pnl_get_settled_lists.argtypes = [vp, vp, vp, C.c_int64]
     L.pnl_set_row_slab.argtypes = [vp, i32, vp, i32, vp]
     L.pnl_tree_build.argtypes = [i32, i32, vp, vp, vp, i32, dbl, i32, i32, i32, C.POINTER(vp)]
     L.pnl_tree_build_blocks.argtypes = [i32, i32, vp, vp, vp, i32, dbl, i32, i32, i32, vp, i32, C.POINTER(vp)]
@@ -524,7 +525,8 @@
         return dict(numCellPairs=int(out[0]), numAssembledCellPairs=int(out[1]), numIntegrations=int(out[2]),
                     numBoundaryPairs=int(out[3]), numBoundaryIntegrations=int(out[4]), orders=hist, singular=sing,
                     uniformTilePairs=int(out[6]), uniformTilePairsByOrder={2+k: int(out[131+k]) for k in range(3)},
-                    settledTiles=int(out[134]), codeBuilds=int(out[135]), workListLength=int(out[136]))
+                    settledTiles=int(out[134]), codeBuilds=int(out[135]), workListLength=int(out[136]),
+                    settledListTiles=int(out[137]))
 
     def phase_ms(self):
         out = np.zeros(7, dtype=np.float32)
@@ -571,6 +573,17 @@
         if n:
             self.check(min(self.L.pnl_get_settled_tiles(self.h, tiles.ctypes.data, n), 0))
         return tiles
+
+    def settled_lists(self):
+        n = self.settled_tiles().shape[0]
+        codes = np.zeros((n, 512), dtype=np.uint16)
+        have = self.L.pnl_get_settled_lists(self.h, codes.ctypes.data if n else None, None, n)
+        self.check(min(have, 0))
+        if not have:
+            return codes, None
+        lists = np.zeros((n, 4104), dtype=np.uint16)
+        self.check(min(self.L.pnl_get_settled_lists(self.h, None, lists.ctypes.data, n), 0))
+        return codes, lists
 
     def fold_plan(self, nblocks):
         nimg = sum(s['images'] for s in self.fold_stages())
diff --git a/pynucleus_amd/csrc/pnl_context.h b/pynucleus_amd/csrc/pnl_context.h
--- a/pynucleus_amd/csrc/pnl_context.h
+++ b/pynucleus_amd/csrc/pnl_context.h
@@ -40,6 +40,7 @@
     bool full_tile_list = false;
     bool slot_used = false, fold_event_set = false, stg_active = false;
     int settled_run = 0;
+    int lists_run = 0;
     int tile_off = 0, n_mixed = 0, n_pure = 0;
     int wl_slots = 0;
     int uni_ctr_next = 0, uni_ctr_fresh = 0;
@@ -96,8 +97,8 @@
     DevBuf b_kcls, b_fcls, b_uni, b_tilecls, b_ttwphif;
     DevBuf b_scolbase, b_srowoff, b_cpoff, b_cpslot, b_cprow, b_foldtab, b_bkcls, b_bfcls, b_bdefer, b_multitiles, b_slotA, b_candtiles, b_candq;
     int slot_S = 0, n_multitiles = 0;
-    DevBuf b_codes;
-    int n_settled = 0, settled_want = -1;
+    DevBuf b_codes, b_lists;
+    int n_settled = 0, settled_want = -1, lists_want = -1;
     std::vector<int2> settled_tiles;
     long long code_builds = 0;
     std::vector<int32_t> rng_blk_off, rng_blk;
@@ -338,6 +339,7 @@
 int pnl_upload_tiles(pnl_context *ctx, std::vector<int2> &tiles, int cell_begin, int cell_end);
 int pnl_tile_order_range(pnl_context *ctx, const DevFormula &qo, int ncand, signed char *host_out);
 int pnl_tile_pair_codes(pnl_context *ctx, const DevFormula &qo, const int2 *tiles, int n, unsigned short *codes, int *host_stat);
+int pnl_tile_pair_lists(pnl_context *ctx, const unsigned short *codes, int n, unsigned short *lists);
 struct WlBins { unsigned *hist, *offs, *coff, *cursor; };
 int pnl_wl_sort(pnl_context *ctx, const int4 *wl, const unsigned *count, unsigned cap, unsigned *aux_base, int4 *sorted, WlBins &B);
 void pnl_scatter_diag(pnl_context *ctx, const DevProblem &P, const double *D, double *A, int64_t ldA);
diff --git a/pynucleus_amd/csrc/pnl_device.h b/pynucleus_amd/csrc/pnl_device.h
--- a/pynucleus_amd/csrc/pnl_device.h
+++ b/pynucleus_amd/csrc/pnl_device.h
@@ -80,6 +80,8 @@
 #ifndef PNL_DIAG_MULT
 #define PNL_DIAG_MULT 21
 #endif
+#define PNL_LIST_HEAD 8
+#define PNL_LIST_STRIDE (PNL_LIST_HEAD+4096)
 __host__ __device__ constexpr int tile_sweep_row(int tid, int k, int tile, int nt) { return k*(nt/tile)+tid/tile; }
 __host__ __device__ constexpr int tile_diag_cell(int r, int j, int tile) { return (r+PNL_DIAG_MULT*j)%tile; }
 
diff --git a/pynucleus_amd/csrc/pnl_hip.hip b/pynucleus_amd/csrc/pnl_hip.hip
--- a/pynucleus_amd/csrc/pnl_hip.hip
+++ b/pynucleus_amd/csrc/pnl_hip.hip
@@ -167,6 +167,14 @@
         return fail(ctx, PNL_ERR_UNSUPPORTED, "a block of %d cells touches %d DoFs: LDS sub-block of %zu bytes exceeds 160 KiB "
                     "(cells must be numbered with spatial locality)", TILE, ctx->nU, lds);
     auto kfun = k_tile_distant<DIM, DPE, TILE, KT, false, false, SETTLED>;
+    const unsigned short *codes = SETTLED ? (const unsigned short*)ctx->b_codes.p : (const unsigned short*)nullptr;
+    if constexpr (can_settle && SETTLED) {
+        if (ctx->b_lists.p) {
+            kfun = k_tile_distant<DIM, DPE, TILE, KT, false, false, true, true>;
+            codes = (const unsigned short*)ctx->b_lists.p;
+            ctx->run.lists_run = ns;
+        }
+    }
     const int grid_mult = pnl_tune("PNL_GRID_MULT") ? atoi(pnl_tune("PNL_GRID_MULT")) : 1;
     const PersistentGrid g = persistent_grid(ctx, kfun, tile_threads(DPE, KT), lds, ntiles, 2, grid_mult);
     if (g.rc) return g.rc;
@@ -181,7 +189,7 @@
                            (const int2*)ctx->b_tiles.p+ctx->run.tile_off+first, A,
                            (long long)ldA, (double*)(ctx->have_tile_order ? ctx->b_Dt.p : ctx->b_D.p), cell_begin, cell_end, acc_stride, (int4*)ctx->b_wl.p,
                            wlc, ctx->wl_cap_each, ctx->ablate | (ctx->run.symflush ? 256 : 0), ntiles, ClusterTiles{},
-                           ctr, SOk, SETTLED ? (const unsigned short*)ctx->b_codes.p : (const unsigned short*)nullptr);
+                           ctr, SOk, codes);
     if (SETTLED) kt_end(ctx, PNL_K_TILE_SETTLED);
     kt_end(ctx, PNL_K_TILE_GENERAL);
     HIPCHK(ctx, hipGetLastError());
@@ -879,6 +887,16 @@
                        host_stat ? (int*)ctx->b_candq.p : (int*)nullptr);
     HIPCHK(ctx, hipGetLastError());
     if (host_stat) HIPCHK(ctx, hipMemcpyAsync(host_stat, ctx->b_candq.p, sizeof(int)*(size_t)n, hipMemcpyDeviceToHost, ctx->stream));
+    HIPCHK(ctx, hipStreamSynchronize(ctx->stream));
+    return PNL_OK;
+}
+
+int pnl_tile_pair_lists(pnl_context *ctx, const unsigned short *codes, int n, unsigned short *lists) {
+    if (n <= 0) return PNL_OK;
+    if (ctx->tile != 64) return fail(ctx, PNL_ERR_STATE, "pair lists: tiles of 64 cells");
+    HIPCHK(ctx, hipMemsetAsync(lists, 0, (size_t)n*PNL_LIST_STRIDE*sizeof(unsigned short), ctx->stream));
+    hipLaunchKernelGGL(k_tile_pair_lists<64>, dim3(std::min(n, 256*8)), dim3(512), 0, ctx->stream, codes, n, lists);
+    HIPCHK(ctx, hipGetLastError());
     HIPCHK(ctx, hipStreamSynchronize(ctx->stream));
     return PNL_OK;
 }
diff --git a/pynucleus_amd/csrc/pnl_kernels.h b/pynucleus_amd/csrc/pnl_kernels.h
--- a/pynucleus_amd/csrc/pnl_kernels.h
+++ b/pynucleus_amd/csrc/pnl_kernels.h
@@ -490,12 +490,13 @@
 #endif
 __host__ __device__ constexpr int tile_threads(int dpe, int kt, bool fh = false) { return (dpe > 3 || (kt == 0 && !PNL_KT0_WIDE) || fh) ? 256 : PNL_TILE_THREADS; }
 __host__ __device__ constexpr int tile_waves(int dpe, int kt, bool fh = false) { return dpe > 3 ? 1 : (((kt == 0 && !PNL_KT0_WIDE) || fh) ? 2 : PNL_TILE_WAVES); }
-template <int DIM, int DPE, int TILE, int KT, bool CLUSTER, bool FH = false, bool SETTLED = false>
+template <int DIM, int DPE, int TILE, int KT, bool CLUSTER, bool FH = false, bool SETTLED = false, bool LISTS = false>
 __global__ void __launch_bounds__(tile_threads(DPE, KT, FH), tile_waves(DPE, KT, FH))
 k_tile_distant(const DevProblem P, const int2 *__restrict__ tiles, double *__restrict__ A, long long ldA,
                double *__restrict__ Dglob, int cell_begin, int cell_end, int acc_stride, int4 *__restrict__ worklist,
                unsigned *__restrict__ wl_count, unsigned wl_cap, int ablate, int ntiles, const ClusterTiles CT,
                unsigned *__restrict__ tile_ctr, const SlotOut SO, const unsigned short *__restrict__ codes) {
+    static_assert(!LISTS || SETTLED, "pair lists: settled tiles only");
     static_assert(!SETTLED || (!CLUSTER && !FH && DIM == 2 && DPE == 3 && TILE*TILE == 8*tile_threads(DPE, KT, FH)),
                   "settled tiles: dense 2D P1, eight pairs per thread");
 #ifdef PNL_DEBUG_ABLATE
@@ -578,7 +579,16 @@
         }
         if (!SETTLED) s_cf[side*TILE+l] = make_int2((vid0 >= 0 ? 1 : 0) | (has_dof ? 2 : 0), __float_as_int((float)P.clog[2*(size_t)P.ncp+c]));
     }
-    if (SETTLED) s_code[tid] = codes[(size_t)tile_idx*NT+tid];
+    if constexpr (LISTS) {
+        static_assert(S::n_int%2 == 0 && S::o_list%4 == 0 && PNL_LIST_HEAD%4 == 0 && PNL_LIST_STRIDE%4 == 0 && 4*2*NT == PAIRS, "8-byte copies of the record");
+        const unsigned short *__restrict__ rec = codes+(size_t)tile_idx*PNL_LIST_STRIDE;
+        const int total = (int)rec[0]+(int)rec[1]+(int)rec[2];
+        if (tid < 3) s_chunk[tid] = rec[tid];
+        const uint2 *__restrict__ src = (const uint2*)(rec+PNL_LIST_HEAD);
+        uint2 *dst = (uint2*)s_list;
+        if (4*tid < total) dst[tid] = src[tid];
+        if (4*(tid+NT) < total) dst[tid+NT] = src[tid+NT];
+    } else if (SETTLED) s_code[tid] = codes[(size_t)tile_idx*NT+tid];
     };
     const bool pipe = !(abl & 256);
     if (pipe) {
@@ -602,9 +612,10 @@
 
     constexpr int NA = (DIM == 2) ? 3 : 2, NB = (DIM == 2) ? 6 : 3;
     int *s_l32 = (int*)(s_list+PAIRS+((((size_t)(s_list+PAIRS)) & 2) ? 1 : 0));
-    int overflow = 0;
     const int lane = tid & 63;
     const unsigned long long lt = (1ull << lane)-1ull;
+    if constexpr (!LISTS) {
+    int overflow = 0;
     int cnt234[3] = {0, 0, 0};
     static_assert(NT%TILE == 0 && PAIRS%NT == 0 && PER_THREAD <= 16, "tile workgroup: whole rows of the tile per sweep");
     constexpr int NG = (PER_THREAD+3)/4;
@@ -727,9 +738,10 @@
         for (int k = 0; k < 3; k++) if (cnt234[k]) atomicAdd(&s_cnt[2+k], cnt234[k]);
     }
     lds_barrier();
+    }
     int next_tile = 0;
     if (tid == 0) next_tile = (int)(gridDim.x+atomicAdd(tile_ctr, 1u));
-    const int nC = __builtin_amdgcn_readfirstlane(s_misc[3]), nBl = __builtin_amdgcn_readfirstlane(s_misc[1]);
+    const int nC = LISTS ? 0 : __builtin_amdgcn_readfirstlane(s_misc[3]), nBl = LISTS ? 0 : __builtin_amdgcn_readfirstlane(s_misc[1]);
     if (nC && tid == 64 && !(abl & 2)) {
         int run = 0, nch = 0;
         for (int q = min(17, P.qmax); q >= 2; q--) {
@@ -793,7 +805,7 @@
     for (int r = 0; r < (PNL_MAXQ+NT)/NT; r++) {
         const int q = 2+tid+r*NT;
         if (q <= P.qmax) {
-            const int cq = s_cnt[q];
+            const int cq = LISTS ? (q <= 4 ? s_chunk[4-q] : 0) : s_cnt[q];
             if (cq) {
                 const int ne = s_ttn[q];
                 const unsigned long long n = (unsigned long long)(ne ? ne : P.off[q+1]-P.off[q]);
@@ -852,8 +864,10 @@
     if (!(abl & 2))
     kern_dispatch<KT, fh>(P.k, lpow, [&](auto ktag) {
     constexpr int KTE = decltype(ktag)::value;
-    const int nAl = __builtin_amdgcn_readfirstlane(s_misc[0]);
-    const int nchC = nC ? __builtin_amdgcn_readfirstlane(s_cnt[0]) : 0, nchB = (nBl+63) >> 6, nchA = (nAl+63) >> 6;
+    const int n4 = LISTS ? __builtin_amdgcn_readfirstlane(s_chunk[0]) : 0, n3 = LISTS ? __builtin_amdgcn_readfirstlane(s_chunk[1]) : 0;
+    const int nAl = __builtin_amdgcn_readfirstlane(LISTS ? s_chunk[2] : s_misc[0]);
+    const int nchC = LISTS ? (n4+63) >> 6 : (nC ? __builtin_amdgcn_readfirstlane(s_cnt[0]) : 0);
+    const int nchB = ((LISTS ? n3 : nBl)+63) >> 6, nchA = (nAl+63) >> 6;
     const int total = nchC+nchB+nchA;
 #pragma unroll 1
     for (;;) {
@@ -863,6 +877,14 @@
         if (c >= total) break;
         int q, p;
         bool act;
+        if constexpr (LISTS) {
+            const int g = c < nchC ? 0 : (c < nchC+nchB ? 1 : 2);
+            const int ng = g == 0 ? n4 : (g == 1 ? n3 : nAl), off = g == 0 ? 0 : (g == 1 ? n4 : n4+n3);
+            const int idx = (c-(g == 0 ? 0 : (g == 1 ? nchC : nchC+nchB)))*64+lane;
+            q = 4-g;
+            act = idx < ng;
+            p = (int)s_list[off+(act ? idx : 0)] & 4095;
+        } else
         if (c < nchC) {
             const int desc = __builtin_amdgcn_readfirstlane(s_chunk[c]);
             const int start = (desc >> 7) & 8191, cnt = (desc & 127)+1;
@@ -3123,3 +3145,45 @@
         __syncthreads();
     }
 }
+
+template <int TILE>
+__global__ void __launch_bounds__(512)
+k_tile_pair_lists(const unsigned short *__restrict__ codes, int ntiles, unsigned short *__restrict__ lists) {
+    constexpr int NT = 512, PER = TILE*TILE/NT, ROWS = NT/TILE;
+    static_assert(PER == 8 && TILE*TILE <= 4096 && PNL_LIST_STRIDE >= PNL_LIST_HEAD+TILE*TILE, "one record holds every pair of a tile");
+    __shared__ unsigned short s_code[NT];
+    __shared__ int s_n[3][NT+1];
+    const int tid = threadIdx.x;
+#pragma unroll 1
+    for (int t = blockIdx.x; t < ntiles; t += gridDim.x) {
+        s_code[tid] = codes[(size_t)t*NT+tid];
+        __syncthreads();
+        int c[PER], n[3] = {0, 0, 0};
+#pragma unroll
+        for (int u = 0; u < PER; u++) {
+            const int p = PER*tid+u, r = p/TILE, j = p%TILE;
+            c[u] = (s_code[(r%ROWS)*TILE+j] >> (2*(r/ROWS))) & 3;
+#pragma unroll
+            for (int g = 0; g < 3; g++) n[g] += c[u] == 3-g ? 1 : 0;
+        }
+#pragma unroll
+        for (int g = 0; g < 3; g++) s_n[g][tid+1] = n[g];
+        __syncthreads();
+        if (tid < 3) {
+            int run = 0;
+            s_n[tid][0] = 0;
+            for (int k = 1; k <= NT; k++) { run += s_n[tid][k]; s_n[tid][k] = run; }
+        }
+        __syncthreads();
+        unsigned short *__restrict__ rec = lists+(size_t)t*PNL_LIST_STRIDE;
+        if (tid < 3) rec[tid] = (unsigned short)s_n[tid][NT];
+        const int n4 = s_n[0][NT], n3 = s_n[1][NT];
+        int pos[3] = {s_n[0][tid], n4+s_n[1][tid], n4+n3+s_n[2][tid]};
+#pragma unroll
+        for (int u = 0; u < PER; u++)
+#pragma unroll
+            for (int g = 0; g < 3; g++)
+                if (c[u] == 3-g) rec[PNL_LIST_HEAD+pos[g]++] = (unsigned short)((PER*tid+u) | ((4-g-2) << 12));
+        __syncthreads();
+    }
+}
diff --git a/pynucleus_amd/csrc/pnl_setup.hip b/pynucleus_amd/csrc/pnl_setup.hip
--- a/pynucleus_amd/csrc/pnl_setup.hip
+++ b/pynucleus_amd/csrc/pnl_setup.hip
@@ -620,7 +620,7 @@
 std::deque<std::string> g_option_values;
 const char *const k_product_options[] = {"PNL_WL_FRAC", "PNL_FH_NOTILES", "PNL_NO_POWTAB", "PNL_VERBOSE", "PNL_PLAN_TIMING", "PNL_PLAN_THREADS", "PNL_BND_OLD",
                                          "PNL_NO_OVERLAP", "PNL_NO_FORK",
-                                         "PNL_TILE_WGS", "PNL_UNI_GENERIC", "PNL_MIXED_GENERIC", "PNL_MIXED_UNSETTLED",
+                                         "PNL_TILE_WGS", "PNL_UNI_GENERIC", "PNL_MIXED_GENERIC", "PNL_MIXED_UNSETTLED", "PNL_SETTLED_CODES",
                                          "PNL_FOLD_STAGES", "PNL_UNI_SPARE", "PNL_BND_MODE"};
 }
 
@@ -1058,12 +1058,13 @@
 
 static int fold_stages_wanted();
 static int settled_wanted() { return pnl_tune("PNL_MIXED_UNSETTLED") ? 0 : 1; }
+static int lists_wanted() { return pnl_tune("PNL_SETTLED_CODES") ? 0 : 1; }
 
 static bool tiles_resident(const pnl_context *ctx, const std::vector<int2> &tiles, const TilePlan &R) {
     const std::vector<pnl_order_formula> &forms = R.forms;
     return tiles.size() == ctx->tiles_cached.size() && ctx->b_tiles.p && ctx->tiles_cb == R.cell_begin && ctx->tiles_ce == R.cell_end &&
         forms.size() == ctx->tiles_forms.size() && std::memcmp(forms.data(), ctx->tiles_forms.data(), sizeof(pnl_order_formula)*R.ncls) == 0 &&
-        ctx->tiles_filter == ctx->run.tile_cell_filter && ctx->stg_want == fold_stages_wanted() && ctx->settled_want == settled_wanted() &&
+        ctx->tiles_filter == ctx->run.tile_cell_filter && ctx->stg_want == fold_stages_wanted() && ctx->settled_want == settled_wanted() && ctx->lists_want == lists_wanted() &&
         (tiles.empty() || std::memcmp(tiles.data(), ctx->tiles_cached.data(), tiles.size()*sizeof(int2)) == 0);
 }
 
@@ -1376,6 +1377,7 @@
         mixed[k].insert(mixed[k].end(), settled.begin(), settled.end());
     }
     if (settled.empty()) ctx->b_codes.release();
+    if (settled.empty() || !lists_wanted()) ctx->b_lists.release();
     ctx->settled_tiles.clear();
     std::vector<int2> all;
     ctx->single_launch = R.p2;
@@ -1397,8 +1399,17 @@
         ctx->n_settled = (int)settled.size();
         ctx->settled_tiles = settled;
         ctx->code_builds++;
+        if (lists_wanted()) {
+            if (ensure(ctx, ctx->b_lists, settled.size()*PNL_LIST_STRIDE*sizeof(unsigned short)) != PNL_OK) {
+                (void)hipGetLastError();
+                ctx->err.clear();
+                ctx->b_lists.release();
+            } else if ((rc = pnl_tile_pair_lists(ctx, (const unsigned short*)ctx->b_codes.p, (int)settled.size(), (unsigned short*)ctx->b_lists.p)))
+                return rc;
+        }
     }
     ctx->settled_want = settled_wanted();
+    ctx->lists_want = lists_wanted();
     ctx->tiles_cached = tiles; ctx->tiles_cb = cell_begin; ctx->tiles_ce = cell_end; ctx->tiles_forms = R.forms;
     ctx->tiles_filter = ctx->run.tile_cell_filter;
     ctx->stg_want = stages_wanted;
@@ -1552,6 +1563,7 @@
     tmp[0] = ctx->run.visited_is_assembled ? tmp[1] : ctx->run.visited_pairs;
     for (int i = 0; i < n && i < PNL_NCOUNTERS; i++) out[i] = (int64_t)tmp[i];
     if (n > PNL_C_SETTLED_TILES) out[PNL_C_SETTLED_TILES] = ctx->run.settled_run;
+    if (n > PNL_C_SETTLED_LIST_TILES) out[PNL_C_SETTLED_LIST_TILES] = ctx->run.lists_run;
     if (n > PNL_C_CODE_BUILDS) out[PNL_C_CODE_BUILDS] = ctx->code_builds;
     if (n > PNL_C_WORKLIST_LENGTH) {
         unsigned wl[PNL_WL_SLOTS];
@@ -1617,6 +1629,19 @@
     return (int)st.size();
 }
 
+int pnl_get_settled_lists(pnl_context *ctx, uint16_t *codes, uint16_t *lists, int64_t ntiles) {
+    if (!ctx || ntiles < 0) return PNL_ERR_INVALID;
+    if (!ctx->b_tiles.p || ctx->cls_n_mixed.empty()) return fail(ctx, PNL_ERR_STATE, "no tile plan yet");
+    const int64_t n = std::min<int64_t>(ntiles, ctx->n_settled);
+    HIPCHK(ctx, hipStreamSynchronize(ctx->stream));
+    if (codes && n > 0) HIPCHK(ctx, hipMemcpy(codes, ctx->b_codes.p, (size_t)n*512*sizeof(uint16_t), hipMemcpyDeviceToHost));
+    if (lists && n > 0) {
+        if (!ctx->b_lists.p) return fail(ctx, PNL_ERR_STATE, "the resident tile plan keeps no pair lists");
+        HIPCHK(ctx, hipMemcpy(lists, ctx->b_lists.p, (size_t)n*PNL_LIST_STRIDE*sizeof(uint16_t), hipMemcpyDeviceToHost));
+    }
+    return ctx->b_lists.p ? ctx->n_settled : 0;
+}
+
 int pnl_get_fold_plan(pnl_context *ctx, int32_t *images, int64_t nimages, int8_t *tile_stage, int8_t *tile_order, int64_t ntiles) {
     if (!ctx) return PNL_ERR_INVALID;
     if (ctx->stg_K <= 0) return fail(ctx, PNL_ERR_STATE, "the resident tile plan has no fold stages");
```

New measurement: 63.21 billion element-pairs/s (median of 6 runs). +1.5%, better.
